# FKGSOFTWARE/TERRA-GAN

Hardware: AMD Instinct MI355X
Metric: DSM tiles/sec train-step (G+D) at 256x256 bs=16 (higher is better)
Workload: dtype f32

## Files before the change

include/terragan_hip.h:

```cpp
#ifndef TERRAGAN_HIP_H
#define TERRAGAN_HIP_H

#include <stddef.h>
#include <stdint.h>

#ifdef __cplusplus
extern "C" {
#endif

typedef void* tg_stream_t;

enum { TG_OK = 0, TG_ERR_ARG = -1, TG_ERR_LAUNCH = -2, TG_ERR_WS = -3 };
enum { TG_ACT_NONE = 0, TG_ACT_RELU = 1, TG_ACT_LEAKY = 2 };
enum { TG_PREC_F32 = 0, TG_PREC_BF16 = 1, TG_PREC_F32_WINO4 = 2 };

typedef struct TgConv {
    int32_t B, H, W, Cin;
    int32_t Ho, Wo, Cout;
    int32_t k, stride, pad;
    int32_t precision;
} TgConv;

int tg_version(void);
const char* tg_last_error(void);


size_t tg_conv_fwd_ws_bytes(const TgConv* g);
int tg_conv_fwd(const TgConv* g, const float* x, const float* in_mask, const float* w,
                const float* bias, const float* ratio, int act, float slope, float* y,
                float* ws, size_t ws_bytes, tg_stream_t stream);

size_t tg_conv_dgrad_ws_bytes(const TgConv* g);
int tg_conv_dgrad(const TgConv* g, const float* dy, const float* w, const float* in_mask,
                  float* dx, int accumulate, float* ws, size_t ws_bytes, tg_stream_t stream);
int tg_conv_dgrad_gated(const TgConv* g, const float* dy, const float* w, const float* in_mask,
                        const float* x_act, int act, float slope, float* dx, float* ws,
                        size_t ws_bytes, tg_stream_t stream);

enum { TG_WPREP_FWD = 0, TG_WPREP_DGRAD = 1 };
size_t tg_conv_wprep_bytes(const TgConv* g, int mode);
int tg_conv_wprep(const TgConv* g, int mode, const float* w, float* wprep, tg_stream_t stream);
size_t tg_conv_wprep_item_bytes(void);
int tg_conv_wprep_item(const TgConv* g, int mode, const float* w, float* wprep, void* item_out);
int tg_conv_wprep_run(const void* items_dev, int n, tg_stream_t stream);
int tg_conv_fwd_p(const TgConv* g, const float* x, const float* in_mask, const float* w, const float* wprep,
                  const float* bias, const float* ratio, int act, float slope, float* y, float* ws,
                  size_t ws_bytes, tg_stream_t stream);
int tg_conv_fwd_pool(const TgConv* g, const float* x, const float* in_mask, const float* w, const float* wprep,
                     const float* bias, const float* ratio, int act, float slope, float* y, float* pool_y, float* ws,
                     size_t ws_bytes, tg_stream_t stream);
int tg_conv_pool_code_supported(const TgConv* g);
int tg_conv_fwd_pool_code(const TgConv* g, const float* x, const float* w, const float* wprep, const float* bias,
                          float* pool_y, unsigned char* code, float* ws, size_t ws_bytes, tg_stream_t stream);
int tg_maxpool2_bwd_code(const float* dout, const unsigned char* code, int B, int Ho, int Wo, int C, float* dx,
                         tg_stream_t stream);
typedef struct TgBnAct {
    const float *mean, *rstd, *gamma, *beta;
    int32_t act;
    float slope;
} TgBnAct;
int tg_conv_bnin_supported(const TgConv* g, int wgrad);
int tg_conv_fwd_bnin(const TgConv* g, const float* x, const TgBnAct* bn, const float* w, const float* bias, int act,
                     float slope, float* y, float* ws, size_t ws_bytes, tg_stream_t stream);
int tg_conv_wgrad_bnin(const TgConv* g, const float* x, const TgBnAct* bn, const float* dy, float* dw, float* db, float* ws,
                       size_t ws_bytes, tg_stream_t stream);
int tg_conv_dgrad_p(const TgConv* g, const float* dy, const float* w, const float* wprep, const float* in_mask,
                    const float* x_act, int act, float slope, float* dx, int accumulate, float* ws,
                    size_t ws_bytes, tg_stream_t stream);
int tg_relu_gate_pack(const float* a, int64_t rows, int C, uint32_t* bits, tg_stream_t stream);
int tg_conv_dgrad_gbits(const TgConv* g, const float* dy, const float* w, const float* wprep, const float* in_mask,
                        const uint32_t* gate_bits, float* dx, int accumulate, float* ws, size_t ws_bytes, tg_stream_t stream);

int tg_set_cu_reserve(int cus);
int tg_set_work_stealing(int mode);

size_t tg_conv_wgrad_ws_bytes(const TgConv* g);
int tg_conv_wgrad(const TgConv* g, const float* x, const float* in_mask, const float* dy,
                  float* dw, float* db, float* ws, size_t ws_bytes, tg_stream_t stream);

int tg_fold_cin(const float* w3, int cout, int taps, int cin, float* w1, tg_stream_t stream);


int tg_mask_update(const float* mask, int B, int H, int W, int k, int stride, int pad, int Ho,
                   int Wo, float* mask_out, float* ratio, tg_stream_t stream);
int tg_mask_up_merge(const float* up_mask, const float* skip_mask, int B, int h, int w, int H,
                     int W, float* out, tg_stream_t stream);

#define TG_MASK_PYRAMID_MAX 24
typedef struct TgMaskOp {
    int kind, H, W, Ho, Wo, k, stride, pad;
    const float* in;
    const float* in2;
    float* out;
    float* out2;
} TgMaskOp;
typedef struct TgMaskPyramid {
    int nops, _pad;
    TgMaskOp op[TG_MASK_PYRAMID_MAX];
} TgMaskPyramid;
int tg_mask_pyramid(const TgMaskPyramid* pm, int B, tg_stream_t stream);


size_t tg_bn_ws_bytes(int64_t rows, int C);
int tg_bn_stats(const float* y, int64_t rows, int C, float eps, float momentum, float* save_mean,
                float* save_rstd, float* running_mean, float* running_var,
                int64_t* num_batches_tracked, float* ws, size_t ws_bytes, tg_stream_t stream);
int tg_bn_fwd(const float* y, int64_t rows, int C, float eps, float momentum, const float* gamma,
              const float* beta, int act, float slope, float* save_mean, float* save_rstd,
              float* running_mean, float* running_var, int64_t* num_batches_tracked, float* out,
              float* ws, size_t ws_bytes, tg_stream_t stream);
int tg_bn_eval_stats(const float* running_mean, const float* running_var, int C, float eps,
                     float* mean, float* rstd, tg_stream_t stream);
int tg_bn_act_fwd(const float* y, int64_t rows, int C, const float* mean, const float* rstd,
                  const float* gamma, const float* beta, int act, float slope, float* out,
                  tg_stream_t stream);
int tg_bn_act_bwd(const float* dout, const float* y, int64_t rows, int C, const float* mean,
                  const float* rstd, const float* gamma, const float* beta, int act, float slope,
                  const float* ratio, float* dy, float* dgamma, float* dbeta, float* dbias, float* ws,
                  size_t ws_bytes, tg_stream_t stream);
int tg_bn_bwd_conv1_supported(int64_t rows, int C);
size_t tg_bn_conv1_ws_bytes(int64_t rows, int C);
int tg_bn_act_bwd_conv1(const float* dz, const float* w, int B, int H, int W, const float* y, int C, const float* mean,
                        const float* rstd, const float* gamma, const float* beta, int act, float slope, const float* ratio,
                        float* dy, float* dgamma, float* dbeta, float* dbias, float* ws, size_t ws_bytes, tg_stream_t stream);
int tg_act_bwd(const float* dout, const float* out, int64_t rows, int C, int act, float slope,
               const float* ratio, float* din, tg_stream_t stream);


int tg_upcat_fwd(const float* up, const float* skip, const float* out_mask, int B, int h, int w,
                 int Cu, int H, int W, int Cs, float* out, tg_stream_t stream);
int tg_upcat_bn_supported(int B, int h, int w, int Cu, int H, int W, int Cs);
int tg_upcat_fwd_bn(const float* up, const TgBnAct* bn, const float* skip, const float* out_mask, int B, int h, int w,
                    int Cu, int H, int W, int Cs, float* out, tg_stream_t stream);
int tg_upcat_bwd(const float* dout, int B, int h, int w, int Cu, int H, int W, int Cs, float* dup,
                 float* dskip, tg_stream_t stream);


int tg_sigmoid_composite_fwd(const float* logits, const float* x, const float* mask, int64_t n,
                             float* out, tg_stream_t stream);
int tg_sigmoid_composite_bwd(const float* dout, const float* logits, const float* mask, int64_t n,
                             float* dlogits, float* dx, tg_stream_t stream);

int tg_maxpool2_fwd(const float* x, int B, int H, int W, int C, float* out, tg_stream_t stream);
int tg_maxpool2_bwd(const float* dout, const float* x, int B, int H, int W, int C, int relu_gate,
                    float* dx, tg_stream_t stream);


size_t tg_pixel_loss_ws_bytes(int B, int H, int W);
int tg_pixel_losses(const float* pred, const float* target, const float* mask,
                    const float* l1_weight, int B, int H, int W,
                    float w_l1, float w_tv, float w_bnd, float bnd_eps, const float* gscale,
                    float* out5, float* dpred, int accumulate, float* ws, size_t ws_bytes,
                    tg_stream_t stream);

size_t tg_reduce_ws_bytes(int64_t n);
int tg_l1_mean(const float* a, const float* b, int64_t n, float coef, const float* gscale,
               float* out1, float* da, float* ws, size_t ws_bytes, tg_stream_t stream);
int tg_l1_mean_relu(const float* a, const float* b, int64_t n, float coef, const float* gscale, float* out1, float* da,
                    float* ws, size_t ws_bytes, tg_stream_t stream);

int tg_bce_logits(const float* z, int64_t n, float target, float coef, const float* gscale,
                  float* out1, float* dz, float* ws, size_t ws_bytes, tg_stream_t stream);


int tg_adam(float* p, const float* g, float* m, float* v, int64_t n, double lr, double beta1,
            double beta2, double eps, int step, float grad_scale, tg_stream_t stream);

typedef struct TgAdamSeg {
    float* p;
    const float* g;
    float* m;
    float* v;
    int64_t n;
} TgAdamSeg;
int tg_adam_multi(const TgAdamSeg* segs_dev, const int32_t* work_dev, int nwork, int chunk_elems,
                  double lr, double beta1, double beta2, double eps, int step, float grad_scale,
                  tg_stream_t stream);

int tg_adam_scalars(double lr, double beta1, double beta2, int step, float* out2_host);
int tg_write_floats(float* dst_dev, int n, const float* vals_host, tg_stream_t stream);
int tg_adam_multi_s(const TgAdamSeg* segs_dev, const int32_t* work_dev, int nwork, int chunk_elems,
                    double beta1, double beta2, double eps, const float* scal_dev, float grad_scale,
                    tg_stream_t stream);

int tg_axpby(const float* x, float a, float b, float* y, int64_t n, tg_stream_t stream);
int tg_lincomb(const float* x, float a, const float* y, float b, float* out, int64_t n,
               tg_stream_t stream);
int tg_mul(const float* a, const float* b, float* out, int64_t n, tg_stream_t stream);
int tg_mul_keep(const float* a, const float* b, float* out, float* a_copy, int64_t n, tg_stream_t stream);
size_t tg_bn_grouped_ws_bytes(int64_t rows_per_group, int groups, int C);
int tg_bn_fwd_grouped(const float* y, int64_t rows_per_group, int groups, int C, float eps, const float* gamma,
                      const float* beta, int act, float slope, float* save_mean, float* save_rstd, float* out,
                      float* ws, size_t ws_bytes, tg_stream_t stream);
int tg_bn_act_bwd_grouped(const float* dout, const float* y, int64_t rows_per_group, int groups, int C,
                          const float* mean, const float* rstd, const float* gamma, const float* beta, int act,
                          float slope, float* dy, float* dgamma, float* dbeta, float* dbias, float* ws,
                          size_t ws_bytes, tg_stream_t stream);
int tg_bn_running_update_multi(const float* save_mean, const float* save_rstd, int64_t rows_per_group, int C,
                               float eps, float momentum, const int* order, int norder, float* running_mean,
                               float* running_var, int64_t* num_batches_tracked, tg_stream_t stream);
int tg_bn_running_update(const float* save_mean, const float* save_rstd, int64_t rows, int C,
                         float eps, float momentum, float* running_mean, float* running_var,
                         int64_t* num_batches_tracked, tg_stream_t stream);
int tg_nchw_to_nhwc(const float* x, int B, int C, int H, int W, float* y, tg_stream_t stream);
int tg_nhwc_to_nchw(const float* x, int B, int C, int H, int W, float* y, tg_stream_t stream);


size_t tg_quality_metrics_ws_bytes(int64_t imgs, int H, int W);
// ... 36 lines not shown
```

terra-gan_amd/csrc/igemm.hip:

```cpp
#include <atomic>
#include <stdlib.h>
#include <string.h>

#include <mutex>
#include <vector>

#include "common.h"

struct ProfRec {
    hipEvent_t a, b;
    int kind;
    double flops, bytes;
    int M, N, K, C, splits, cfg;
    char tag[32];
};
static std::mutex g_prof_mu;
static bool g_prof_on = false;
static std::vector<ProfRec> g_prof;
static thread_local char g_prof_tag[32] = "";

struct ProfScope {
    bool on = false;
    ProfRec r{};
    hipStream_t s;
// ... 1098 lines not shown
        p.splits = cdiv(p.T, p.steps_per_split);
        p.ws = ws + off_f;
        off_f += (size_t)p.splits * p.M * p.N;
        pm.zbeg[i] = i == 0 ? 0 : pm.zbeg[i - 1] + cls[i - 1].splits;
        pm.c[i] = p;
    }
    pm.zbeg[ncls] = pm.zbeg[ncls - 1] + cls[ncls - 1].splits;
    for (int i = ncls; i < 4; ++i) {
        pm.c[i] = pm.c[0];
        pm.zbeg[i + 1] = pm.zbeg[ncls];
    }
    if (cls[0].bf16) *rc = bn == 128 ? launch_igemm_multi_cfg<2, 2, 2, 2, true>(pm, ncls, s) : launch_igemm_multi_cfg<2, 2, 2, 1, true>(pm, ncls, s);
    else *rc = bn == 128 ? launch_igemm_multi_cfg<2, 2, 2, 2, false>(pm, ncls, s) : launch_igemm_multi_cfg<2, 2, 2, 1, false>(pm, ncls, s);
    return true;
}

static int check_conv(const TgConv* g, const char* who) {
    TG_REQUIRE(g != nullptr, "%s: null geometry", who);
    TG_REQUIRE(g->B > 0 && g->H > 0 && g->W > 0 && g->Cin > 0 && g->Cout > 0, "%s: non-positive dims", who);
    TG_REQUIRE(g->k > 0 && g->stride > 0 && g->pad >= 0, "%s: bad k/stride/pad", who);
    TG_REQUIRE(g->Ho == (g->H + 2 * g->pad - g->k) / g->stride + 1 && g->Wo == (g->W + 2 * g->pad - g->k) / g->stride + 1,
               "%s: Ho/Wo (%d,%d) inconsistent with H,W,k,s,p (%d,%d,%d,%d,%d)", who, g->Ho, g->Wo, g->H, g->W, g->k,
               g->stride, g->pad);
    TG_REQUIRE(g->Ho > 0 && g->Wo > 0, "%s: empty output", who);
    TG_REQUIRE((int64_t)g->B * g->H * g->W * (int64_t)g->Cin < (1ll << 31) &&
                   (int64_t)g->B * g->Ho * g->Wo * (int64_t)g->Cout < (1ll << 31),
               "%s: tensor too large for 32-bit pixel indexing", who);
    return TG_OK;
}
static bool aligned16(const void* ptr) { return (reinterpret_cast<uintptr_t>(ptr) & 15) == 0; }

static size_t align_up(size_t v, size_t a) { return (v + a - 1) / a * a; }
#include "wino22.inc"
static size_t conv_wino_floats(const TgConv* g) {
    if (wino22_fwd_geom_ok(g) || wino22_dgrad_geom_ok(g)) return wino22_u_floats(g);
    if (g->k != 3 || g->stride != 1 || (g->Cin % 8) != 0 || (g->Cout % 8) != 0) return 0;
    if (g->precision == TG_PREC_F32_WINO4) return align_up(wino44_u_floats(g->Cout, g->Cin), 64);
    return align_up(wino_u_floats(g->Cout, g->Cin), 64);
}

__global__ __launch_bounds__(256) void s2d_kernel(const float* __restrict__ x, const float* __restrict__ mask, float* __restrict__ x2,
                                                  int B, int H, int W, int C) {
    const int C4 = C >> 2;
    const int64_t total = (int64_t)B * H * W * C4;
    for (int64_t idx = (int64_t)blockIdx.x * 256 + threadIdx.x; idx < total; idx += (int64_t)gridDim.x * 256) {
        const int c4 = (int)(idx % C4);
        int64_t pix = idx / C4;
        const int xw = (int)(pix % W);
        int64_t t = pix / W;
        const int yh = (int)(t % H);
        const int b = (int)(t / H);
        f32x4 v = *reinterpret_cast<const f32x4*>(x + pix * C + 4 * c4);
        if (mask) v *= mask[pix];
        const int64_t p2 = ((int64_t)b * (H >> 1) + (yh >> 1)) * (W >> 1) + (xw >> 1);
        *reinterpret_cast<f32x4*>(x2 + p2 * (4 * C) + ((yh & 1) * 2 + (xw & 1)) * C + 4 * c4) = v;
    }
}
__global__ __launch_bounds__(256) void d2s_kernel(const float* __restrict__ dx2, const float* __restrict__ mask, float* __restrict__ dx,
                                                  int B, int H, int W, int C, int accumulate) {
    const int C4 = C >> 2;
    const int64_t total = (int64_t)B * H * W * C4;
    for (int64_t idx = (int64_t)blockIdx.x * 256 + threadIdx.x; idx < total; idx += (int64_t)gridDim.x * 256) {
        const int c4 = (int)(idx % C4);
        int64_t pix = idx / C4;
        const int xw = (int)(pix % W);
        int64_t t = pix / W;
        const int yh = (int)(t % H);
        const int b = (int)(t / H);
        const int64_t p2 = ((int64_t)b * (H >> 1) + (yh >> 1)) * (W >> 1) + (xw >> 1);
        f32x4 v = *reinterpret_cast<const f32x4*>(dx2 + p2 * (4 * C) + ((yh & 1) * 2 + (xw & 1)) * C + 4 * c4);
        if (mask) v *= mask[pix];
        float* o = dx + pix * C + 4 * c4;
        if (accumulate) v += *reinterpret_cast<const f32x4*>(o);
        *reinterpret_cast<f32x4*>(o) = v;
    }
}
__global__ __launch_bounds__(256) void w5x5_s2d_kernel(const float* __restrict__ src, float* __restrict__ dst, int Cout, int C, int to3) {
    const int64_t total = to3 ? (int64_t)Cout * 36 * C : (int64_t)Cout * 25 * C;
    for (int64_t idx = (int64_t)blockIdx.x * 256 + threadIdx.x; idx < total; idx += (int64_t)gridDim.x * 256) {
        const int c = (int)(idx % C);
        int64_t t = idx / C;
        if (to3) {
            const int ph = (int)(t % 4), tap = (int)((t / 4) % 9), co = (int)(t / 36);
            const int ky = 2 * (tap / 3) + (ph >> 1), kx = 2 * (tap % 3) + (ph & 1);
            dst[idx] = (ky < 5 && kx < 5) ? src[((int64_t)co * 25 + ky * 5 + kx) * C + c] : 0.f;
        } else {
            const int k = (int)(t % 25), co = (int)(t / 25);
            const int ky = k / 5, kx = k % 5;
            dst[idx] = src[(((int64_t)co * 9 + (ky >> 1) * 3 + (kx >> 1)) * 4 + (ky & 1) * 2 + (kx & 1)) * C + c];
        }
    }
}
static bool s2d_ok(const TgConv* g) {
    static const bool off = getenv("TG_NO_WINO") != nullptr || getenv("TG_NO_S2D") != nullptr;
    if (off || (g->precision == TG_PREC_BF16 && getenv("TG_NO_WINO16"))) return false;
    return g->k == 5 && g->stride == 2 && g->pad == 2 && (g->H % 2) == 0 && (g->W % 2) == 0 && (g->Cin % 16) == 0 &&
           (g->Cout % 64) == 0 && g->Ho >= 32 && g->Wo >= 32 && g->Ho == g->H / 2 && g->Wo == g->W / 2;
}
static TgConv s2d_geom(const TgConv* g) {
    TgConv g2 = *g;
    g2.H = g->H / 2; g2.W = g->W / 2; g2.Cin = 4 * g->Cin; g2.k = 3; g2.stride = 1; g2.pad = 1;
    return g2;
}
static size_t s2d_x_floats(const TgConv* g) { return align_up((size_t)g->B * g->H * g->W * g->Cin, 64); }
static size_t s2d_w_floats(const TgConv* g) { return align_up((size_t)g->Cout * 36 * g->Cin, 64); }

static size_t splitk_room_floats(size_t out) {
    const size_t cap = (size_t)64 << 20;
    return out * 64 < cap ? out * 64 : cap;
}
static size_t min_floats(size_t a, size_t b) { return a < b ? a : b; }

extern "C" size_t tg_conv_fwd_ws_bytes(const TgConv* g) {
    if (!g) return 0;
    const size_t out = (size_t)g->B * g->Ho * g->Wo * g->Cout;
    size_t base = (splitk_room_floats(out) + conv_wino_floats(g)) * sizeof(float);
    if (s2d_ok(g)) {
        const TgConv g2 = s2d_geom(g);
        base = (s2d_x_floats(g) + s2d_w_floats(g)) * sizeof(float) + tg_conv_fwd_ws_bytes(&g2);
    }
    return base;
}

static int wino_kc(const TgConv* g) {
    static const bool off16 = getenv("TG_NO_WINO16") != nullptr;
    return g->precision == TG_PREC_BF16 ? (off16 ? 0 : 16) : 8;
}
static bool wino_fwd_geom_ok(const TgConv* g) {
    static const bool off = getenv("TG_NO_WINO") != nullptr;
    const int kc = wino_kc(g);
    return !off && kc && g->k == 3 && g->stride == 1 && (g->Cin % kc) == 0 && (g->Cout % WINO_BN) == 0 && g->Ho >= 16 && g->Wo >= 16;
}
static bool wino_dgrad_geom_ok(const TgConv* g) {
    static const bool off = getenv("TG_NO_WINO") != nullptr;
    const int kc = wino_kc(g);
    return !off && kc && g->k == 3 && g->stride == 1 && (g->Cout % kc) == 0 && (g->Cin % WINO_BN) == 0 && g->H >= 16 && g->W >= 16;
}
static size_t dgrad_wt_floats(const TgConv* g);
extern "C" size_t tg_conv_wprep_bytes(const TgConv* g, int mode) {
    if (!g) return 0;
    if (s2d_ok(g)) {
        const TgConv g2 = s2d_geom(g);
        return s2d_w_floats(g) * sizeof(float) + tg_conv_wprep_bytes(&g2, mode);
    }
    if (mode == TG_WPREP_FWD) return wino_fwd_geom_ok(g) || wino22_fwd_geom_ok(g) ? conv_wino_floats(g) * sizeof(float) : 0;
    if (mode == TG_WPREP_DGRAD) return dgrad_wt_floats(g) * sizeof(float);
    return 0;
}

struct FwdExtras {
    float* pool_dst = nullptr;
    unsigned char* pool_code = nullptr;
    const BnIn* in_bn = nullptr;
    int pool_fused = 0;
};
static int conv_fwd_impl(const TgConv* g, const float* x, const float* in_mask, const float* w, float* wprep, int prep,
                         const float* bias, const float* ratio, int act, float slope, float* y, float* ws, size_t ws_bytes,
                         tg_stream_t stream, float* pool_y = nullptr, FwdExtras* ex = nullptr) {
    if (pool_y) {
        TG_REQUIRE(g && x && y && prep >= 0 && (g->Ho % 2) == 0 && (g->Wo % 2) == 0 && aligned16(pool_y),
                   "tg_conv_fwd_pool: even output sizes and a 16-byte aligned pool_y expected");
        int fused = 0;
        if (!s2d_ok(g) && !wino22_fwd_geom_ok(g)) {
            FwdExtras e;
            e.pool_dst = pool_y;
            const int rc1 = conv_fwd_impl(g, x, in_mask, w, wprep, prep, bias, ratio, act, slope, y, ws, ws_bytes, stream, nullptr, &e);
            if (rc1) return rc1;
            fused = e.pool_fused;
        } else if (int rc1 = conv_fwd_impl(g, x, in_mask, w, wprep, prep, bias, ratio, act, slope, y, ws, ws_bytes, stream)) {
            return rc1;
        }
        return fused ? TG_OK : tg_maxpool2_fwd(y, g->B, g->Ho, g->Wo, g->Cout, pool_y, stream);
    }
    int rc = check_conv(g, "tg_conv_fwd");
    if (rc) return rc;
    TG_REQUIRE(w && (prep < 0 || (x && y)), "tg_conv_fwd: null pointer");
    TG_REQUIRE(aligned16(x) && aligned16(w) && aligned16(y) && aligned16(wprep), "tg_conv_fwd: pointers must be 16-byte aligned");
    TG_REQUIRE(prep == 0 || wprep != nullptr, "tg_conv_fwd: prepared weights expected");
    const bool ws_ok = ws && aligned16(ws) && ws_bytes >= tg_conv_fwd_ws_bytes(g);
    if (s2d_ok(g) && (prep < 0 || ws_ok)) {
        hipStream_t s = (hipStream_t)stream;
        const TgConv g2 = s2d_geom(g);
        float* x2 = ws;
        float* w2 = prep ? wprep : ws + s2d_x_floats(g);
        float* ws2 = ws ? ws + s2d_x_floats(g) + s2d_w_floats(g) : nullptr;
        if (prep < 0 && g_wprep_capture) {
            const int rc2 = conv_fwd_impl(&g2, nullptr, nullptr, w2, wprep + s2d_w_floats(g), -1, nullptr, nullptr, 0, 0.f, nullptr, nullptr,
                                          0, stream);
            if (rc2 == TG_OK && g_wprep_captured == 1 && g_wprep_capture->kind == 1) {
                g_wprep_capture->kind = 4; g_wprep_capture->w = w; g_wprep_capture->taps = g->Cin;
            } else {
                g_wprep_captured = -1;
            }
            return rc2;
        }
        if (prep <= 0) {
            hipLaunchKernelGGL(w5x5_s2d_kernel, dim3(ew_grid((int64_t)g->Cout * 36 * g->Cin, 256)), dim3(256), 0, s, w, w2, g->Cout, g->Cin, 1);
            TG_CHECK_LAUNCH("w5x5_s2d_kernel");
        }
        if (prep >= 0) {
            hipLaunchKernelGGL(s2d_kernel, dim3(ew_grid((int64_t)g->B * g->H * g->W * (g->Cin / 4), 256)), dim3(256), 0, s, x, in_mask, x2,
                               g->B, g->H, g->W, g->Cin);
            TG_CHECK_LAUNCH("s2d_kernel");
        }
        AlgScale sc(25.0 / 36.0);
        return conv_fwd_impl(&g2, x2, nullptr, w2, prep ? wprep + s2d_w_floats(g) : nullptr, prep, bias, ratio, act, slope, y, ws2,
                             ws ? ws_bytes - (s2d_x_floats(g) + s2d_w_floats(g)) * sizeof(float) : 0, stream);
    }
    TG_REQUIRE(!(s2d_ok(g) && prep > 0), "tg_conv_fwd: workspace too small for the prepared 5x5 stride-2 path");
    IGemmParams p = {};
    p.src = x; p.amask = in_mask; p.wmat = w; p.bias = bias; p.rowscale = ratio; p.dst = y; p.ws = ws;
    p.B = g->B; p.IH = g->H; p.IW = g->W; p.C = g->Cin;
    p.OH = g->Ho; p.OW = g->Wo; p.N = g->Cout; p.M = g->B * g->Ho * g->Wo;
    p.DH = g->Ho; p.DW = g->Wo; p.ds = 1; p.dy0 = 0; p.dx0 = 0;
    p.TH = g->k; p.TW = g->k; p.ss = g->stride; p.tstep = 1; p.sy0 = -g->pad; p.sx0 = -g->pad;
    p.KW = g->k; p.kstep = 1; p.ky0 = 0; p.kx0 = 0;
    p.Kfull = g->k * g->k * g->Cin;
    p.act = act; p.slope = slope; p.accumulate = 0;
    p.bf16 = g->precision == TG_PREC_BF16;
    p.wino4 = g->precision == TG_PREC_F32_WINO4;
    p.Ktot = p.TH * p.TW * p.C; p.nchunks = cdiv(p.C, 32);
    p.T = (p.C % 4) ? cdiv(p.Ktot, 32) : p.TH * p.TW * p.nchunks;
    size_t ws_floats = ws ? ws_bytes / sizeof(float) : 0;
    const size_t uf = conv_wino_floats(g);
    const size_t room = splitk_room_floats((size_t)p.M * p.N);
    if (wino22_fwd_geom_ok(g) && (prep || (ws_floats >= uf && aligned16(ws)))) {
        p.w_raw = w;
        p.wino_u = prep ? wprep : ws;
        p.wino_ready = prep;
        if (!prep) {
            p.ws = ws + uf;
            ws_floats -= uf;
        }
        return launch_wino22(g, p, 0, min_floats(ws_floats, room), (hipStream_t)stream);
    }
    if (wino_fwd_geom_ok(g) && (prep || (ws_floats >= uf && aligned16(ws)))) {
        p.w_raw = w; p.w_sn = (long)p.Kfull; p.w_sk = 1; p.w_stap = g->Cin;
        p.wino_u = prep ? wprep : ws;
        p.wino_ready = prep;
        bool in_ws = !prep;
        if (wino44_prepared_unusable(p)) {
            TG_REQUIRE(ws_floats >= uf && aligned16(ws), "tg_conv_fwd: workspace too small to re-prepare the weights (%zu < %zu floats)",
                       ws_floats, uf);
            p.wino_u = ws;
            p.wino_ready = 0;
            in_ws = true;
        }
        TG_REQUIRE(p.bf16 ? wino16_ok(p) : wino_ok(p), "tg_conv_fwd: internal: Winograd geometry predicate mismatch");
        if (in_ws) {
            p.ws = ws + uf;
            ws_floats -= uf;
        }
    }
    if (prep < 0 && !p.wino_u) return TG_OK;
    if (ex) {
        p.pool_dst = ex->pool_dst;
        p.pool_code = ex->pool_code;
        p.pool_only = ex->pool_code != nullptr;
        if (ex->in_bn) {
            p.in_bn = *ex->in_bn;
            TG_REQUIRE(smallconv_bnin_fwd_ok(p), "tg_conv_fwd_bnin: geometry not supported (ask tg_conv_bnin_supported first)");
        }
    }
    ws_floats = min_floats(ws_floats, room);
    plan_splits(p, ws_floats);
    rc = launch_igemm(p, (hipStream_t)stream, ws_floats);
    if (ex) ex->pool_fused = p.pool_done;
    return rc;
}
extern "C" int tg_conv_fwd_pool(const TgConv* g, const float* x, const float* in_mask, const float* w, const float* wprep,
                                const float* bias, const float* ratio, int act, float slope, float* y, float* pool_y, float* ws,
                                size_t ws_bytes, tg_stream_t stream) {
    TG_REQUIRE(pool_y, "tg_conv_fwd_pool: null pointer");
    return conv_fwd_impl(g, x, in_mask, w, const_cast<float*>(wprep), wprep ? 1 : 0, bias, ratio, act, slope, y, ws, ws_bytes, stream,
                         pool_y);
}
extern "C" int tg_conv_pool_code_supported(const TgConv* g) {
    if (!g || (g->precision != TG_PREC_F32 && g->precision != TG_PREC_BF16) || !wino_fwd_geom_ok(g) || s2d_ok(g) || (g->Ho & 1) || (g->Wo & 1)) return 0;
    if (getenv("TG_NO_FUSED_POOL") || getenv("TG_NO_POOL_CODE") || getenv("TG_WINO_NO_PIPE") || getenv("TG_WINO_NO_FAST")) return 0;
    if ((size_t)g->B * g->Ho * g->Wo * g->Cout * 4 >= ((size_t)1 << 31) || (size_t)g->B * g->H * g->W * g->Cin * 4 >= ((size_t)1 << 31)) return 0;
    const int nchunks = g->Cin / wino_kc(g);
    if (nchunks < 2) return 0;
    const long work = (long)cdiv(g->Wo, 16) * cdiv(g->Ho, 16) * g->B * (g->Cout / WINO_BN);
    return nchunks < 16 || work >= 4L * WINO_PLAN_CUS ? 1 : 0;
}
extern "C" int tg_conv_fwd_pool_code(const TgConv* g, const float* x, const float* w, const float* wprep, const float* bias,
                                     float* pool_y, unsigned char* code, float* ws, size_t ws_bytes, tg_stream_t stream) {
    TG_REQUIRE(pool_y && code && aligned16(pool_y) && (reinterpret_cast<uintptr_t>(code) & 3) == 0, "tg_conv_fwd_pool_code: bad pointers");
    TG_REQUIRE(tg_conv_pool_code_supported(g), "tg_conv_fwd_pool_code: geometry not supported (ask tg_conv_pool_code_supported first)");
    FwdExtras e;
    e.pool_dst = pool_y;
    e.pool_code = code;
    const int rc = conv_fwd_impl(g, x, nullptr, w, const_cast<float*>(wprep), wprep ? 1 : 0, bias, nullptr, TG_ACT_RELU, 0.f, pool_y, ws,
                                 ws_bytes, stream, nullptr, &e);
    if (rc) return rc;
    TG_REQUIRE(e.pool_fused, "tg_conv_fwd_pool_code: internal: the launch did not take the fused path");
    return TG_OK;
}
static bool bnin_geom_ok(const TgConv* g) {
    return g && g->Cout == 1 && g->Cin == 64 && g->k == 3 && g->stride == 1 && g->pad == 1 && (g->Wo % 4) == 0;
}
static BnIn bnin_of(const TgBnAct* bn) { return BnIn{bn->mean, bn->rstd, bn->gamma, bn->beta, bn->act, bn->slope}; }
extern "C" int tg_conv_bnin_supported(const TgConv* g, int wgrad) {
    if (!bnin_geom_ok(g)) return 0;
    if (wgrad) {
        WgradParams p = {};
        p.B = g->B; p.H = g->H; p.W = g->W; p.C = g->Cin; p.Ho = g->Ho; p.Wo = g->Wo; p.Cout = g->Cout;
        p.k = g->k; p.stride = g->stride; p.pad = g->pad;
        p.Mpix = g->B * g->Ho * g->Wo; p.Ktot = g->k * g->k * g->Cin;
        return smallconv_wgrad_applies(p) && smallconv_bnin_wgrad_ok(p) ? 1 : 0;
    }
    IGemmParams p = {};
    p.B = g->B; p.IH = g->H; p.IW = g->W; p.C = g->Cin; p.OH = g->Ho; p.OW = g->Wo; p.N = g->Cout; p.M = g->B * g->Ho * g->Wo;
    p.TH = g->k; p.TW = g->k; p.ss = g->stride; p.tstep = 1; p.sy0 = -g->pad; p.sx0 = -g->pad;
    return smallconv_bnin_fwd_ok(p) ? 1 : 0;
}
extern "C" int tg_conv_fwd_bnin(const TgConv* g, const float* x, const TgBnAct* bn, const float* w, const float* bias, int act,
                                float slope, float* y, float* ws, size_t ws_bytes, tg_stream_t stream) {
    TG_REQUIRE(bn && bn->mean && bn->rstd && bn->gamma && bn->beta, "tg_conv_fwd_bnin: null pointer");
    TG_REQUIRE(tg_conv_bnin_supported(g, 0), "tg_conv_fwd_bnin: geometry not supported (ask tg_conv_bnin_supported first)");
    const BnIn b = bnin_of(bn);
    FwdExtras e;
    e.in_bn = &b;
    return conv_fwd_impl(g, x, nullptr, w, nullptr, 0, bias, nullptr, act, slope, y, ws, ws_bytes, stream, nullptr, &e);
}
extern "C" int tg_conv_fwd(const TgConv* g, const float* x, const float* in_mask, const float* w, const float* bias,
                           const float* ratio, int act, float slope, float* y, float* ws, size_t ws_bytes,
                           tg_stream_t stream) {
    return conv_fwd_impl(g, x, in_mask, w, nullptr, 0, bias, ratio, act, slope, y, ws, ws_bytes, stream);
}
extern "C" int tg_conv_fwd_p(const TgConv* g, const float* x, const float* in_mask, const float* w, const float* wprep,
                             const float* bias, const float* ratio, int act, float slope, float* y, float* ws, size_t ws_bytes,
                             tg_stream_t stream) {
    return conv_fwd_impl(g, x, in_mask, w, const_cast<float*>(wprep), wprep ? 1 : 0, bias, ratio, act, slope, y, ws, ws_bytes,
                         stream);
}

__global__ __launch_bounds__(256) void transpose_w_kernel(const float* __restrict__ w, float* __restrict__ wt,
                                                          int cout, int taps, int cin) {
    const size_t total = (size_t)cout * taps * cin;
    for (size_t idx = (size_t)blockIdx.x * 256 + threadIdx.x; idx < total; idx += (size_t)gridDim.x * 256) {
        int co = (int)(idx % cout);
        size_t r = idx / cout;
        int t = (int)(r % taps);
        int ci = (int)(r / taps);
        wt[idx] = w[((size_t)co * taps + t) * cin + ci];
    }
}

static size_t dgrad_wt_floats(const TgConv* g) {
    size_t wt = align_up((size_t)g->Cout * g->k * g->k * g->Cin, 64);
    size_t uf = conv_wino_floats(g);
    return wt > uf ? wt : uf;
}
extern "C" size_t tg_conv_dgrad_ws_bytes(const TgConv* g) {
    if (!g) return 0;
    if (s2d_ok(g)) {
        const TgConv g2 = s2d_geom(g);
        return (s2d_x_floats(g) + s2d_w_floats(g)) * sizeof(float) + tg_conv_dgrad_ws_bytes(&g2);
    }
    return (dgrad_wt_floats(g) + splitk_room_floats((size_t)g->B * g->H * g->W * g->Cin)) * sizeof(float);
}

static int conv_dgrad_impl(const TgConv* g, const float* dy, const float* w, float* wprep, int prep, const float* in_mask, float* dx,
                           int accumulate, const float* gate, int gate_act, float gate_slope, float* ws, size_t ws_bytes,
                           tg_stream_t stream, const uint32_t* gate_bits = nullptr, int* gate_bits_done = nullptr);
extern "C" int tg_conv_dgrad(const TgConv* g, const float* dy, const float* w, const float* in_mask, float* dx,
                             int accumulate, float* ws, size_t ws_bytes, tg_stream_t stream) {
    return conv_dgrad_impl(g, dy, w, nullptr, 0, in_mask, dx, accumulate, nullptr, 0, 0.f, ws, ws_bytes, stream);
}
extern "C" int tg_conv_dgrad_gated(const TgConv* g, const float* dy, const float* w, const float* in_mask, const float* x_act,
                                   int act, float slope, float* dx, float* ws, size_t ws_bytes, tg_stream_t stream) {
    TG_REQUIRE(x_act != nullptr && (act == TG_ACT_RELU || act == TG_ACT_LEAKY), "tg_conv_dgrad_gated: needs x_act and a ReLU/LeakyReLU");
    return conv_dgrad_impl(g, dy, w, nullptr, 0, in_mask, dx, 0, x_act, act, slope, ws, ws_bytes, stream);
}
extern "C" int tg_conv_dgrad_p(const TgConv* g, const float* dy, const float* w, const float* wprep, const float* in_mask,
                               const float* x_act, int act, float slope, float* dx, int accumulate, float* ws, size_t ws_bytes,
                               tg_stream_t stream) {
    TG_REQUIRE(x_act == nullptr || ((act == TG_ACT_RELU || act == TG_ACT_LEAKY) && !accumulate),
               "tg_conv_dgrad_p: a gated dgrad needs a ReLU/LeakyReLU and accumulate == 0");
    const bool usable = wprep != nullptr && !(x_act != nullptr && g && s2d_ok(g));
    return conv_dgrad_impl(g, dy, w, usable ? const_cast<float*>(wprep) : nullptr, usable ? 1 : 0, in_mask, dx, accumulate, x_act,
                           act, slope, ws, ws_bytes, stream);
}
extern "C" int tg_conv_dgrad_gbits(const TgConv* g, const float* dy, const float* w, const float* wprep, const float* in_mask,
                                   const uint32_t* gate_bits, float* dx, int accumulate, float* ws, size_t ws_bytes, tg_stream_t stream) {
    int rc = check_conv(g, "tg_conv_dgrad_gbits");
    if (rc) return rc;
    TG_REQUIRE(dy && w && gate_bits && dx && ws, "tg_conv_dgrad_gbits: null pointer");
    TG_REQUIRE(!accumulate, "tg_conv_dgrad_gbits: a gated dgrad does not accumulate");
    TG_REQUIRE(g->Cin % 32 == 0, "tg_conv_dgrad_gbits: needs Cin %% 32 == 0 (one gate word per 32 channels), got %d", g->Cin);
    TG_REQUIRE((reinterpret_cast<uintptr_t>(gate_bits) & 15) == 0, "tg_conv_dgrad_gbits: pointers must be 16-byte aligned");
    const bool usable = wprep != nullptr && !s2d_ok(g);
    int done = 0;
    rc = conv_dgrad_impl(g, dy, w, usable ? const_cast<float*>(wprep) : nullptr, usable ? 1 : 0, in_mask, dx, 0, nullptr, TG_ACT_NONE, 0.f,
                         ws, ws_bytes, stream, gate_bits, &done);
    if (rc || done) return rc;
    return gate_bits_apply_launch(dx, gate_bits, (int64_t)g->B * g->H * g->W, g->Cin, (hipStream_t)stream);
}
extern "C" int tg_conv_wprep(const TgConv* g, int mode, const float* w, float* wprep, tg_stream_t stream) {
    TG_REQUIRE(g && w && wprep, "tg_conv_wprep: null pointer");
    TG_REQUIRE(mode == TG_WPREP_FWD || mode == TG_WPREP_DGRAD, "tg_conv_wprep: bad mode %d", mode);
    TG_REQUIRE(tg_conv_wprep_bytes(g, mode) > 0, "tg_conv_wprep: this (geometry, mode) runs on the raw weights");
    if (mode == TG_WPREP_FWD)
        return conv_fwd_impl(g, nullptr, nullptr, w, wprep, -1, nullptr, nullptr, 0, 0.f, nullptr, nullptr, 0, stream);
    return conv_dgrad_impl(g, nullptr, w, wprep, -1, nullptr, nullptr, 0, nullptr, 0, 0.f, nullptr, 0, stream);
}
extern "C" size_t tg_conv_wprep_item_bytes(void) { return sizeof(TgWprepItem); }
extern "C" int tg_conv_wprep_item(const TgConv* g, int mode, const float* w, float* wprep, void* item_out) {
    if (!g || !w || !wprep || !item_out || (mode != TG_WPREP_FWD && mode != TG_WPREP_DGRAD)) return 0;
    if (tg_conv_wprep_bytes(g, mode) == 0) return 0;
    TgWprepItem it = {};
    g_wprep_capture = &it;
    g_wprep_captured = 0;
    int rc = mode == TG_WPREP_FWD ? conv_fwd_impl(g, nullptr, nullptr, w, wprep, -1, nullptr, nullptr, 0, 0.f, nullptr, nullptr, 0, nullptr)
                                  : conv_dgrad_impl(g, nullptr, w, wprep, -1, nullptr, nullptr, 0, nullptr, 0, 0.f, nullptr, 0, nullptr);
    g_wprep_capture = nullptr;
    if (rc != TG_OK || g_wprep_captured != 1) return 0;
    memcpy(item_out, &it, sizeof(it));
    return 1;
}
extern "C" int tg_conv_wprep_run(const void* items_dev, int n, tg_stream_t stream) {
    TG_REQUIRE(items_dev && n > 0, "tg_conv_wprep_run: bad arguments");
    hipLaunchKernelGGL(wprep_multi_kernel, dim3(2048, n), dim3(256), 0, (hipStream_t)stream, static_cast<const TgWprepItem*>(items_dev));
    TG_CHECK_LAUNCH("wprep_multi_kernel");
    return TG_OK;
}
static int conv_dgrad_impl(const TgConv* g, const float* dy, const float* w, float* wprep, int prep, const float* in_mask, float* dx,
                           int accumulate, const float* gate, int gate_act, float gate_slope, float* ws, size_t ws_bytes,
                           tg_stream_t stream, const uint32_t* gate_bits, int* gate_bits_done) {
    int rc = check_conv(g, "tg_conv_dgrad");
    if (rc) return rc;
    TG_REQUIRE(w && (prep < 0 || (dy && dx && ws)), "tg_conv_dgrad: null pointer");
    TG_REQUIRE(aligned16(dy) && aligned16(w) && aligned16(dx) && aligned16(ws) && aligned16(wprep),
               "tg_conv_dgrad: pointers must be 16-byte aligned");
    TG_REQUIRE(prep == 0 || wprep != nullptr, "tg_conv_dgrad: prepared weights expected");
    if (s2d_ok(g) && gate == nullptr && gate_bits == nullptr && (prep < 0 || ws_bytes >= tg_conv_dgrad_ws_bytes(g))) {
        hipStream_t s2 = (hipStream_t)stream;
        const TgConv g2 = s2d_geom(g);
        float* dx2 = ws;
        float* w2 = prep ? wprep : ws + s2d_x_floats(g);
        float* wsr = ws ? ws + s2d_x_floats(g) + s2d_w_floats(g) : nullptr;
        if (prep < 0 && g_wprep_capture) {
            const int rc2 = conv_dgrad_impl(&g2, nullptr, w2, wprep + s2d_w_floats(g), -1, nullptr, nullptr, 0, nullptr, 0, 0.f, nullptr, 0, stream);
            if (rc2 == TG_OK && g_wprep_captured == 1 && g_wprep_capture->kind == 1) {
                g_wprep_capture->kind = 4; g_wprep_capture->w = w; g_wprep_capture->taps = g->Cin;
            } else {
                g_wprep_captured = -1;
            }
            return rc2;
// ... 816 lines not shown
```

terra-gan_amd/csrc/igemm_params.h:

```cpp
#pragma once
#include "common.h"

struct BnIn {
    const float *mean, *rstd, *gamma, *beta;
    int act;
    float slope;
};
struct IGemmParams {
    const float* src;
    const float* amask;
    const float* wmat;
    const float* bias;
    const float* rowscale;
    float* dst;
    float* ws;
    int B, IH, IW, C;
    int OH, OW, N, M;
    int DH, DW, ds, dy0, dx0;
    int TH, TW, ss, tstep, sy0, sx0;
    int KW, kstep, ky0, kx0;
    int Kfull, Ktot;
    int nchunks, T;
    int splits, steps_per_split;
    int act;
    float slope;
    int accumulate;
    int bf16;
    const float* gate;
    int gate_act;
    float gate_slope;
    const float* w_raw;
    long w_sn, w_sk, w_stap;
    float* wino_u;
    int wino4;
    int wino_ready;
    float* pool_dst;
    int pool_done;
    unsigned char* pool_code;
    int pool_only;
    BnIn in_bn;
    const uint32_t* gate_bits;
    int gate_bits_done;
};
__device__ __forceinline__ float gate_factor(const IGemmParams& p, size_t idx) {
    const float gv = p.gate[idx];
    return gv > 0.f ? 1.f : (p.gate_act == TG_ACT_LEAKY ? p.gate_slope : 0.f);
}

int gate_bits_apply_launch(float* dx, const uint32_t* bits, int64_t rows, int C, hipStream_t s);

struct IGemmMulti {
    IGemmParams c[4];
    int zbeg[5];
};

struct WgradParams {
    const float* x;
    const float* amask;
    const float* dy;
    float* out;
    int B, H, W, C, Ho, Wo, Cout, k, stride, pad;
    int Mpix, Ktot, T, splits, steps_per_split;
    int nx, ny;
    int rowseg;
    BnIn in_bn;
};

bool smallconv_fwd_applies(const IGemmParams& p);
int smallconv_fwd_launch(const IGemmParams& p, hipStream_t s);
bool smallconv_to1_multi_applies(const IGemmParams* cls, int ncls);
int smallconv_to1_multi_launch(const IGemmParams* cls, int ncls, hipStream_t s);
bool smallconv_wgrad_applies(const WgradParams& p);
bool smallconv_bnin_fwd_ok(const IGemmParams& p);
bool smallconv_bnin_wgrad_ok(const WgradParams& p);
size_t smallconv_wgrad_ws_floats(const WgradParams& p);
int smallconv_wgrad_launch(const WgradParams& p, float* dw, float* ws, size_t ws_floats, hipStream_t s, float* db = nullptr,
                           int* db_done = nullptr);
```

terra-gan_amd/csrc/pointwise.hip:

```cpp
#include <math.h>
#include <string.h>

#include "common.h"

static thread_local char g_err[512] = "";
void tg_set_error(const char* fmt, ...) {
    va_list ap;
    va_start(ap, fmt);
    vsnprintf(g_err, sizeof(g_err), fmt, ap);
    va_end(ap);
}
extern "C" const char* tg_last_error(void) { return g_err; }
extern "C" int tg_version(void) { return 100; }

static size_t align_up(size_t v, size_t a) { return (v + a - 1) / a * a; }
static inline hipStream_t S(tg_stream_t s) { return (hipStream_t)s; }

constexpr int CR_MAXPASS = 4;

struct ColGeom {
    int cpp;
    int rlanes;
    int npass;
    int grid;
// ... 158 lines not shown
    const float* x;
    int C;
    __device__ void operator()(int64_t r, int c, float (&q)[1]) const { q[0] += x[r * C + c]; }
};
__global__ __launch_bounds__(256) void colsum_final_kernel(const float* __restrict__ partial, int nblocks, int C,
                                                           float* __restrict__ out) {
    double s[1];
    int c;
    if (final_reduce<1>(partial, nblocks, C, s, &c)) out[c] = (float)s[0];
}
size_t tg_colsum_ws_floats(int64_t rows, int C) {
    ColGeom g = col_geom(rows, C);
    return align_up((size_t)g.grid * C, 64);
}
int tg_colsum_launch(const float* x, int64_t rows, int C, float* out, float* ws, hipStream_t s) {
    TG_REQUIRE(C >= 1 && C <= 1024, "colsum: C=%d out of range [1,1024]", C);
    ColGeom g = col_geom(rows, C);
    ColSumF f{x, C};
    hipLaunchKernelGGL((colreduce_kernel<1, ColSumF>), dim3(g.grid), dim3(256), 0, s, f, rows, C, g.cpp, g.rlanes,
                       g.rows_per_block, ws);
    TG_CHECK_LAUNCH("colsum");
    hipLaunchKernelGGL(colsum_final_kernel, dim3(fr_grid(C)), dim3(256), 0, s, ws, g.grid, C, out);
    TG_CHECK_LAUNCH("colsum_final");
    return TG_OK;
}

__global__ __launch_bounds__(256) void mask_update_kernel(const float* __restrict__ mask, int B, int H, int W, int k,
                                                          int stride, int pad, int Ho, int Wo,
                                                          float* __restrict__ mask_out, float* __restrict__ ratio) {
    const int64_t total = (int64_t)B * Ho * Wo;
    for (int64_t idx = (int64_t)blockIdx.x * 256 + threadIdx.x; idx < total; idx += (int64_t)gridDim.x * 256) {
        int ox = (int)(idx % Wo);
        int64_t t = idx / Wo;
        int oy = (int)(t % Ho);
        int b = (int)(t / Ho);
        float s = 0.f;
        for (int ky = 0; ky < k; ++ky) {
            int iy = oy * stride - pad + ky;
            if (iy < 0 || iy >= H) continue;
            for (int kx = 0; kx < k; ++kx) {
                int ix = ox * stride - pad + kx;
                if (ix < 0 || ix >= W) continue;
                s += mask[((int64_t)b * H + iy) * W + ix];
            }
        }
        const float on = s > 0.f ? 1.f : 0.f;
        mask_out[idx] = on;
        ratio[idx] = (1.0f / (s + 1e-8f)) * (float)(k * k) * on;
    }
}
extern "C" int tg_mask_update(const float* mask, int B, int H, int W, int k, int stride, int pad, int Ho, int Wo,
                              float* mask_out, float* ratio, tg_stream_t stream) {
    TG_REQUIRE(mask && mask_out && ratio, "tg_mask_update: null pointer");
    TG_REQUIRE(B > 0 && H > 0 && W > 0 && k > 0 && stride > 0 && pad >= 0, "tg_mask_update: bad dims");
    TG_REQUIRE(Ho == (H + 2 * pad - k) / stride + 1 && Wo == (W + 2 * pad - k) / stride + 1 && Ho > 0 && Wo > 0,
               "tg_mask_update: Ho/Wo inconsistent");
    hipLaunchKernelGGL(mask_update_kernel, dim3(ew_grid((int64_t)B * Ho * Wo, 256)), dim3(256), 0, S(stream), mask, B, H, W,
                       k, stride, pad, Ho, Wo, mask_out, ratio);
    TG_CHECK_LAUNCH("mask_update_kernel");
    return TG_OK;
}

__host__ __device__ inline int floordiv2(int a) { return a >= 0 ? a / 2 : -((-a + 1) / 2); }

__global__ __launch_bounds__(256) void mask_up_merge_kernel(const float* __restrict__ up, const float* __restrict__ skip,
                                                            int B, int h, int w, int H, int W, int offy, int offx,
                                                            float* __restrict__ out) {
    const int64_t total = (int64_t)B * H * W;
    for (int64_t idx = (int64_t)blockIdx.x * 256 + threadIdx.x; idx < total; idx += (int64_t)gridDim.x * 256) {
        int X = (int)(idx % W);
        int64_t t = idx / W;
        int Y = (int)(t % H);
        int b = (int)(t / H);
        int yu = Y - offy, xu = X - offx;
        float v = 0.f;
        if (yu >= 0 && yu < 2 * h && xu >= 0 && xu < 2 * w) v = up[((int64_t)b * h + (yu >> 1)) * w + (xu >> 1)];
        out[idx] = fmaxf(v, skip[idx]);
    }
}
extern "C" int tg_mask_up_merge(const float* up_mask, const float* skip_mask, int B, int h, int w, int H, int W,
                                float* out, tg_stream_t stream) {
    TG_REQUIRE(up_mask && skip_mask && out && B > 0 && h > 0 && w > 0 && H > 0 && W > 0, "tg_mask_up_merge: bad arguments");
    hipLaunchKernelGGL(mask_up_merge_kernel, dim3(ew_grid((int64_t)B * H * W, 256)), dim3(256), 0, S(stream), up_mask,
                       skip_mask, B, h, w, H, W, floordiv2(H - 2 * h), floordiv2(W - 2 * w), out);
    TG_CHECK_LAUNCH("mask_up_merge_kernel");
    return TG_OK;
}


__device__ __forceinline__ void mask_update_one(const float* __restrict__ mask, int H, int W, int k, int stride, int pad, int Ho,
                                                int Wo, int b, int idx, float* __restrict__ mask_out, float* __restrict__ ratio) {
    const int ox = idx % Wo, oy = idx / Wo;
    float s = 0.f;
    if (k == 3) {
        float v[9];
#pragma unroll
        for (int t = 0; t < 9; ++t) {
            const int iy = oy * stride - pad + t / 3, ix = ox * stride - pad + t % 3;
            const bool ok = iy >= 0 && iy < H && ix >= 0 && ix < W;
            const float m = mask[((int64_t)b * H + (ok ? iy : 0)) * W + (ok ? ix : 0)];
            v[t] = ok ? m : 0.f;
        }
#pragma unroll
        for (int t = 0; t < 9; ++t) s += v[t];
    } else {
        for (int ky = 0; ky < k; ++ky) {
            const int iy = oy * stride - pad + ky;
            if (iy < 0 || iy >= H) continue;
            for (int kx = 0; kx < k; ++kx) {
                const int ix = ox * stride - pad + kx;
                if (ix < 0 || ix >= W) continue;
                s += mask[((int64_t)b * H + iy) * W + ix];
            }
        }
    }
    const float on = s > 0.f ? 1.f : 0.f;
    const int64_t o = ((int64_t)b * Ho + oy) * Wo + ox;
    mask_out[o] = on;
    ratio[o] = (1.0f / (s + 1e-8f)) * (float)(k * k) * on;
}
__global__ __launch_bounds__(1024) void mask_pyramid_kernel(const TgMaskPyramid pm) {
    const int b = blockIdx.x;
    for (int i = 0; i < pm.nops; ++i) {
        const TgMaskOp op = pm.op[i];
        if (op.kind == 0) {
            for (int idx = threadIdx.x; idx < op.Ho * op.Wo; idx += 1024)
                mask_update_one(op.in, op.H, op.W, op.k, op.stride, op.pad, op.Ho, op.Wo, b, idx, op.out, op.out2);
        } else {
            const int offy = floordiv2(op.Ho - 2 * op.H), offx = floordiv2(op.Wo - 2 * op.W);
            for (int idx = threadIdx.x; idx < op.Ho * op.Wo; idx += 1024) {
                const int X = idx % op.Wo, Y = idx / op.Wo;
                const int yu = Y - offy, xu = X - offx;
                float v = 0.f;
                if (yu >= 0 && yu < 2 * op.H && xu >= 0 && xu < 2 * op.W) v = op.in[((int64_t)b * op.H + (yu >> 1)) * op.W + (xu >> 1)];
                const int64_t o = ((int64_t)b * op.Ho + Y) * op.Wo + X;
                op.out[o] = fmaxf(v, op.in2[o]);
            }
        }
        __syncthreads();
    }
}
extern "C" int tg_mask_pyramid(const TgMaskPyramid* pm, int B, tg_stream_t stream) {
    TG_REQUIRE(pm && B > 0 && pm->nops >= 1 && pm->nops <= TG_MASK_PYRAMID_MAX, "tg_mask_pyramid: bad arguments");
    for (int i = 0; i < pm->nops; ++i) {
        const TgMaskOp& op = pm->op[i];
        TG_REQUIRE(op.in && op.out && (op.kind == 0 ? op.out2 != nullptr : op.in2 != nullptr), "tg_mask_pyramid: op %d: null pointer", i);
        TG_REQUIRE(op.H > 0 && op.W > 0 && op.Ho > 0 && op.Wo > 0, "tg_mask_pyramid: op %d: bad dims", i);
        if (op.kind == 0)
            TG_REQUIRE(op.k > 0 && op.stride > 0 && op.pad >= 0 && op.Ho == (op.H + 2 * op.pad - op.k) / op.stride + 1 &&
                       op.Wo == (op.W + 2 * op.pad - op.k) / op.stride + 1, "tg_mask_pyramid: op %d: Ho/Wo inconsistent", i);
    }
    hipLaunchKernelGGL(mask_pyramid_kernel, dim3(B), dim3(1024), 0, S(stream), *pm);
    TG_CHECK_LAUNCH("mask_pyramid_kernel");
    return TG_OK;
}

struct BnStatF {
    const float* y;
    int C;
    __device__ BnStatF group(int g, int64_t rows_g) const { return BnStatF{y + (size_t)g * rows_g * C, C}; }
    __device__ void operator()(int64_t r, int c, float (&q)[2]) const {
        float d = y[r * C + c] - y[c];
        q[0] += d;
        q[1] += d * d;
    }
    __device__ void quad(int64_t r, int c0, float (&q)[2][4]) const {
        const f32x4 v = *reinterpret_cast<const f32x4*>(y + r * C + c0);
        const f32x4 sh = *reinterpret_cast<const f32x4*>(y + c0);
#pragma unroll
        for (int e = 0; e < 4; ++e) {
            float d = v[e] - sh[e];
            q[0][e] += d;
            q[1][e] += d * d;
        }
    }
};
__global__ __launch_bounds__(256) void bn_finalize_kernel(const float* __restrict__ partial, int nblocks, int C,
                                                          const float* __restrict__ y, int64_t rows, float eps,
                                                          float momentum, float* __restrict__ mean_out,
                                                          float* __restrict__ rstd_out, float* __restrict__ rm,
                                                          float* __restrict__ rv, int64_t* __restrict__ nbt) {
    if (blockIdx.x == 0 && threadIdx.x == 0 && nbt) *nbt += 1;
    double q[2];
    int c;
    if (!final_reduce<2>(partial, nblocks, C, q, &c)) return;
    const double n = (double)rows;
    const double md = q[0] / n;
    double var = q[1] / n - md * md;
    if (var < 0.0) var = 0.0;
    const double mean = (double)y[c] + md;
    mean_out[c] = (float)mean;
    rstd_out[c] = (float)(1.0 / sqrt(var + (double)eps));
    if (rm) rm[c] = (float)((1.0 - (double)momentum) * (double)rm[c] + (double)momentum * mean);
    if (rv) rv[c] = (float)((1.0 - (double)momentum) * (double)rv[c] + (double)momentum * var * (n / (n - 1.0)));
}
extern "C" size_t tg_bn_ws_bytes(int64_t rows, int C) {
    if (rows <= 0 || C <= 0) return 0;
    ColGeom g = col_geom(rows, C);
    int grid = g.grid;
    if (C % 4 == 0) {
        ColGeom4 g4 = col_geom4(rows, C);
        if (g4.grid > grid) grid = g4.grid;
    }
    return align_up((size_t)grid * 5 * C, 64) * sizeof(float);
}
extern "C" int tg_bn_stats(const float* y, int64_t rows, int C, float eps, float momentum, float* save_mean,
                           float* save_rstd, float* running_mean, float* running_var, int64_t* num_batches_tracked,
                           float* ws, size_t ws_bytes, tg_stream_t stream) {
    TG_REQUIRE(y && save_mean && save_rstd && ws, "tg_bn_stats: null pointer");
    TG_REQUIRE(C >= 1 && C <= 1024, "tg_bn_stats: C=%d out of range [1,1024]", C);
    TG_REQUIRE(rows > 1, "tg_bn_stats: Expected more than 1 value per channel when training (rows=%lld)", (long long)rows);
    TG_REQUIRE(ws_bytes >= tg_bn_ws_bytes(rows, C), "tg_bn_stats: workspace too small");
    BnStatF f{y, C};
    int nblocks;
    if (C % 4 == 0) {
        ColGeom4 g = col_geom4(rows, C);
        nblocks = g.grid;
        hipLaunchKernelGGL((colreduce4_kernel<2, BnStatF>), dim3(g.grid), dim3(256), 0, S(stream), f, rows, C, g.qpp, g.rlanes,
                           g.rows_per_block, ws, 0);
    } else {
        ColGeom g = col_geom(rows, C);
        nblocks = g.grid;
        hipLaunchKernelGGL((colreduce_kernel<2, BnStatF>), dim3(g.grid), dim3(256), 0, S(stream), f, rows, C, g.cpp, g.rlanes,
                           g.rows_per_block, ws);
    }
    TG_CHECK_LAUNCH("bn_stats");
    hipLaunchKernelGGL(bn_finalize_kernel, dim3(fr_grid(C)), dim3(256), 0, S(stream), ws, nblocks, C, y, rows, eps,
                       momentum, save_mean, save_rstd, running_mean, running_var, num_batches_tracked);
    TG_CHECK_LAUNCH("bn_finalize");
    return TG_OK;
}

__global__ __launch_bounds__(256) void bn_eval_stats_kernel(const float* rm, const float* rv, int C, float eps, float* mean,
                                                            float* rstd) {
    int c = blockIdx.x * 256 + threadIdx.x;
    if (c >= C) return;
    mean[c] = rm[c];
    rstd[c] = 1.0f / sqrtf(rv[c] + eps);
}
extern "C" int tg_bn_eval_stats(const float* running_mean, const float* running_var, int C, float eps, float* mean,
                                float* rstd, tg_stream_t stream) {
    TG_REQUIRE(running_mean && running_var && mean && rstd && C > 0, "tg_bn_eval_stats: bad arguments");
    hipLaunchKernelGGL(bn_eval_stats_kernel, dim3(cdiv(C, 256)), dim3(256), 0, S(stream), running_mean, running_var, C, eps,
                       mean, rstd);
    TG_CHECK_LAUNCH("bn_eval_stats_kernel");
    return TG_OK;
}

__global__ __launch_bounds__(256) void bn_act_fwd4_kernel(const float* __restrict__ y, int64_t rows, int C, int qpp, int rlanes,
                                                          const float* __restrict__ mean, const float* __restrict__ rstd,
                                                          const float* __restrict__ gamma, const float* __restrict__ beta,
                                                          int act, float slope, float* __restrict__ out) {
    const int cq = threadIdx.x % qpp, rl = threadIdx.x / qpp;
    if (rl >= rlanes) return;
    const int nquads = C >> 2;
    for (int q0 = blockIdx.y * qpp; q0 < nquads; q0 += gridDim.y * qpp) {
        const int c0 = (q0 + cq) * 4;
        if (c0 >= C) continue;
        const f32x4 mv = *reinterpret_cast<const f32x4*>(mean + c0), rv = *reinterpret_cast<const f32x4*>(rstd + c0);
        const f32x4 gv = *reinterpret_cast<const f32x4*>(gamma + c0), bv = *reinterpret_cast<const f32x4*>(beta + c0);
        for (int64_t r = (int64_t)blockIdx.x * rlanes + rl; r < rows; r += (int64_t)gridDim.x * rlanes) {
            const f32x4 v = *reinterpret_cast<const f32x4*>(y + r * C + c0);
            f32x4 o;
#pragma unroll
            for (int e = 0; e < 4; ++e) o[e] = apply_act(bn_affine(v[e], mv[e], rv[e], gv[e], bv[e]), act, slope);
            *reinterpret_cast<f32x4*>(out + r * C + c0) = o;
        }
    }
}
__global__ __launch_bounds__(256) void bn_act_fwd1_kernel(const float* __restrict__ y, int64_t total, int C,
                                                          const float* __restrict__ mean, const float* __restrict__ rstd,
                                                          const float* __restrict__ gamma, const float* __restrict__ beta,
                                                          int act, float slope, float* __restrict__ out) {
    for (int64_t i = (int64_t)blockIdx.x * 256 + threadIdx.x; i < total; i += (int64_t)gridDim.x * 256) {
        const int c = (int)(i % C);
        float xh = (y[i] - mean[c]) * rstd[c];
        out[i] = apply_act(xh * gamma[c] + beta[c], act, slope);
    }
}
struct RowGeom {
    int qpp, rlanes;
    dim3 grid;
};
static RowGeom row_geom(int64_t rows, int C) {
    RowGeom g;
    const int nquads = C / 4;
    g.qpp = nquads < 256 ? nquads : 256;
    g.rlanes = 256 / g.qpp;
    int64_t gx = cdiv64(rows, (int64_t)g.rlanes * 4);
    if (gx > 2048) gx = 2048;
    if (gx < 1) gx = 1;
    g.grid = dim3((unsigned)gx, (unsigned)cdiv(nquads, g.qpp));
    return g;
}
extern "C" int tg_bn_act_fwd(const float* y, int64_t rows, int C, const float* mean, const float* rstd, const float* gamma,
                             const float* beta, int act, float slope, float* out, tg_stream_t stream) {
    TG_REQUIRE(y && mean && rstd && gamma && beta && out && rows > 0 && C > 0, "tg_bn_act_fwd: bad arguments");
    if (C % 4 == 0) {
        RowGeom g = row_geom(rows, C);
        hipLaunchKernelGGL(bn_act_fwd4_kernel, g.grid, dim3(256), 0, S(stream), y, rows, C, g.qpp, g.rlanes, mean, rstd, gamma,
                           beta, act, slope, out);
    } else {
        hipLaunchKernelGGL(bn_act_fwd1_kernel, dim3(ew_grid(rows * C, 256)), dim3(256), 0, S(stream), y, rows * C, C, mean, rstd,
                           gamma, beta, act, slope, out);
    }
    TG_CHECK_LAUNCH("bn_act_fwd_kernel");
// ... 1697 lines not shown
```

terra-gan_amd/csrc/wino.inc:

```
#pragma once
#include <utility>

struct WinoGeom {
    int tiles_x, tiles_y, total_work, chunks_per_split, nt;
    int sy_min, sx_min;
    int interleave;
    int* qctr;
};
struct WinoWeights {
    long sn, sk, stap;
    int kyu[3], kxv[3];
    int k_fast;
};
typedef unsigned int u32x4 __attribute__((ext_vector_type(4)));
constexpr int WINO_BN = 64;
constexpr int WINO_V = 16 * 64 * 8;
constexpr int WINO_U = 16 * WINO_BN * 8;
constexpr int WINO_PPIX = 18 * 18;
constexpr int WINO_P = WINO_PPIX * 8;
constexpr int WINO_LDS_FLOATS = 2 * WINO_V + 2 * WINO_U + WINO_P;
constexpr int WINO_THREADS = 512;

__device__ __forceinline__ void wino_barrier() { asm volatile("s_waitcnt lgkmcnt(0)\n\ts_barrier" ::: "memory"); }

template <class F, int... T>
__device__ __forceinline__ void wino_static_for(std::integer_sequence<int, T...>, F&& f) {
    (f(std::integral_constant<int, T>{}), ...);
}

__device__ __forceinline__ void wino_distribute(int total, int interleave, int& item, int& item_end, int& step) {
    const int G = gridDim.x;
    if (interleave) {
        const int xcd = blockIdx.x & 7, slot = blockIdx.x >> 3, nslots = (G - xcd + 7) >> 3;
        const int ch_q = total >> 3, ch_r = total & 7;
        const int chunk0 = xcd < ch_r ? xcd * (ch_q + 1) : ch_r * (ch_q + 1) + (xcd - ch_r) * ch_q;
        item = chunk0 + slot;
        item_end = chunk0 + ch_q + (xcd < ch_r ? 1 : 0);
        step = nslots;
    } else {
        const int rblk = xcd_remap(blockIdx.x, G);
        const int per = total / G, rem = total % G;
        item = rblk * per + min(rblk, rem);
        item_end = item + per + (rblk < rem ? 1 : 0);
        step = 1;
    }
}

constexpr int WQ_Z = 16;
constexpr int WQ_INTS = 8 * WQ_Z + 8;
__device__ __forceinline__ int wq_chunk0(int total, int c) { const int q = total >> 3, r = total & 7; return c < r ? c * (q + 1) : r * (q + 1) + (c - r) * q; }
__device__ __forceinline__ int wq_len(int total, int c) { return (total >> 3) + (c < (total & 7) ? 1 : 0); }
template <bool STEAL>
struct WinoWork {
    int item;
    int item_end, step;
    int* home_ctr;
    int home_c0, home_len;

    __device__ __forceinline__ void init(int total, int interleave, int* ctr, int* slot) {
        if constexpr (!STEAL) {
            wino_distribute(total, interleave, item, item_end, step);
            if (item >= item_end) item = -1;
        } else {
            const int home = blockIdx.x & 7, rank = blockIdx.x >> 3;
            const int nwg = (gridDim.x - home + 7) >> 3;
            const int len = wq_len(total, home), c0 = wq_chunk0(total, home);
            home_ctr = ctr + 8 * blockIdx.z + home;
            home_c0 = c0 + nwg;
            home_len = len - nwg;
            item = rank < len ? c0 + rank : -1;
            step = 0; item_end = 0;
            if (threadIdx.x == 0) {
                int nx = -1;
                if (item >= 0 && home_len > 0) {
                    const int i = atomicAdd(home_ctr, 1);
                    if (i < home_len) nx = home_c0 + i;
                }
                slot[0] = nx;
            }
            __syncthreads();
        }
    }
    __device__ __forceinline__ int next(const int* slot) const {
        if constexpr (!STEAL) return item + step < item_end ? item + step : -1;
        else return __builtin_amdgcn_readfirstlane(slot[step]);
    }
    __device__ __forceinline__ int request(int nxt) const {
        int r = -1;
        if constexpr (STEAL) {
            if (threadIdx.x == 0 && nxt >= 0) {
                const int i = atomicAdd(home_ctr, 1);
                r = i < home_len ? home_c0 + i : -1;
            }
        }
        return r;
    }
    __device__ __forceinline__ void publish(int pulled, int* slot) const {
        if constexpr (STEAL) { if (threadIdx.x == 0) slot[step ^ 1] = pulled; }
    }
    __device__ __forceinline__ void advance(int nxt) {
        item = nxt;
        if constexpr (STEAL) step ^= 1;
    }
    __device__ __forceinline__ void done(int* ctr) const {
        if constexpr (STEAL) {
            if (threadIdx.x == 0) {
                const int n = gridDim.x * gridDim.z;
                if (atomicAdd(ctr + 8 * WQ_Z, 1) == n - 1) {
                    for (int i = 0; i <= 8 * WQ_Z; ++i) __hip_atomic_store(ctr + i, 0, __ATOMIC_RELAXED, __HIP_MEMORY_SCOPE_AGENT);
                }
            }
        }
    }
};

static bool wino_interleave_ok(size_t u_bytes) {
    static const char* e = getenv("TG_WINO_INTERLEAVE");
    if (e) return atoi(e) != 0;
    return u_bytes <= ((size_t)6 << 20);
}

__host__ __device__ __forceinline__ int wino_swz(int row, int kk) { return ((((kk >> 2) ^ (row >> 4)) & 1) << 2) + (kk & 3); }

template <bool S2D>
__device__ __forceinline__ void wino_weights_body(const float* __restrict__ w, float* __restrict__ U, int N, int K,
                                                  const WinoWeights& ww, int cin5 = 0) {
    const int NT = N / WINO_BN;
    const size_t total = (size_t)N * K;
    const int KC = K >> 3;
    for (size_t idx = (size_t)blockIdx.x * 256 + threadIdx.x; idx < total; idx += (size_t)gridDim.x * 256) {
        const int blk = (int)(idx >> 9);
        const int k = (blk % KC) * 8 + (int)(idx & 7), n = (blk / KC) * WINO_BN + (int)((idx >> 3) & 63);
        float g[3][3];
        if constexpr (S2D) {
            const int c2 = ww.k_fast ? k : n, co = ww.k_fast ? n : k;
            const int ph = c2 / cin5, c = c2 - ph * cin5, dy = ph >> 1, dx = ph & 1;
            const float* wp = w + (size_t)co * 25 * cin5 + c;
#pragma unroll
            for (int u = 0; u < 3; ++u)
#pragma unroll
                for (int v = 0; v < 3; ++v) {
                    const int ky = 2 * ww.kyu[u] + dy, kx = 2 * ww.kxv[v] + dx;
                    g[u][v] = (ky < 5 && kx < 5) ? wp[(size_t)(ky * 5 + kx) * cin5] : 0.f;
                }
        } else {
            const float* wp = w + (size_t)n * ww.sn + (size_t)k * ww.sk;
#pragma unroll
            for (int u = 0; u < 3; ++u)
#pragma unroll
                for (int v = 0; v < 3; ++v) g[u][v] = wp[(size_t)(ww.kyu[u] * 3 + ww.kxv[v]) * ww.stap];
        }
        float tg[4][3];
#pragma unroll
        for (int v = 0; v < 3; ++v) {
            tg[0][v] = g[0][v];
            tg[1][v] = 0.5f * (g[0][v] + g[1][v] + g[2][v]);
            tg[2][v] = 0.5f * (g[0][v] - g[1][v] + g[2][v]);
            tg[3][v] = g[2][v];
        }
        const int row = n % WINO_BN;
// ... 164 lines not shown

    if (wk.item < 0 || c_begin >= c_end) { wk.done(q.qctr); return; }
    locate();
    decode();
#pragma unroll
    for (int i = 0; i < 2; ++i) pload1(c_begin, i);
#pragma unroll
    for (int j = 0; j < 4; ++j) uload1(c_begin, j);

    for (;;) {
    f32x16 acc[8];
#pragma unroll
    for (int i = 0; i < 8; ++i)
#pragma unroll
        for (int r = 0; r < 16; ++r) acc[i][r] = 0.f;

    {
#pragma unroll
        for (int i = 0; i < 2; ++i) pstore1(i);
#pragma unroll
        for (int j = 0; j < 4; ++j) ustore1(0, j);
#pragma unroll
        for (int i = 0; i < 2; ++i) pload1(min(c_begin + 1, c_last), i);
#pragma unroll
        for (int j = 0; j < 4; ++j) uload1(min(c_begin + 1, c_last), j);
        wino_barrier();
#pragma unroll
        for (int k = 0; k < 8; ++k) t_read1(k);
#pragma unroll
        for (int j = 0; j < 4; ++j) t_row1(j);
#pragma unroll
        for (int k = 0; k < 4; ++k) t_col1(0, k);
        wino_barrier();
        f32x4 fa[2], fb[2];
        fa[0] = *reinterpret_cast<const f32x4*>(Vs + a_off);
        fb[0] = *reinterpret_cast<const f32x4*>(Us + b_off);
        int cur = 0;
        for (int c = c_begin; c < c_end; ++c) {
            const int nxt = cur ^ 1;
            const int c2 = min(c + 2, c_last);
            const float* Vc = Vs + cur * WINO_V + a_off;
            const float* Uc = Us + cur * WINO_U + b_off;
            const float* Vn = Vs + nxt * WINO_V + a_off;
            const float* Un = Us + nxt * WINO_U + b_off;
            wino_static_for(std::make_integer_sequence<int, 32>{}, [&](auto tc) {
                constexpr int t = decltype(tc)::value;
                constexpr int xi = t >> 2, e = t & 3;
                if constexpr (t < 2) pstore1(t);
                if constexpr (t >= 2 && t < 4) pload1(c2, t - 2);
                if constexpr (t == 4) wino_barrier();
                if constexpr (t >= 5 && t < 9) { t_read1(t - 5); t_read1(4 + t - 5); }
                if constexpr (t >= 8 && t < 12) { t_row1(t - 8); }
                if constexpr (t >= 14 && t < 18) t_col1(nxt, t - 14);
                if constexpr (t >= 18 && t < 22) ustore1(nxt, t - 18);
                if constexpr (t >= 22 && t < 26) uload1(c2, t - 22);
                if constexpr (t == 26) wino_barrier();
                if constexpr (e == 0 && xi < 7) {
                    fa[(xi + 1) & 1] = *reinterpret_cast<const f32x4*>(Vc + (xi + 1) * 512);
                    fb[(xi + 1) & 1] = *reinterpret_cast<const f32x4*>(Uc + (xi + 1) * 512);
                }
                if constexpr (e == 0 && xi == 7) {
                    fa[0] = *reinterpret_cast<const f32x4*>(Vn);
                    fb[0] = *reinterpret_cast<const f32x4*>(Un);
                }
                __builtin_amdgcn_sched_barrier(0);
                acc[xi] = __builtin_amdgcn_mfma_f32_32x32x2f32(fa[xi & 1][e], fb[xi & 1][e], acc[xi], 0, 0, 0);
                __builtin_amdgcn_sched_barrier(0);
            });
            cur = nxt;
        }
    }
    const int e_n0 = n0, e_oy0 = oy0, e_ox0 = ox0, e_b = b;
    const int wq_next = wk.next(wq_slot);
    const bool more_items = wq_next >= 0;
    const int wq_pulled = wk.request(wq_next);
    wino_barrier();

    float* X = smem;
    float* scratch = smem + 16 * 1024 + wave * (32 * 36);
    f32x16 own[2];
#pragma unroll
    for (int j = 0; j < 2; ++j) {
        float* xs = X + (((xh * 2 + nw) * 2 + mw) * 2 + j) * 1024 + lane;
#pragma unroll
        for (int r = 0; r < 16; ++r) {
            const float s0 = j == 0 ? acc[0][r] + acc[1][r] + acc[2][r] : acc[1][r] - acc[2][r] - acc[3][r];
            const float s1 = j == 0 ? acc[4][r] + acc[5][r] + acc[6][r] : acc[5][r] - acc[6][r] - acc[7][r];
            own[j][r] = xh == 0 ? s0 + s1 : -s0 - s1;
            xs[r * 64] = xh == 0 ? s1 : s0;
        }
    }
    if (more_items) {
        wk.item = wq_next;
        locate();
        decode();
#pragma unroll
        for (int i = 0; i < 2; ++i) pload1(c_begin, i);
#pragma unroll
        for (int j = 0; j < 4; ++j) uload1(c_begin, j);
    }
    wino_barrier();
    constexpr bool gated = GATED;
    f32x4 bq = {0.f, 0.f, 0.f, 0.f};
    if (p.bias && p.splits == 1) bq = *reinterpret_cast<const f32x4*>(p.bias + e_n0 + 32 * nw + 4 * (lane & 7));
    float rsq[2][4] = {{1.f, 1.f, 1.f, 1.f}, {1.f, 1.f, 1.f, 1.f}};
    if (p.rowscale && p.splits == 1) {
#pragma unroll
        for (int j = 0; j < 2; ++j)
#pragma unroll
            for (int t4 = 0; t4 < 4; ++t4) {
                const int t = 32 * mw + (lane >> 3) + 8 * t4;
                const int oy = min(e_oy0 + 2 * (t >> 3) + xh, p.OH - 1), ox = min(e_ox0 + 2 * (t & 7) + j, p.OW - 1);
                rsq[j][t4] = p.rowscale[((size_t)e_b * p.DH + (oy * p.ds + p.dy0)) * p.DW + (ox * p.ds + p.dx0)];
            }
    }
#pragma unroll
    for (int j = 0; j < 2; ++j) {
        f32x4 gq[GATED ? 4 : 1];
        if constexpr (gated) {
#pragma unroll
            for (int t4 = 0; t4 < 4; ++t4) {
                const int t = 32 * mw + (lane >> 3) + 8 * t4;
                const int oy = min(e_oy0 + 2 * (t >> 3) + xh, p.OH - 1), ox = min(e_ox0 + 2 * (t & 7) + j, p.OW - 1);
                const size_t pix = ((size_t)e_b * p.DH + (oy * p.ds + p.dy0)) * p.DW + (ox * p.ds + p.dx0);
                gq[t4] = *reinterpret_cast<const f32x4*>(p.gate + pix * p.N + e_n0 + 32 * nw + 4 * (lane & 7));
            }
        }
        const float* xr = X + ((((xh ^ 1) * 2 + nw) * 2 + mw) * 2 + j) * 1024 + lane;
        f32x16 y;
#pragma unroll
        for (int r = 0; r < 16; ++r) y[r] = own[j][r] + xr[r * 64];
        tile_rows4i(scratch, y, lane, [&](int t4, int rr, int cc, f32x4 v4) {
            const int t = 32 * mw + rr;
            const int oy = e_oy0 + 2 * (t >> 3) + xh, ox = e_ox0 + 2 * (t & 7) + j;
            const int nb = e_n0 + 32 * nw + cc;
            if (oy >= p.OH || ox >= p.OW) return;
            if (p.splits > 1) {
                const size_t m = ((size_t)e_b * p.OH + oy) * p.OW + ox;
                *reinterpret_cast<f32x4*>(p.ws + ((size_t)blockIdx.z * p.M + m) * p.N + nb) = v4;
            } else {
                const size_t pix = ((size_t)e_b * p.DH + (oy * p.ds + p.dy0)) * p.DW + (ox * p.ds + p.dx0);
                *reinterpret_cast<f32x4*>(p.dst + pix * p.N + nb) = epilogue4(p, v4, pix, nb, gated ? &gq[gated ? t4 : 0] : nullptr, &rsq[j][t4], &bq);
            }
        });
    }
    wk.publish(wq_pulled, wq_slot);
    if (!more_items) break;
    wino_barrier();
    wk.advance(wq_next);
    }
    wk.done(q.qctr);
}

template <bool GATED, bool STEAL, bool POOL = false, bool GBITS = false>
__global__ __launch_bounds__(WINO_THREADS) void wino_pipe_kernel(const IGemmParams p, const WinoGeom q, const float* __restrict__ U) {
    extern __shared__ __attribute__((aligned(16))) float smem[];
    float* Vs = smem;
    float* Us = smem + 2 * WINO_V;
    float* Ps = smem + 2 * WINO_V + 2 * WINO_U;

    const int tid = threadIdx.x, lane = tid & 63, wave = tid >> 6;
    const int mw = wave & 1, nw = (wave >> 1) & 1, xh = wave >> 2;
    __shared__ int wq_slot[2];
    WinoWork<STEAL> wk;
    wk.init(q.total_work, q.interleave, q.qctr, wq_slot);

    struct Item { int nt, n0, oy0, ox0, b; uint32_t poff[2]; };
    auto decode_item = [&](int it) {
        Item r;
        r.nt = it % q.nt;
        int tile = it / q.nt;
        const int tx = tile % q.tiles_x;
        tile /= q.tiles_x;
        const int ty = tile % q.tiles_y;
        r.b = tile / q.tiles_y;
        r.n0 = r.nt * WINO_BN; r.oy0 = ty * 16; r.ox0 = tx * 16;
        const int py0 = r.oy0 + q.sy_min, px0 = r.ox0 + q.sx_min;
#pragma unroll
        for (int i = 0; i < 2; ++i) {
            const int pp = (tid + WINO_THREADS * i) >> 1, spy = pp / 18, spx = pp - spy * 18;
            const int iy = py0 + spy, ix = px0 + spx;
            r.poff[i] = 0x80000000u;
            if (pp < WINO_PPIX && iy >= 0 && iy < p.IH && ix >= 0 && ix < p.IW)
                r.poff[i] = ((((uint32_t)r.b * p.IH + iy) * p.IW + ix) * (uint32_t)p.C + 4 * (tid & 1)) * 4u;
        }
        return r;
    };
    const auto srsrc = __builtin_amdgcn_make_buffer_rsrc(const_cast<float*>(p.src), 0, (int)((size_t)p.B * p.IH * p.IW * p.C * 4), 0x00020000);
    const auto ursrc = __builtin_amdgcn_make_buffer_rsrc(const_cast<float*>(U), 0, (int)((size_t)16 * p.N * p.C * 4), 0x00020000);
    const uint32_t u_voff = tid * 16;
    const bool p1_ok = ((tid + WINO_THREADS) >> 1) < WINO_PPIX;
    const int c_begin = blockIdx.z * q.chunks_per_split;
    const int c_end = min(p.C >> 3, c_begin + q.chunks_per_split);
    const size_t ustep = (size_t)q.nt * WINO_U;

    f32x4 ru[4], rp[2];
    auto pload1 = [&](uint32_t voff, int c, int i) { rp[i] = __builtin_bit_cast(f32x4, __builtin_amdgcn_raw_buffer_load_b128(srsrc, voff, c * 32, 0)); };
    auto uload1 = [&](int nt, int c, int j) {
        ru[j] = __builtin_bit_cast(f32x4, __builtin_amdgcn_raw_buffer_load_b128(
            ursrc, u_voff, (int)(((size_t)nt * WINO_U + (size_t)c * ustep) * 4) + 16 * WINO_THREADS * j, 0));
    };
    auto pstore1 = [&](int i) { if (i == 0 || p1_ok) *reinterpret_cast<f32x4*>(Ps + 4 * (tid + WINO_THREADS * i)) = rp[i]; };
    auto ustore1 = [&](int buf, int j) { *reinterpret_cast<f32x4*>(Us + buf * WINO_U + 4 * (tid + WINO_THREADS * j)) = ru[j]; };

    const int t_quad = lane & 1, t_tile = (lane >> 1) + 32 * (wave & 1), t_a = wave >> 1;
    const int t_r0 = t_a == 0 ? 0 : (t_a == 2 ? 2 : 1), t_r1 = t_a == 3 ? 3 : (t_a == 2 ? 1 : 2);
    const float t_s1 = t_a == 1 ? 1.f : -1.f;
    const int t_src0 = ((2 * (t_tile >> 3) + t_r0) * 18 + 2 * (t_tile & 7)) * 8 + 4 * t_quad;
    const int t_src1 = ((2 * (t_tile >> 3) + t_r1) * 18 + 2 * (t_tile & 7)) * 8 + 4 * t_quad;
    const int t_dst = (t_a * 4) * 512 + t_tile * 8 + (((t_quad ^ (t_tile >> 4)) & 1) << 2);
    f32x4 td[2][4], tt[4];
    auto t_read1 = [&](int k) { td[k >> 2][k & 3] = *reinterpret_cast<const f32x4*>(Ps + ((k >> 2) ? t_src1 : t_src0) + (k & 3) * 8); };
    auto t_row1 = [&](int j) { tt[j] = td[0][j] + td[1][j] * t_s1; };
    auto t_col1 = [&](int buf, int k) {
        const f32x4 v = k == 0 ? tt[0] - tt[2] : k == 1 ? tt[1] + tt[2] : k == 2 ? tt[2] - tt[1] : tt[1] - tt[3];
        *reinterpret_cast<f32x4*>(Vs + buf * WINO_V + t_dst + k * 512) = v;
    };

    const int arow = 32 * mw + (lane & 31), brow = 32 * nw + (lane & 31);
    const int a_off = (8 * xh) * 512 + arow * 8 + ((((lane >> 5) ^ (arow >> 4)) & 1) << 2);
    const int b_off = (8 * xh) * 512 + brow * 8 + ((((lane >> 5) ^ (brow >> 4)) & 1) << 2);

    if (wk.item < 0 || c_begin >= c_end) { wk.done(q.qctr); return; }
    Item ci = decode_item(wk.item);
#pragma unroll
    for (int i = 0; i < 2; ++i) pload1(ci.poff[i], c_begin, i);
#pragma unroll
    for (int j = 0; j < 4; ++j) uload1(ci.nt, c_begin, j);
#pragma unroll
    for (int i = 0; i < 2; ++i) pstore1(i);
#pragma unroll
    for (int j = 0; j < 4; ++j) ustore1(0, j);
#pragma unroll
    for (int i = 0; i < 2; ++i) pload1(ci.poff[i], c_begin + 1, i);
#pragma unroll
    for (int j = 0; j < 4; ++j) uload1(ci.nt, c_begin + 1, j);
    wino_barrier();
#pragma unroll
    for (int k = 0; k < 8; ++k) t_read1(k);
#pragma unroll
    for (int j = 0; j < 4; ++j) t_row1(j);
#pragma unroll
    for (int k = 0; k < 4; ++k) t_col1(0, k);
    wino_barrier();
    int cur = 0;

    for (;;) {
        f32x16 acc[8];
#pragma unroll
        for (int i = 0; i < 8; ++i)
#pragma unroll
            for (int r = 0; r < 16; ++r) acc[i][r] = 0.f;
        const int wq_next = wk.next(wq_slot);
        const bool more_items = wq_next >= 0;
        const Item ni = decode_item(more_items ? wq_next : wk.item);
        f32x4 fa[2], fb[2];
        fa[0] = *reinterpret_cast<const f32x4*>(Vs + cur * WINO_V + a_off);
        fb[0] = *reinterpret_cast<const f32x4*>(Us + cur * WINO_U + b_off);
        auto kstep = [&](uint32_t pv0, uint32_t pv1, int unt, int c2) {
            const int nxt = cur ^ 1;
            const float* Vc = Vs + cur * WINO_V + a_off;
            const float* Uc = Us + cur * WINO_U + b_off;
            const float* Vn = Vs + nxt * WINO_V + a_off;
            const float* Un = Us + nxt * WINO_U + b_off;
            wino_static_for(std::make_integer_sequence<int, 32>{}, [&](auto tc) {
                constexpr int t = decltype(tc)::value;
                constexpr int xi = t >> 2, e = t & 3;
                if constexpr (t < 2) pstore1(t);
                if constexpr (t == 2) pload1(pv0, c2, 0);
                if constexpr (t == 3) pload1(pv1, c2, 1);
                if constexpr (t == 4) wino_barrier();
                if constexpr (t >= 5 && t < 9) { t_read1(t - 5); t_read1(4 + t - 5); }
                if constexpr (t >= 8 && t < 12) { t_row1(t - 8); }
                if constexpr (t >= 14 && t < 18) t_col1(nxt, t - 14);
                if constexpr (t >= 18 && t < 22) ustore1(nxt, t - 18);
                if constexpr (t >= 22 && t < 26) uload1(unt, c2, t - 22);
                if constexpr (t == 26) wino_barrier();
                if constexpr (e == 0 && xi < 7) {
                    fa[(xi + 1) & 1] = *reinterpret_cast<const f32x4*>(Vc + (xi + 1) * 512);
                    fb[(xi + 1) & 1] = *reinterpret_cast<const f32x4*>(Uc + (xi + 1) * 512);
                }
                if constexpr (e == 0 && xi == 7) {
                    fa[0] = *reinterpret_cast<const f32x4*>(Vn);
                    fb[0] = *reinterpret_cast<const f32x4*>(Un);
                }
                __builtin_amdgcn_sched_barrier(0);
                acc[xi] = __builtin_amdgcn_mfma_f32_32x32x2f32(fa[xi & 1][e], fb[xi & 1][e], acc[xi], 0, 0, 0);
                __builtin_amdgcn_sched_barrier(0);
            });
            cur = nxt;
        };
        for (int c = c_begin; c < c_end - 2; ++c) kstep(ci.poff[0], ci.poff[1], ci.nt, c + 2);
        kstep(ni.poff[0], ni.poff[1], ni.nt, c_begin);
        kstep(ni.poff[0], ni.poff[1], ni.nt, c_begin + 1);
        const int wq_pulled = wk.request(wk.next(wq_slot));
        const int fr = cur ^ 1;
        float* X = Vs + fr * WINO_V;
        float* scratch = wave < 7 ? Us + fr * WINO_U + wave * (32 * 36) : Ps;
        const int e_wave = __builtin_amdgcn_readfirstlane(wave);
        const int e_mw = e_wave & 1, e_nw = (e_wave >> 1) & 1, e_xh = e_wave >> 2;
        const int e_row0 = ci.oy0 + 8 * e_mw + e_xh;
        const int e_pitch = p.DW * p.ds;
        const int e_pix0 = (ci.b * p.DH + p.dy0) * p.DW + p.dx0 + ci.ox0 * p.ds;
        const int e_nb0 = ci.n0 + 32 * e_nw;
        const uint32_t e_lane_px = 2 * (lane >> 3) * p.ds;
        const bool e_single = p.splits == 1;
        const float act_neg = p.act == TG_ACT_RELU ? 0.f : (p.act == TG_ACT_LEAKY ? p.slope : 1.f);
        const float gate_neg = p.gate_act == TG_ACT_LEAKY ? p.gate_slope : 0.f;
        const auto drsrc = __builtin_amdgcn_make_buffer_rsrc(p.dst, 0, (int)((size_t)p.B * p.DH * p.DW * p.N * 4), 0x00020000);
        f32x4 bq = {0.f, 0.f, 0.f, 0.f};
        if (p.bias && e_single) bq = *reinterpret_cast<const f32x4*>(p.bias + e_nb0 + 4 * (lane & 7));
        f32x4 pmx[POOL ? 4 : 1];
        uint32_t jbits = 0;
        if constexpr (POOL) {
#pragma unroll
            for (int t4 = 0; t4 < 4; ++t4) pmx[t4] = f32x4{0.f, 0.f, 0.f, 0.f};
        }
        float rsq[2][4] = {{1.f, 1.f, 1.f, 1.f}, {1.f, 1.f, 1.f, 1.f}};
        if (p.rowscale && e_single) {
            const auto rrsrc = __builtin_amdgcn_make_buffer_rsrc(const_cast<float*>(p.rowscale), 0, (int)((size_t)p.B * p.DH * p.DW * 4), 0x00020000);
#pragma unroll
            for (int j = 0; j < 2; ++j) {
                const uint32_t voff = ci.ox0 + 2 * (lane >> 3) + j < p.OW ? e_lane_px * 4u : 0x80000000u;
#pragma unroll
                for (int t4 = 0; t4 < 4; ++t4) {
                    const int row = min(e_row0 + 2 * t4, p.OH - 1);
                    rsq[j][t4] = __builtin_bit_cast(float, __builtin_amdgcn_raw_buffer_load_b32(
                        rrsrc, voff, (e_pix0 + row * e_pitch + j * p.ds) * 4, 0));
                }
            }
        }
#pragma unroll
        for (int j = 0; j < 2; ++j) {
            f32x16 own;
            {
                float* xs = X + ((xh * 2 + nw) * 2 + mw) * 1024 + lane;
#pragma unroll
                for (int r = 0; r < 16; ++r) {
                    const float s0 = j == 0 ? acc[0][r] + acc[1][r] + acc[2][r] : acc[1][r] - acc[2][r] - acc[3][r];
                    const float s1 = j == 0 ? acc[4][r] + acc[5][r] + acc[6][r] : acc[5][r] - acc[6][r] - acc[7][r];
                    own[r] = xh == 0 ? s0 + s1 : -s0 - s1;
                    xs[r * 64] = xh == 0 ? s1 : s0;
                }
            }
            const uint32_t e_voff = ci.ox0 + 2 * (lane >> 3) + j < p.OW
                                        ? ((e_lane_px + j * p.ds) * (uint32_t)p.N + 4 * (lane & 7)) * 4u : 0x80000000u;
            f32x4 gq[GATED && !GBITS ? 4 : 1];
            uint32_t gw[GBITS ? 4 : 1];
            if constexpr (GBITS) {
                const int nw32 = p.N >> 5;
                const auto brsrc = __builtin_amdgcn_make_buffer_rsrc(const_cast<uint32_t*>(p.gate_bits), 0, (int)((size_t)p.B * p.DH * p.DW * nw32 * 4), 0x00020000);
                const uint32_t b_voff = ci.ox0 + 2 * (lane >> 3) + j < p.OW ? (e_lane_px + j * p.ds) * (uint32_t)nw32 * 4u : 0x80000000u;
#pragma unroll
                for (int t4 = 0; t4 < 4; ++t4) {
                    const int row = min(e_row0 + 2 * t4, p.OH - 1);
                    gw[t4] = __builtin_amdgcn_raw_buffer_load_b32(brsrc, b_voff, ((e_pix0 + row * e_pitch) * nw32 + (e_nb0 >> 5)) * 4, 0)
                             >> (4 * (lane & 7));
                }
            } else if constexpr (GATED) {
                const auto grsrc = __builtin_amdgcn_make_buffer_rsrc(const_cast<float*>(p.gate), 0, (int)((size_t)p.B * p.DH * p.DW * p.N * 4), 0x00020000);
#pragma unroll
                for (int t4 = 0; t4 < 4; ++t4) {
                    const int row = min(e_row0 + 2 * t4, p.OH - 1);
                    gq[t4] = __builtin_bit_cast(f32x4, __builtin_amdgcn_raw_buffer_load_b128(
                        grsrc, e_voff, ((e_pix0 + row * e_pitch) * p.N + e_nb0) * 4, 0));
                }
            }
            wino_barrier();
            const float* xr = X + (((xh ^ 1) * 2 + nw) * 2 + mw) * 1024 + lane;
            f32x16 y;
#pragma unroll
            for (int r = 0; r < 16; ++r) y[r] = own[r] + xr[r * 64];
            tile_rows4i(scratch, y, lane, [&](int t4, int rr, int cc, f32x4 v4) {
                if (e_single) {
                    const int row = e_row0 + 2 * t4;
                    if (row >= p.OH) return;
                    const int soff = ((e_pix0 + row * e_pitch) * p.N + e_nb0) * 4;
                    f32x4 o = (v4 + bq) * rsq[j][t4];
#pragma unroll
                    for (int e = 0; e < 4; ++e) o[e] = o[e] > 0.f ? o[e] : o[e] * act_neg + 0.f;
                    if constexpr (GBITS) {
#pragma unroll
                        for (int e = 0; e < 4; ++e) o[e] *= (gw[t4] >> e) & 1u ? 1.f : 0.f;
                    } else if constexpr (GATED) {
#pragma unroll
                        for (int e = 0; e < 4; ++e) o[e] *= gq[t4][e] > 0.f ? 1.f : gate_neg;
                    }
                    if (p.accumulate) o += __builtin_bit_cast(f32x4, __builtin_amdgcn_raw_buffer_load_b128(drsrc, e_voff, soff, 0));
                    if constexpr (POOL) {
#pragma unroll
                        for (int e = 0; e < 4; ++e) {
                            const bool gt = j == 1 && o[e] > pmx[t4][e];
                            pmx[t4][e] = (j == 0 || gt) ? o[e] : pmx[t4][e];
                            jbits |= (gt ? 1u : 0u) << (4 * t4 + e);
                        }
                        if (p.pool_only) return;
                    }
                    __builtin_amdgcn_raw_buffer_store_b128(__builtin_bit_cast(u32x4, o), drsrc, e_voff + (uint32_t)soff, 0, 0);
                } else {
                    const int t = 32 * mw + rr;
                    const int oy = ci.oy0 + 2 * (t >> 3) + xh, ox = ci.ox0 + 2 * (t & 7) + j;
                    if (oy >= p.OH || ox >= p.OW) return;
                    const size_t m = ((size_t)ci.b * p.OH + oy) * p.OW + ox;
                    *reinterpret_cast<f32x4*>(p.ws + ((size_t)blockIdx.z * p.M + m) * p.N + ci.n0 + 32 * nw + cc) = v4;
                }
            });
            if constexpr (POOL) {
                if (j == 1 && e_xh == 1) {
                    float* ps = X + ((0 * 2 + nw) * 2 + mw) * 1024 + lane;
#pragma unroll
                    for (int t4 = 0; t4 < 4; ++t4)
#pragma unroll
                        for (int e = 0; e < 4; ++e) {
                            const float v = pmx[t4][e];
                            ps[(t4 * 4 + e) * 64] = (p.pool_code && ((jbits >> (4 * t4 + e)) & 1u)) ? -v : v;
                        }
                }
            }
            wino_barrier();
        }
        if constexpr (POOL) {
            if (e_xh == 0 && e_single) {
                const float* pr = X + ((0 * 2 + nw) * 2 + mw) * 1024 + lane;
                const int PH = p.OH >> 1, PW = p.OW >> 1;
                const auto prsrc = __builtin_amdgcn_make_buffer_rsrc(p.pool_dst, 0, (int)((size_t)p.B * PH * PW * p.N * 4), 0x00020000);
                const uint32_t p_voff = (ci.ox0 >> 1) + (lane >> 3) < PW ? ((uint32_t)(lane >> 3) * p.N + 4 * (lane & 7)) * 4u : 0x80000000u;
                const auto crsrc = __builtin_amdgcn_make_buffer_rsrc(p.pool_code ? p.pool_code : reinterpret_cast<unsigned char*>(p.pool_dst), 0,
                                                                     (int)((size_t)p.B * PH * PW * p.N), 0x00020000);
                const uint32_t c_voff = (ci.ox0 >> 1) + (lane >> 3) < PW ? (uint32_t)(lane >> 3) * p.N + 4 * (lane & 7) : 0x80000000u;
#pragma unroll
                for (int t4 = 0; t4 < 4; ++t4) {
                    const int prow = (ci.oy0 >> 1) + 4 * e_mw + t4;
                    if (prow >= PH) continue;
                    f32x4 m;
                    uint32_t code = 0;
#pragma unroll
                    for (int e = 0; e < 4; ++e) {
                        const float raw = pr[(t4 * 4 + e) * 64];
                        const float r0 = pmx[t4][e], r1 = p.pool_code ? fabsf(raw) : raw;
                        const bool row1 = r1 > r0;
                        m[e] = row1 ? r1 : r0;
                        const uint32_t j0 = (jbits >> (4 * t4 + e)) & 1u, j1 = __float_as_uint(raw) >> 31;
                        code |= ((row1 ? 2u + j1 : j0) | (m[e] > 0.f ? 4u : 0u)) << (8 * e);
                    }
                    const int pix = (ci.b * PH + prow) * PW + (ci.ox0 >> 1);
                    __builtin_amdgcn_raw_buffer_store_b128(__builtin_bit_cast(u32x4, m), prsrc, p_voff + (uint32_t)((pix * p.N + e_nb0) * 4), 0, 0);
                    if (p.pool_code) __builtin_amdgcn_raw_buffer_store_b32(code, crsrc, c_voff + (uint32_t)(pix * p.N + e_nb0), 0, 0);
                }
            }
        }
        wk.publish(wq_pulled, wq_slot);
        const int wq_nxt2 = wk.next(wq_slot);
        if (wq_nxt2 < 0) break;
        ci = ni;
        if constexpr (STEAL) wino_barrier();
        wk.advance(wq_nxt2);
    }
    wk.done(q.qctr);
}

static bool wino_ok(const IGemmParams& p) {
    static const bool off = getenv("TG_NO_WINO") != nullptr;
    if (off || p.wino_u == nullptr || p.bf16) return false;
    if (p.TH != 3 || p.TW != 3 || p.ss != 1 || (p.tstep != 1 && p.tstep != -1) || (p.kstep != 1 && p.kstep != -1)) return false;
    if ((p.C % 8) != 0 || (p.N % WINO_BN) != 0 || p.OH < 16 || p.OW < 16) return false;
    return true;
}
static size_t wino_u_floats(int N, int C) { return (size_t)16 * N * C; }

static int launch_wino(IGemmParams& p, size_t ws_floats_avail, hipStream_t s) {
    WinoGeom q = {};
    q.tiles_x = cdiv(p.OW, 16);
    q.tiles_y = cdiv(p.OH, 16);
    q.nt = p.N / WINO_BN;
    q.total_work = q.tiles_x * q.tiles_y * p.B * q.nt;
    q.interleave = wino_interleave_ok(wino_u_floats(p.N, p.C) * sizeof(float));
    const int sy_b = p.sy0 + 2 * p.tstep, sx_b = p.sx0 + 2 * p.tstep;
    q.sy_min = p.sy0 < sy_b ? p.sy0 : sy_b;
    q.sx_min = p.sx0 < sx_b ? p.sx0 : sx_b;
    WinoWeights ww = {};
    ww.sn = p.w_sn; ww.sk = p.w_sk; ww.stap = p.w_stap;
    ww.k_fast = p.w_sk == 1;
    for (int t = 0; t < 3; ++t) {
        ww.kyu[p.sy0 + t * p.tstep - q.sy_min] = p.ky0 + t * p.kstep;
        ww.kxv[p.sx0 + t * p.tstep - q.sx_min] = p.kx0 + t * p.kstep;
    }
    const int nchunks = p.C / 8;
    int splits = 1;
    if (nchunks >= 16) {
        int smax = nchunks / 8 < 16 ? nchunks / 8 : 16;
        while (smax > 1 && (size_t)smax * p.M * p.N > ws_floats_avail) --smax;
        splits = choose_splits(q.total_work, smax, WINO_PLAN_CUS);
    }
    q.chunks_per_split = cdiv(nchunks, splits);
    p.splits = cdiv(nchunks, q.chunks_per_split);
    p.Ktot = 9 * p.C;

    if (p.wino_ready < 0 && g_wprep_capture) {
        TgWprepItem it = {};
        it.kind = 1; it.N = p.N; it.K = p.C; it.w = p.w_raw; it.out = p.wino_u; it.ww = ww;
        *g_wprep_capture = it;
        g_wprep_captured = 1;
        return TG_OK;
    }
    if (p.wino_ready <= 0) {
        hipLaunchKernelGGL(wino_weights_kernel, dim3(ew_grid((int64_t)p.N * p.C, 256)), dim3(256), 0, s, p.w_raw, p.wino_u, p.N,
                           p.C, ww);
        TG_CHECK_LAUNCH("wino_weights_kernel");
    }
    if (p.wino_ready < 0) return TG_OK;
    const size_t lds = (size_t)WINO_LDS_FLOATS * sizeof(float);
    static const bool no_fast = getenv("TG_WINO_NO_FAST") != nullptr;
    const bool fast = !no_fast && p.amask == nullptr && (size_t)p.B * p.IH * p.IW * p.C * 4 < ((size_t)1 << 31) &&
                      wino_u_floats(p.N, p.C) * 4 < ((size_t)1 << 31);
    const bool gated = p.gate != nullptr && p.splits == 1;
    static const bool no_pipe = getenv("TG_WINO_NO_PIPE") != nullptr;
    const bool pipe = fast && !no_pipe && nchunks - (p.splits - 1) * q.chunks_per_split >= 2 && q.chunks_per_split >= 2 &&
                      (size_t)p.B * p.DH * p.DW * p.N * 4 < ((size_t)1 << 31);
    typedef void (*WinoKern)(const IGemmParams, const WinoGeom, const float*);
    static const WinoKern kerns[16] = {wino_kernel<false, false, false>, wino_kernel<false, true, false>, wino_kernel<true, false, false>,
                                       wino_kernel<true, true, false>, wino_pipe_kernel<false, false>, wino_pipe_kernel<true, false>,
                                       wino_kernel<false, false, true>, wino_kernel<false, true, true>, wino_kernel<true, false, true>,
                                       wino_kernel<true, true, true>, wino_pipe_kernel<false, true>, wino_pipe_kernel<true, true>,
                                       wino_pipe_kernel<false, false, true>, wino_pipe_kernel<false, true, true>,
                                       wino_pipe_kernel<true, false, false, true>, wino_pipe_kernel<true, true, false, true>};
    static LdsOptIn opts[16];
    q.qctr = wino_queue_block(s, p.splits, q.total_work);
    static const bool no_pool = getenv("TG_NO_FUSED_POOL") != nullptr;
    const bool pool = p.pool_dst && !no_pool && pipe && !gated && p.splits == 1 && !(p.OH & 1) && !(p.OW & 1) && p.ds == 1 && p.dy0 == 0 &&
                      p.dx0 == 0 && p.DH == p.OH && p.DW == p.OW && !p.accumulate;
    if (pool) p.pool_done = 1;
    TG_REQUIRE(pool || !(p.pool_code || p.pool_only), "tg_conv_fwd_pool_code: this launch cannot write the pool from its output transform");
    TG_REQUIRE(!p.pool_code || p.act == TG_ACT_RELU, "tg_conv_fwd_pool_code: needs a ReLU output");
    const bool gbits = p.gate_bits != nullptr && pipe && p.splits == 1;
    if (gbits) p.gate_bits_done = 1;
    const int ki = gbits ? (q.qctr ? 15 : 14)
                 : pool ? (q.qctr ? 13 : 12) : (q.qctr ? 6 : 0) + (pipe ? 4 + (gated ? 1 : 0) : (fast ? 2 : 0) + (gated ? 1 : 0));
    if (int rc = lds_opt_in(opts[ki], reinterpret_cast<const void*>(kerns[ki]), lds, "wino")) return rc;
    {
        const double flops = 2.0 * p.M * (double)p.N * p.Ktot * g_alg_scale;
        const double bytes = 4.0 * ((double)p.B * p.IH * p.IW * p.C + (double)p.M + (double)p.N * p.Ktot + (double)p.M * p.N +
                                    (p.amask ? (double)p.B * p.IH * p.IW : 0.0) + (pool ? 0.25 * (double)p.M * p.N : 0.0)) -
                             (p.pool_only ? (4.0 - 0.25) * (double)p.M * p.N : 0.0);
        ProfScope ps(s, 0, flops, bytes, p.M, p.N, p.Ktot, p.C, p.splits, 4064);
        const int grid = q.total_work < wino_cus() ? q.total_work : wino_cus();
        hipLaunchKernelGGL(kerns[ki], dim3(grid, 1, p.splits), dim3(WINO_THREADS), lds, s, p, q, (const float*)p.wino_u);
    }
    TG_CHECK_LAUNCH("wino_kernel");
    if (p.splits > 1) {
        hipLaunchKernelGGL(igemm_splitk_epilogue, dim3(ew_grid((int64_t)p.M * p.N, 256)), dim3(256), 0, s, p);
        TG_CHECK_LAUNCH("igemm_splitk_epilogue");
    }
    return TG_OK;
}

struct WinoWgradGeom {
    int strips_x, tiles_y, nstrips, steps_per_split, splits, ntco, ntci;
};

constexpr int WG_PITCH = 72;
constexpr int WG_XR = 4 * 18 * WG_PITCH;
constexpr int WG_DR = 2 * 16 * WG_PITCH;
constexpr int WINO_WG_LDS_FLOATS = 4 * WINO_V + WG_XR + WG_DR;

__global__ __launch_bounds__(WINO_THREADS) void wino_wgrad_kernel(const WgradParams p, const WinoWgradGeom q, float* __restrict__ slabs) {
    extern __shared__ __attribute__((aligned(16))) float smem[];
    float* As = smem;
    float* Bs = smem + 2 * WINO_V;
    float* Xr = smem + 4 * WINO_V;
    float* Dr = Xr + WG_XR;

    const int tid = threadIdx.x, lane = tid & 63, wave = tid >> 6;
    const int mw = wave & 1, nw = (wave >> 1) & 1, xh = wave >> 2;
    const int work = xcd_remap(blockIdx.x, q.ntco * q.ntci * q.splits);
    const int tco = work % q.ntco, tci = (work / q.ntco) % q.ntci, split = work / (q.ntco * q.ntci);
    const int s_begin = split * q.steps_per_split;
    const int s_end = min(q.nstrips, s_begin + q.steps_per_split);

    const int k = lane & 7, qd = (lane >> 3) + 8 * (wave & 1), a = wave >> 1;
    const int r0 = a == 0 ? 0 : (a == 2 ? 2 : 1), r1 = a == 3 ? 3 : (a == 2 ? 1 : 2);
    const float xs1 = a == 1 ? 1.f : -1.f;
    const float dc0 = a == 3 ? 0.f : 1.f, dc1 = a == 0 ? 0.f : (a == 1 ? 1.f : -1.f);
    int icol[4];
#pragma unroll
    for (int e = 0; e < 4; ++e) icol[e] = (4 * a) * 512 + (qd + 16 * e) * 8 + ((((k >> 2) ^ e) & 1) << 2) + (k & 3);
    const int xrd0 = (r0 * 18 + 2 * k) * WG_PITCH + 4 * qd, xrd1 = (r1 * 18 + 2 * k) * WG_PITCH + 4 * qd;
    const int drd = (2 * k) * WG_PITCH + 4 * qd;

    const auto xrsrc = __builtin_amdgcn_make_buffer_rsrc(const_cast<float*>(p.x), 0, (int)((size_t)p.B * p.H * p.W * p.C * 4), 0x00020000);
    const auto drsrc = __builtin_amdgcn_make_buffer_rsrc(const_cast<float*>(p.dy), 0, (int)((size_t)p.B * p.Ho * p.Wo * p.Cout * 4), 0x00020000);
    const uint32_t OOB = 0xFFFFFFF0u;

    int xs_r[3], xs_px[3], xs_lds[3];
    bool xs_on[3];
    uint32_t xs_ch;
#pragma unroll
    for (int i = 0; i < 3; ++i) {
        const int idx = tid + WINO_THREADS * i;
        const int ps = idx >> 4;
        xs_on[i] = ps < 4 * 18;
        xs_r[i] = ps / 18;
        xs_px[i] = ps - xs_r[i] * 18;
        xs_lds[i] = ps * WG_PITCH + 4 * (idx & 15);
    }
    xs_ch = (uint32_t)(tci * 64 + 4 * (tid & 15)) * 4u;
    const int ds_i = tid >> 8, ds_px = (tid >> 4) & 15, ds_lds = (tid >> 4) * WG_PITCH + 4 * (tid & 15);
    const uint32_t ds_ch = (uint32_t)(tco * 64 + 4 * (tid & 15)) * 4u;

    f32x4 rx[3], rd;
    int ls = s_begin, lsx = s_begin % q.strips_x, lty = (s_begin / q.strips_x) % q.tiles_y, lb = s_begin / (q.strips_x * q.tiles_y);
    auto raw_load = [&]() {
        const bool live = ls < s_end;
#pragma unroll
        for (int i = 0; i < 3; ++i) {
            const int py = 2 * lty - p.pad + xs_r[i], px = 16 * lsx - p.pad + xs_px[i];
            const bool ok = live && xs_on[i] && py >= 0 && py < p.H && px >= 0 && px < p.W;
            const uint32_t off = ok ? (((uint32_t)(lb * p.H + py) * p.W + px) * (uint32_t)p.C) * 4u + xs_ch : OOB;
            rx[i] = __builtin_bit_cast(f32x4, __builtin_amdgcn_raw_buffer_load_b128(xrsrc, off, 0, 0));
        }
        {
            const int oy = 2 * lty + ds_i, ox = 16 * lsx + ds_px;
            const bool ok = live && oy < p.Ho && ox < p.Wo;
            const uint32_t off = ok ? (((uint32_t)(lb * p.Ho + oy) * p.Wo + ox) * (uint32_t)p.Cout) * 4u + ds_ch : OOB;
            rd = __builtin_bit_cast(f32x4, __builtin_amdgcn_raw_buffer_load_b128(drsrc, off, 0, 0));
        }
        ++ls;
        if (++lsx == q.strips_x) { lsx = 0; if (++lty == q.tiles_y) { lty = 0; ++lb; } }
    };
    auto raw_store = [&]() {
#pragma unroll
        for (int i = 0; i < 3; ++i)
            if (xs_on[i]) *reinterpret_cast<f32x4*>(Xr + xs_lds[i]) = rx[i];
        *reinterpret_cast<f32x4*>(Dr + ds_lds) = rd;
    };
    f32x4 xr[2][4], dr[2][2], tt[4], rr[2];
    auto x_read = [&](int j) {
        xr[0][j] = *reinterpret_cast<const f32x4*>(Xr + xrd0 + j * WG_PITCH);
        xr[1][j] = *reinterpret_cast<const f32x4*>(Xr + xrd1 + j * WG_PITCH);
    };
    auto d_read = [&](int i) {
        dr[i][0] = *reinterpret_cast<const f32x4*>(Dr + drd + (i * 16) * WG_PITCH);
        dr[i][1] = *reinterpret_cast<const f32x4*>(Dr + drd + (i * 16 + 1) * WG_PITCH);
    };
    auto x_rows = [&]() {
#pragma unroll
        for (int j = 0; j < 4; ++j) tt[j] = xr[0][j] + xr[1][j] * xs1;
    };
    auto d_rows = [&]() {
#pragma unroll
        for (int j = 0; j < 2; ++j) rr[j] = dr[0][j] * dc0 + dr[1][j] * dc1;
    };
    auto x_out = [&](int buf, int b, int h) {
        const f32x4 v = b == 0 ? tt[0] - tt[2] : b == 1 ? tt[1] + tt[2] : b == 2 ? tt[2] - tt[1] : tt[1] - tt[3];
        float* dst = Bs + buf * WINO_V + b * 512;
        dst[icol[2 * h]] = v[2 * h];
        dst[icol[2 * h + 1]] = v[2 * h + 1];
    };
    auto d_out = [&](int buf, int b, int h) {
        const f32x4 v = b == 0 ? rr[0] : b == 1 ? rr[0] + rr[1] : b == 2 ? rr[0] - rr[1] : -rr[1];
        float* dst = As + buf * WINO_V + b * 512;
        dst[icol[2 * h]] = v[2 * h];
        dst[icol[2 * h + 1]] = v[2 * h + 1];
    };

    const int arow = 32 * mw + (lane & 31), brow = 32 * nw + (lane & 31);
    const int a_off = (8 * xh) * 512 + arow * 8 + ((((lane >> 5) ^ (arow >> 4)) & 1) << 2);
    const int b_off = (8 * xh) * 512 + brow * 8 + ((((lane >> 5) ^ (brow >> 4)) & 1) << 2);

    f32x16 acc[8];
#pragma unroll
    for (int i = 0; i < 8; ++i)
#pragma unroll
        for (int r = 0; r < 16; ++r) acc[i][r] = 0.f;

    if (s_begin < s_end) {
        raw_load();
        raw_store();
        raw_load();
        wino_barrier();
#pragma unroll
        for (int j = 0; j < 4; ++j) x_read(j);
        d_read(0);
        d_read(1);
        x_rows();
        d_rows();
#pragma unroll
        for (int b = 0; b < 4; ++b) { x_out(0, b, 0); x_out(0, b, 1); d_out(0, b, 0); d_out(0, b, 1); }
        wino_barrier();
        f32x4 fa[2], fb[2];
// ... 137 lines not shown
```

terra-gan_amd/tg_hip/engine.py:

```python
import os
from types import SimpleNamespace as NS

import torch

from . import ops as O

G_ENC = [("enc1", 1, 64, 7, 2, 3), ("enc2", 64, 128, 5, 2, 2), ("enc3", 128, 256, 5, 2, 2),
         ("enc4", 256, 512, 3, 2, 1), ("enc5", 512, 512, 3, 2, 1), ("enc6", 512, 512, 3, 2, 1),
         ("enc7", 512, 512, 3, 2, 1)]
G_DEC = [("dec7", 1024, 512, 3, 1, 1), ("dec6", 1024, 512, 3, 1, 1), ("dec5", 1024, 512, 3, 1, 1),
         ("dec4", 768, 256, 3, 1, 1), ("dec3", 384, 128, 3, 1, 1), ("dec2", 192, 64, 3, 1, 1),
         ("dec1", 64, 64, 3, 1, 1)]
D_LAYERS = [(0, None, None, 64, 4, 2, 1, True), (2, 3, 64, 128, 4, 2, 1, True), (5, 6, 128, 256, 4, 2, 1, True),
            (8, 9, 256, 512, 4, 2, 1, True), (11, None, 512, 1, 4, 1, 1, False)]
VGG_TRUNK = [0, 2, "M", 5, 7, "M", 10, 12, 14]


VGG_WINO4 = os.environ.get("TG_VGG_WINO4", "1") != "0"
VGG_WINO4_FWD = os.environ.get("TG_VGG_WINO4_FWD", "0") == "1"
VGG_WINO4_MINCH = int(os.environ.get("TG_VGG_WINO4_MINCH", "128"))
POOL_CODE = os.environ.get("TG_NO_POOL_CODE") is None


def _vgg_wino4(w, B, H, W, cout, mode=None, default=True):
    if mode is False or (mode is None and not default):
        return False
    wide = max(w.shape[0], w.shape[1]) >= VGG_WINO4_MINCH
    if mode is True:
        return wide
    items = B * ((H + 15) // 16) * ((W + 31) // 32) * (cout // 64)
    return wide and items >= 256
_side = {}
SIDE_WGRAD = os.environ.get("TG_SIDE_STREAM") == "1"
PROBE = None


def _side_stream():
    dev = torch.cuda.current_device()
    st = _side.get(dev)
    if st is None:
        st = _side[dev] = torch.cuda.Stream(device=dev)
    return st


def _wgrad(gbuf, inputs, fn):
    if gbuf is None or not SIDE_WGRAD:
        return fn()
    main, side = torch.cuda.current_stream(), _side_stream()
    side.wait_stream(main)
    with torch.cuda.stream(side):
        out = fn()
    for t in inputs:
        if t is not None:
            t.record_stream(side)
    return out


def join_side():
    if SIDE_WGRAD and torch.cuda.current_device() in _side:
        torch.cuda.current_stream().wait_stream(_side_stream())


def _pconv_fwd(P, name, k, s, p, x, in_mask, ratio, training, premasked=False, defer_act=False):
    O.tag(f"{name}.fwd")
    y = O.conv_fwd(x, P[f"{name}.input_conv.weight"], P[f"{name}.input_conv.bias"].detach(), k, s, p,
                   in_mask=None if premasked else in_mask, ratio=ratio)
    if training:
        mean, rstd, a = O.bn_fwd(y, P[f"{name}.bn.weight"], P[f"{name}.bn.bias"], O.ACT_RELU, 0.0, P[f"{name}.bn.running_mean"],
                                 P[f"{name}.bn.running_var"], P[f"{name}.bn.num_batches_tracked"], apply=not defer_act)
    else:
        mean, rstd = O.bn_eval_stats(P[f"{name}.bn.running_mean"], P[f"{name}.bn.running_var"])
        a = None if defer_act else O.bn_act_fwd(y, mean, rstd, P[f"{name}.bn.weight"], P[f"{name}.bn.bias"], O.ACT_RELU)
    if PROBE is not None:
        PROBE("fwd", name, a if a is not None else O.bn_act_fwd(y, mean, rstd, P[f"{name}.bn.weight"], P[f"{name}.bn.bias"], O.ACT_RELU))
    return a, NS(name=name, k=k, s=s, p=p, x=x, in_mask=in_mask, ratio=ratio, y=y, mean=mean, rstd=rstd,
                 premasked=premasked)


def _notify(on_ready, grads, keys):
    if on_ready is not None and not SIDE_WGRAD:
        for k in keys:
            on_ready(k, grads[k])


def _pconv_bwd(P, c, da, grads, dx_out=None, want_dx=True, gbuf=None, on_ready=None, conv1=None):
    name = c.name
    if PROBE is not None:
        PROBE("bwd", name, da)
    outs = (gbuf[f"{name}.bn.weight"], gbuf[f"{name}.bn.bias"], gbuf[f"{name}.input_conv.bias"]) if gbuf is not None else None
    if conv1 is not None:
        dyr, dgamma, dbeta, db = O.bn_act_bwd_conv1(conv1[0], conv1[1], c.y, c.mean, c.rstd, P[f"{name}.bn.weight"], P[f"{name}.bn.bias"],
                                                    O.ACT_RELU, ratio=c.ratio, outs=outs)
    else:
        dyr, dgamma, dbeta, db = O.bn_act_bwd(da, c.y, c.mean, c.rstd, P[f"{name}.bn.weight"], P[f"{name}.bn.bias"], O.ACT_RELU,
                                              ratio=c.ratio, outs=outs)
    O.tag(f"{name}.dgrad")
    dx = O.conv_dgrad(dyr, P[f"{name}.input_conv.weight"], tuple(c.x.shape), c.k, c.s, c.p, in_mask=c.in_mask, out=dx_out) \
        if want_dx else None
    wmask = None if getattr(c, "premasked", False) else c.in_mask
    O.tag(f"{name}.wgrad")
    dw, _ = _wgrad(gbuf, (c.x, dyr, wmask), lambda: O.conv_wgrad(
        c.x, dyr, P[f"{name}.input_conv.weight"], c.k, c.s, c.p, in_mask=wmask, want_bias=False,
        dw_out=gbuf[f"{name}.input_conv.weight"] if gbuf is not None else None))
    grads[f"{name}.input_conv.weight"], grads[f"{name}.input_conv.bias"] = dw, db
    grads[f"{name}.bn.weight"], grads[f"{name}.bn.bias"] = dgamma, dbeta
    _notify(on_ready, grads, (f"{name}.bn.bias", f"{name}.bn.weight", f"{name}.input_conv.bias", f"{name}.input_conv.weight"))
    return dx


def generator_forward(P, x, mask, training=True, checkpoint=False, out=None):
    B, H, W = x.shape
    m, er, dmasks, dr = O.mask_pyramid(mask, [(k, s, p) for (_n, _ci, _co, k, s, p) in G_ENC],
                                       [(k, s, p) for (_n, _ci, _co, k, s, p) in G_DEC])

    enc_ctx, e = [], [x.reshape(B, H, W, 1)]
    for i, (name, _ci, _co, k, s, p) in enumerate(G_ENC):
        a, c = _pconv_fwd(P, name, k, s, p, e[-1], m[i], er[i + 1], training)
        e.append(a)
        enc_ctx.append(c)
    d, dec_ctx = e[7], []
    fshape = (B, H, W, G_DEC[6][2])
    bnin_final = BNIN_FINAL and O.conv_bnin_supported(fshape, 1, 3, 1, 1) and O.conv_bnin_supported(fshape, 1, 3, 1, 1, wgrad=True)
    up_c = None
    for i, (name, _ci, _co, k, s, p) in enumerate(G_DEC):
        skip = e[6 - i] if i < 6 else None
        Hs, Ws = (skip.shape[1], skip.shape[2]) if skip is not None else (H, W)
        if up_c is not None:
            up_shape = tuple(up_c.y.shape)
            cat = O.upcat_fwd(up_c.y, skip, Hs, Ws, out_mask=dmasks[i], up_bn=_bn_in(P, up_c))
        else:
            up_shape = tuple(d.shape)
            cat = O.upcat_fwd(d, skip, Hs, Ws, out_mask=dmasks[i])
        if i == 6:
            defer = bnin_final
        else:
            nskip = e[5 - i] if i < 5 else None
            nH, nW = (nskip.shape[1], nskip.shape[2]) if nskip is not None else (H, W)
            defer = BNIN_UPCAT and Hs * Ws * B > O.BN_SMALL_ROWS and \
                O.upcat_bn_supported((B, Hs, Ws, _co), None if nskip is None else tuple(nskip.shape), nH, nW)
        d, c = _pconv_fwd(P, name, k, s, p, cat, dmasks[i], dr[i], training, premasked=True, defer_act=defer)
        up_c = c if (defer and i < 6) else None
        c.up_shape, c.x_shape, c.skip_hw = up_shape, tuple(cat.shape), (Hs, Ws)
        if checkpoint:
            c.x = None
        dec_ctx.append(c)
    O.tag("final.fwd")
    if bnin_final:
        logits = O.conv_fwd_bnin(dec_ctx[6].y, _bn_in(P, dec_ctx[6]), P["final.weight"], P["final.bias"].detach(), 3, 1, 1)
    else:
        logits = O.conv_fwd(d, P["final.weight"], P["final.bias"].detach(), 3, 1, 1)
    out = O.sigmoid_composite_fwd(logits.reshape(B, H, W), x, mask, out=out)
    if PROBE is not None:
        PROBE("fwd", "final", logits)
        PROBE("fwd", "gen", out)
    if checkpoint:
        for i in range(1, 7):
            enc_ctx[i].x_shape = tuple(enc_ctx[i].x.shape)
            enc_ctx[i].x = None
        d = None
    return out, NS(enc=enc_ctx, dec=dec_ctx, d0=d, logits=logits, mask=mask, shape=(B, H, W), checkpoint=checkpoint,
                   bnin_final=bnin_final)


def _act_of(P, c):
    return O.bn_act_fwd(c.y, c.mean, c.rstd, P[f"{c.name}.bn.weight"], P[f"{c.name}.bn.bias"], O.ACT_RELU)


def _bn_in(P, c):
    return (c.mean, c.rstd, P[f"{c.name}.bn.weight"], P[f"{c.name}.bn.bias"], O.ACT_RELU, 0.0)


BNIN_FINAL = os.environ.get("TG_NO_BNIN") is None
BN_CONV1 = os.environ.get("TG_NO_BN_CONV1") is None
# ... 45 lines not shown
            dskips[6 - i] = dskip
    dx = None
    for i in range(6, -1, -1):
        c = ctx.enc[i]
        if ckpt and i > 0:
            c.x = _act_of(P, ctx.enc[i - 1])
        if i > 0:
            da = _pconv_bwd(P, c, da, grads, dx_out=dskips[i], gbuf=gbuf, on_ready=on_ready)
            if ckpt:
                c.x = None
        else:
            dx = _pconv_bwd(P, c, da, grads, want_dx=want_dx, gbuf=gbuf, on_ready=on_ready)
    if want_dx:
        dx = O.axpby_(dx_comp, 1.0, 1.0, dx.reshape(B, H, W))
    join_side()
    return grads, dx


def discriminator_forward(P, img, training=True, groups=1, update_running=True):
    h = img if img.dim() == 4 else img.reshape(*img.shape, 1)
    Bg = h.shape[0] // groups
    assert Bg * groups == h.shape[0]
    layers = []
    for (ci, bi, _cin, _cout, k, s, p, leaky) in D_LAYERS:
        w, b = P[f"model.{ci}.weight"], P[f"model.{ci}.bias"].detach()
        O.tag(f"d{ci}.fwd")
        if bi is None:
            act = O.ACT_LEAKY if leaky else O.ACT_NONE
            a = O.conv_fwd(h, w, b, k, s, p, act=act, slope=0.2)
            layers.append(NS(ci=ci, bi=None, k=k, s=s, p=p, x=h, a=a, act=act))
        else:
            y = O.conv_fwd(h, w, b, k, s, p)
            if groups > 1 and training and y.shape[-1] % 4 == 0:
                mean2, rstd2, a = O.bn_fwd_grouped(y, groups, P[f"model.{bi}.weight"], P[f"model.{bi}.bias"], O.ACT_LEAKY, 0.2)
                if update_running:
                    O.bn_running_update_multi(mean2, rstd2, y.numel() // y.shape[-1] // groups, list(range(groups)),
                                              P[f"model.{bi}.running_mean"], P[f"model.{bi}.running_var"],
                                              P[f"model.{bi}.num_batches_tracked"])
                means, rstds = [mean2[gi] for gi in range(groups)], [rstd2[gi] for gi in range(groups)]
                layers.append(NS(ci=ci, bi=bi, k=k, s=s, p=p, x=h, y=y, mean=means[0], rstd=rstds[0], means=means, rstds=rstds,
                                 mean2=mean2, rstd2=rstd2, a=a))
                h = a
                continue
            a = torch.empty_like(y)
            means, rstds = [], []
            for gi in range(groups):
                yg, ag = y[gi * Bg:(gi + 1) * Bg], a[gi * Bg:(gi + 1) * Bg]
                if training:
                    run = (P[f"model.{bi}.running_mean"], P[f"model.{bi}.running_var"], P[f"model.{bi}.num_batches_tracked"]) \
                        if update_running else (None, None, None)
                    mean, rstd = O.bn_stats(yg, *run)
                else:
                    mean, rstd = O.bn_eval_stats(P[f"model.{bi}.running_mean"], P[f"model.{bi}.running_var"])
                O.bn_act_fwd(yg, mean, rstd, P[f"model.{bi}.weight"], P[f"model.{bi}.bias"], O.ACT_LEAKY, 0.2, out=ag)
                means.append(mean), rstds.append(rstd)
            layers.append(NS(ci=ci, bi=bi, k=k, s=s, p=p, x=h, y=y, mean=means[0], rstd=rstds[0], means=means, rstds=rstds, a=a))
        h = a
    return h, NS(layers=layers, groups=groups)


def discriminator_group(ctx, gi):
    G = ctx.groups
    out = []
    for c in ctx.layers:
        Bg = c.x.shape[0] // G
        sl = slice(gi * Bg, (gi + 1) * Bg)
        d = dict(vars(c))
        d["x"], d["a"] = c.x[sl], c.a[sl]
        if c.bi is not None:
            d["y"], d["mean"], d["rstd"] = c.y[sl], c.means[gi], c.rstds[gi]
            d["means"], d["rstds"] = [c.means[gi]], [c.rstds[gi]]
        out.append(NS(**d))
    return NS(layers=out, groups=1)


def discriminator_backward(P, ctx, dlogits, want_wgrad=True, want_dimg=False, gbuf=None, on_ready=None):
    grads, da, gated = {}, dlogits, False
    for li in range(len(ctx.layers) - 1, -1, -1):
        c = ctx.layers[li]
        w = P[f"model.{c.ci}.weight"]
        db = None
        if c.bi is None:
            dy = da if (gated or c.act == O.ACT_NONE) else O.act_bwd(da, c.a, c.act, 0.2)
        else:
            outs = (gbuf[f"model.{c.bi}.weight"], gbuf[f"model.{c.bi}.bias"], gbuf[f"model.{c.ci}.bias"]) \
                if (gbuf is not None and want_wgrad) else None
            G_ = getattr(ctx, "groups", 1)
            if G_ > 1 and hasattr(c, "mean2"):
                dy, dgamma, dbeta, db = O.bn_act_bwd_grouped(da, c.y, G_, c.mean2, c.rstd2, P[f"model.{c.bi}.weight"],
                                                             P[f"model.{c.bi}.bias"], O.ACT_LEAKY, 0.2, want_dbias=want_wgrad, outs=outs)
            elif G_ == 1:
                dy, dgamma, dbeta, db = O.bn_act_bwd(da, c.y, c.mean, c.rstd, P[f"model.{c.bi}.weight"], P[f"model.{c.bi}.bias"],
                                                     O.ACT_LEAKY, 0.2, want_dbias=want_wgrad, outs=outs)
            else:
                Bg = da.shape[0] // G_
                dy = da
                for gi in range(G_):
                    sl = slice(gi * Bg, (gi + 1) * Bg)
                    _d, g1, b1, db1 = O.bn_act_bwd(da[sl], c.y[sl], c.means[gi], c.rstds[gi], P[f"model.{c.bi}.weight"],
                                                   P[f"model.{c.bi}.bias"], O.ACT_LEAKY, 0.2, want_dbias=want_wgrad,
                                                   outs=outs if gi == 0 else None)
                    if gi == 0:
                        dgamma, dbeta, db = g1, b1, db1
                    elif want_wgrad:
                        O.axpby_(g1, 1.0, 1.0, dgamma), O.axpby_(b1, 1.0, 1.0, dbeta), O.axpby_(db1, 1.0, 1.0, db)
            if want_wgrad:
                grads[f"model.{c.bi}.weight"], grads[f"model.{c.bi}.bias"] = dgamma, dbeta
        gated = False
        O.tag(f"d{c.ci}.dgrad")
        if li > 0 or want_dimg:
            below = ctx.layers[li - 1] if li > 0 else None
            if below is not None and below.bi is None and below.act != O.ACT_NONE:
                da = O.conv_dgrad(dy, w, tuple(c.x.shape), c.k, c.s, c.p, gate=below.a, gate_act=below.act, gate_slope=0.2)
                gated = True
            else:
                da = O.conv_dgrad(dy, w, tuple(c.x.shape), c.k, c.s, c.p)
        else:
            da = None
        O.tag(f"d{c.ci}.wgrad")
        if want_wgrad:
            dw, db2 = _wgrad(gbuf, (c.x, dy), lambda c=c, dy=dy, w=w, db=db: O.conv_wgrad(
                c.x, dy, w, c.k, c.s, c.p, want_bias=db is None,
                dw_out=gbuf[f"model.{c.ci}.weight"] if gbuf is not None else None,
                db_out=gbuf[f"model.{c.ci}.bias"] if (gbuf is not None and db is None) else None))
            grads[f"model.{c.ci}.weight"], grads[f"model.{c.ci}.bias"] = dw, (db if db is not None else db2)
            if c.bi is not None:
                _notify(on_ready, grads, (f"model.{c.bi}.bias", f"model.{c.bi}.weight"))
            _notify(on_ready, grads, (f"model.{c.ci}.bias", f"model.{c.ci}.weight"))
    join_side()
    return grads, da


def discriminator_replay_running_stats(P, ctx, order=(0,)):
    G_ = getattr(ctx, "groups", 1)
    for c in ctx.layers:
        if c.bi is not None:
            rows = c.y.numel() // c.y.shape[-1] // G_
            if hasattr(c, "mean2"):
                O.bn_running_update_multi(c.mean2, c.rstd2, rows, list(order), P[f"model.{c.bi}.running_mean"],
                                          P[f"model.{c.bi}.running_var"], P[f"model.{c.bi}.num_batches_tracked"])
                continue
            for gi in order:
                mean, rstd = (c.means[gi], c.rstds[gi]) if hasattr(c, "means") else (c.mean, c.rstd)
                O.bn_running_update(mean, rstd, rows, P[f"model.{c.bi}.running_mean"], P[f"model.{c.bi}.running_var"],
                                    P[f"model.{c.bi}.num_batches_tracked"])


def vgg_forward(V, img, keep=True, wino4=None, nb=None):
    gates = keep == "gates"
    assert keep in (True, False) or gates, keep
    h = img.reshape(*img.shape, 1)
    steps = []
    pooled = code = None
    for i, item in enumerate(VGG_TRUNK):
        if item == "M":
            o = pooled if pooled is not None else O.maxpool2_fwd(h)
            if keep:
                steps.append(NS(kind="M", x=h if (code is None or not gates) else None, code=code))
            pooled = code = None
        else:
            w = V["0.folded"] if item == 0 else V[f"{item}.weight"]
            O.tag(f"vgg{item}.fwd")
            pool = i + 1 < len(VGG_TRUNK) and VGG_TRUNK[i + 1] == "M" and h.shape[1] % 2 == 0 and h.shape[2] % 2 == 0
            w4 = _vgg_wino4(w, h.shape[0], h.shape[1], h.shape[2], w.shape[0], wino4, VGG_WINO4_FWD)
            if pool and POOL_CODE and not w4 and O.conv_pool_code_supported(tuple(h.shape), w.shape[0]):
                pooled, code = O.conv_fwd_pool_code(h, w, V[f"{item}.bias"])
                o = None
            else:
                o = O.conv_fwd(h, w, V[f"{item}.bias"], 3, 1, 1, act=O.ACT_RELU, pool=pool, wino4=w4)
                if pool:
                    o, pooled = o
            if gates:
                feeds = i + 1 < len(VGG_TRUNK) and VGG_TRUNK[i + 1] != "M"
                steps.append(NS(kind="C", w=w, x_shape=tuple(h.shape), a=None, bits=O.relu_gate_pack(o, nb) if feeds else None))
            elif keep:
                steps.append(NS(kind="C", w=w, x_shape=tuple(h.shape), a=o))
        h = o
    return h, NS(steps=steps)


def vgg_backward(ctx, dfeat, nb=None, wino4=None, gated=False):
    da = dfeat
    steps = ctx.steps
    w4 = wino4
    for i in range(len(steps) - 1, -1, -1):
        st = steps[i]
        if st.kind == "M":
            if getattr(st, "code", None) is not None:
                da = O.maxpool2_bwd_code(da, st.code)
            else:
                x = st.x if nb is None else st.x[:nb]
                da = O.maxpool2_bwd(da, x, relu_gate=True)
            gated = True
        else:
            a = None if st.a is None else (st.a if nb is None else st.a[:nb])
            if not gated and a is None:
                raise ValueError("vgg_backward: this context keeps no activation of the trunk's output: pass gated=True")
            dy = da if gated else O.act_bwd(da, a, O.ACT_RELU)
            shp = st.x_shape if nb is None else (nb,) + tuple(st.x_shape[1:])
            below = steps[i - 1] if i > 0 else None
            O.tag(f"vgg{VGG_TRUNK[i]}.dgrad")
            if below is not None and below.kind == "C" and getattr(below, "bits", None) is not None:
                assert below.bits.shape[0] == shp[0], "vgg_backward: the gate bits were packed for another number of images"
                da = O.conv_dgrad(dy, st.w, shp, 3, 1, 1, gate_bits=below.bits,
                                  wino4=_vgg_wino4(st.w, shp[0], shp[1], shp[2], shp[3], w4, VGG_WINO4))
                gated = True
            elif below is not None and below.kind == "C":
                ga = below.a if nb is None else below.a[:nb]
                da = O.conv_dgrad(dy, st.w, shp, 3, 1, 1, gate=ga, gate_act=O.ACT_RELU,
                                  wino4=_vgg_wino4(st.w, shp[0], shp[1], shp[2], shp[3], w4, VGG_WINO4))
                gated = True
            else:
                da = O.conv_dgrad(dy, st.w, shp, 3, 1, 1, wino4=_vgg_wino4(st.w, shp[0], shp[1], shp[2], shp[3], w4, VGG_WINO4))
                gated = False
    return da.reshape(da.shape[0], da.shape[1], da.shape[2])
```

terra-gan_amd/tg_hip/lib.py:

```python
import ctypes as C
import os

import torch

_HERE = os.path.dirname(os.path.abspath(__file__))
LIB_PATH = os.environ.get("TG_HIP_LIB") or os.path.join(os.path.dirname(_HERE), "lib", "libterragan_hip.so")


class TgConv(C.Structure):
    _fields_ = [(n, C.c_int32) for n in ("B", "H", "W", "Cin", "Ho", "Wo", "Cout", "k", "stride", "pad", "precision")]


TG_MASK_PYRAMID_MAX = 24


class TgMaskOp(C.Structure):
    _fields_ = [(n, C.c_int32) for n in ("kind", "H", "W", "Ho", "Wo", "k", "stride", "pad")] + \
               [(n, C.c_void_p) for n in ("in_", "in2", "out", "out2")]


class TgMaskPyramid(C.Structure):
    _fields_ = [("nops", C.c_int32), ("_pad", C.c_int32), ("op", TgMaskOp * TG_MASK_PYRAMID_MAX)]


class TgBnAct(C.Structure):
    _fields_ = [(n, C.c_void_p) for n in ("mean", "rstd", "gamma", "beta")] + [("act", C.c_int32), ("slope", C.c_float)]


class TgRasterPlan(C.Structure):
    _fields_ = [(n, C.c_int32) for n in ("H", "W", "wh", "ww", "overlap", "ny", "nx")]


class TgError(RuntimeError):
    pass


P, I, I64, F, SZ, D = C.c_void_p, C.c_int, C.c_int64, C.c_float, C.c_size_t, C.c_double
CP = C.POINTER(TgConv)
RP = C.POINTER(TgRasterPlan)

SIGNATURES = {
    "tg_version": (I, []),
    "tg_last_error": (C.c_char_p, []),
    "tg_conv_fwd_ws_bytes": (SZ, [CP]),
    "tg_conv_fwd": (I, [CP, P, P, P, P, P, I, F, P, P, SZ, P]),
    "tg_conv_dgrad_ws_bytes": (SZ, [CP]),
    "tg_conv_dgrad": (I, [CP, P, P, P, P, I, P, SZ, P]),
    "tg_conv_dgrad_gated": (I, [CP, P, P, P, P, I, F, P, P, SZ, P]),
    "tg_set_cu_reserve": (I, [I]),
    "tg_set_work_stealing": (I, [I]),
    "tg_conv_wprep_bytes": (SZ, [CP, I]),
    "tg_conv_wprep": (I, [CP, I, P, P, P]),
    "tg_conv_wprep_item_bytes": (SZ, []),
    "tg_conv_wprep_item": (I, [CP, I, P, P, P]),
    "tg_conv_wprep_run": (I, [P, I, P]),
    "tg_conv_fwd_p": (I, [CP, P, P, P, P, P, P, I, F, P, P, SZ, P]),
    "tg_conv_fwd_pool": (I, [CP, P, P, P, P, P, P, I, F, P, P, P, SZ, P]),
    "tg_conv_pool_code_supported": (I, [CP]),
    "tg_conv_fwd_pool_code": (I, [CP, P, P, P, P, P, P, P, SZ, P]),
    "tg_maxpool2_bwd_code": (I, [P, P, I, I, I, I, P, P]),
    "tg_conv_bnin_supported": (I, [CP, I]),
    "tg_conv_fwd_bnin": (I, [CP, P, C.POINTER(TgBnAct), P, P, I, F, P, P, SZ, P]),
    "tg_conv_wgrad_bnin": (I, [CP, P, C.POINTER(TgBnAct), P, P, P, P, SZ, P]),
    "tg_conv_dgrad_p": (I, [CP, P, P, P, P, P, I, F, P, I, P, SZ, P]),
    "tg_relu_gate_pack": (I, [P, I64, I, P, P]),
    "tg_conv_dgrad_gbits": (I, [CP, P, P, P, P, P, P, I, P, SZ, P]),
    "tg_conv_wgrad_ws_bytes": (SZ, [CP]),
    "tg_conv_wgrad": (I, [CP, P, P, P, P, P, P, SZ, P]),
    "tg_fold_cin": (I, [P, I, I, I, P, P]),
    "tg_mask_update": (I, [P, I, I, I, I, I, I, I, I, P, P, P]),
    "tg_mask_up_merge": (I, [P, P, I, I, I, I, I, P, P]),
    "tg_mask_pyramid": (I, [C.POINTER(TgMaskPyramid), I, P]),
    "tg_bn_ws_bytes": (SZ, [I64, I]),
    "tg_bn_stats": (I, [P, I64, I, F, F, P, P, P, P, P, P, SZ, P]),
    "tg_bn_eval_stats": (I, [P, P, I, F, P, P, P]),
    "tg_bn_act_fwd": (I, [P, I64, I, P, P, P, P, I, F, P, P]),
    "tg_bn_fwd": (I, [P, I64, I, F, F, P, P, I, F, P, P, P, P, P, P, P, SZ, P]),
    "tg_bn_act_bwd": (I, [P, P, I64, I, P, P, P, P, I, F, P, P, P, P, P, P, SZ, P]),
    "tg_bn_bwd_conv1_supported": (I, [I64, I]),
    "tg_bn_conv1_ws_bytes": (SZ, [I64, I]),
    "tg_bn_act_bwd_conv1": (I, [P, P, I, I, I, P, I, P, P, P, P, I, F, P, P, P, P, P, P, SZ, P]),
    "tg_act_bwd": (I, [P, P, I64, I, I, F, P, P, P]),
    "tg_upcat_fwd": (I, [P, P, P, I, I, I, I, I, I, I, P, P]),
    "tg_upcat_bn_supported": (I, [I, I, I, I, I, I, I]),
    "tg_upcat_fwd_bn": (I, [P, C.POINTER(TgBnAct), P, P, I, I, I, I, I, I, I, P, P]),
    "tg_upcat_bwd": (I, [P, I, I, I, I, I, I, I, P, P, P]),
    "tg_sigmoid_composite_fwd": (I, [P, P, P, I64, P, P]),
    "tg_sigmoid_composite_bwd": (I, [P, P, P, I64, P, P, P]),
    "tg_maxpool2_fwd": (I, [P, I, I, I, I, P, P]),
    "tg_maxpool2_bwd": (I, [P, P, I, I, I, I, I, P, P]),
    "tg_pixel_loss_ws_bytes": (SZ, [I, I, I]),
    "tg_pixel_losses": (I, [P, P, P, P, I, I, I, F, F, F, F, P, P, P, I, P, SZ, P]),
    "tg_reduce_ws_bytes": (SZ, [I64]),
    "tg_l1_mean": (I, [P, P, I64, F, P, P, P, P, SZ, P]),
    "tg_l1_mean_relu": (I, [P, P, I64, F, P, P, P, P, SZ, P]),
    "tg_bce_logits": (I, [P, I64, F, F, P, P, P, P, SZ, P]),
    "tg_adam": (I, [P, P, P, P, I64, D, D, D, D, I, F, P]),
    "tg_adam_multi": (I, [P, P, I, I, D, D, D, D, I, F, P]),
    "tg_adam_scalars": (I, [D, D, D, I, P]),
    "tg_write_floats": (I, [P, I, P, P]),
    "tg_adam_multi_s": (I, [P, P, I, I, D, D, D, P, F, P]),
    "tg_axpby": (I, [P, F, F, P, I64, P]),
    "tg_lincomb": (I, [P, F, P, F, P, I64, P]),
    "tg_mul": (I, [P, P, P, I64, P]),
    "tg_mul_keep": (I, [P, P, P, P, I64, P]),
    "tg_bn_running_update": (I, [P, P, I64, I, F, F, P, P, P, P]),
    "tg_bn_grouped_ws_bytes": (SZ, [I64, I, I]),
    "tg_bn_fwd_grouped": (I, [P, I64, I, I, F, P, P, I, F, P, P, P, P, SZ, P]),
    "tg_bn_act_bwd_grouped": (I, [P, P, I64, I, I, P, P, P, P, I, F, P, P, P, P, P, SZ, P]),
    "tg_bn_running_update_multi": (I, [P, P, I64, I, F, F, C.POINTER(C.c_int), I, P, P, P, P]),
    "tg_quality_metrics_ws_bytes": (SZ, [I64, I, I]),
    "tg_quality_metrics": (I, [P, P, P, I64, I, I, P, P, SZ, P]),
    "tg_u8_to_tiles": (I, [P, P, I64, P, P, P]),
    "tg_raster_window_stats": (I, [P, P, RP, I, F, P, P, P, P]),
    "tg_raster_gather": (I, [P, P, RP, I, F, P, P, P, I, P, P, P]),
    "tg_raster_blend": (I, [P, P, RP, I, F, P, P, P, P, I, P, P, P]),
    "tg_hole_masks": (I, [P, P, I, I, P, P]),
    "tg_raster_sample": (I, [P, I64, I64, P, I, I, P, I, P, P, P, P]),
    "tg_prof_enable": (I, [I]),
    "tg_prof_summary": (I, [I, C.POINTER(C.c_double), C.POINTER(C.c_int64), C.POINTER(C.c_double), C.POINTER(C.c_double)]),
    "tg_prof_dump": (I, [C.c_char_p]),
    "tg_prof_tag": (I, [C.c_char_p]),
    "tg_nchw_to_nhwc": (I, [P, I, I, I, I, P, P]),
    "tg_nhwc_to_nchw": (I, [P, I, I, I, I, P, P]),
}

_lib = None


def load():
    global _lib
    if _lib is None:
        if not os.path.exists(LIB_PATH):
            raise TgError(f"{LIB_PATH} is missing: build it with `python terra-gan_amd/build.py` "
                          "(or __graft_entry__.build()); this framework has no CPU / eager fallback")
        lib = C.CDLL(LIB_PATH)
        for name, (res, args) in SIGNATURES.items():
            fn = getattr(lib, name)
            fn.restype, fn.argtypes = res, args
        _lib = lib
    return _lib


def check(rc, what=""):
    if rc != 0:
        raise TgError(f"{what} failed (rc={rc}): {load().tg_last_error().decode()}")
```

terra-gan_amd/tg_hip/ops.py:

```python
import ctypes as C

import torch

from . import lib as L

ACT_NONE, ACT_RELU, ACT_LEAKY = 0, 1, 2
PREC_F32, PREC_BF16, PREC_F32_WINO4 = 0, 1, 2
_precision = PREC_F32


def set_precision(name):
    global _precision
    _precision = {"f32": PREC_F32, "fp32": PREC_F32, "bf16": PREC_BF16}[name]


def get_precision():
    return "bf16" if _precision == PREC_BF16 else "f32"
BN_EPS, BN_MOMENTUM = 1e-5, 0.1
PROF_TAGS = False


def tag(name):
    if PROF_TAGS:
        _lib().tg_prof_tag(name.encode())
# ... 4 lines not shown
def _lib():
    return L.load()


def _stream():
    return C.c_void_p(torch.cuda.current_stream().cuda_stream)


def _p(t):
    return None if t is None else C.c_void_p(t.data_ptr())


def _chk(t, name="tensor"):
    if t is None:
        return
    if not t.is_cuda:
        raise L.TgError(f"{name}: expected a HIP (cuda) tensor -- there is no CPU path")
    if t.dtype != torch.float32:
        raise L.TgError(f"{name}: expected float32, got {t.dtype}")
    if not t.is_contiguous():
        raise L.TgError(f"{name}: expected a contiguous tensor, strides {t.stride()}")


def workspace(nbytes):
    dev = torch.cuda.current_device()
    key = (dev, torch.cuda.current_stream().cuda_stream)
    buf = _ws.get(key)
    if buf is None or buf.numel() * 4 < nbytes:
        n = max(int(nbytes) // 4 + 64, 1 << 20)
        buf = torch.empty(n, dtype=torch.float32, device=f"cuda:{dev}")
        _ws[key] = buf
    return buf


def empty(*shape, like=None, device=None):
    return torch.empty(*shape, dtype=torch.float32, device=like.device if like is not None else device)


def weight_view(w):
    v = w.detach().permute(0, 2, 3, 1)
    if not v.is_contiguous():
        w.data = w.data.contiguous(memory_format=torch.channels_last)
        v = w.detach().permute(0, 2, 3, 1)
        if not v.is_contiguous():
            dense = v.contiguous()
            w.data = dense.permute(0, 3, 1, 2)
            v = w.detach().permute(0, 2, 3, 1)
    return v


def _prec(wino4):
    return PREC_F32_WINO4 if (wino4 and _precision == PREC_F32) else _precision


def conv_geom(x, cout, k, stride, pad, wino4=False):
    B, H, W, Cin = x.shape
    Ho, Wo = (H + 2 * pad - k) // stride + 1, (W + 2 * pad - k) // stride + 1
    return L.TgConv(B, H, W, Cin, Ho, Wo, cout, k, stride, pad, _prec(wino4))


WPREP_FWD, WPREP_DGRAD = 0, 1
WPREP_CACHE = True
WPREP_VERIFY = __import__("os").environ.get("TG_WPREP_VERIFY") == "1"
WPREP_BATCH = True
_wprep = {}
_wstamp = {}
_wprep_tables = {}
wprep_capture_log = None


def weights_updated(params):
    ptrs = set()
    for p in params:
        if p.dim() == 4:
            ptr = p.data_ptr()
            _wstamp[ptr] = _wstamp.get(ptr, 0) + 1
            ptrs.add(ptr)
    if WPREP_BATCH and WPREP_CACHE and ptrs:
        _prepare_batch(ptrs)


def _prepare_batch(ptrs):
    ents = []
    for key, e in _wprep.items():
        if key[0] in ptrs and e[3] and e[4] and e[0]() is not None:
            ents.append((key, e))
    if not ents:
        return
    raw = b"".join(e[3] for _, e in ents)
    tkey = (ents[0][1][2].device, raw)
    table = _wprep_tables.get(tkey)
    if table is None:
        import numpy as np
        table = torch.from_numpy(np.frombuffer(raw, dtype=np.uint8).copy()).to(ents[0][1][2].device)
        if len(_wprep_tables) > 16:
            _wprep_tables.clear()
        _wprep_tables[tkey] = table
    L.check(_lib().tg_conv_wprep_run(C.c_void_p(table.data_ptr()), len(ents), _stream()), "tg_conv_wprep_run")
    for key, e in ents:
        e[1] = (e[0]()._version, _wstamp.get(key[0], 0))
        e[4] = False
    if wprep_capture_log is not None:
        wprep_capture_log.extend(key for key, _e in ents)


def graph_replayed(weight_ptrs, refreshed_keys):
    for ptr in weight_ptrs:
        _wstamp[ptr] = _wstamp.get(ptr, 0) + 1
    for key in refreshed_keys:
        e = _wprep.get(key)
        if e is not None:
            w = e[0]()
            if w is not None:
                e[1] = (w._version, _wstamp.get(key[0], 0))


def _prepared(w, wv, g, mode):
    if not WPREP_CACHE:
        return None
    import weakref
    ptr = wv.data_ptr()
    key = (ptr, mode, g.H, g.W, g.Cin, g.Cout, g.k, g.stride, g.pad, g.precision)
    stamp = (w._version, _wstamp.get(ptr, 0))
    ent = _wprep.get(key)
    if ent is not None and ent[0]() is w and ent[1] == stamp:
        ent[4] = True
        if WPREP_VERIFY and ent[2] is not None:
            fresh = torch.empty_like(ent[2])
            L.check(_lib().tg_conv_wprep(C.byref(g), mode, _p(wv), _p(fresh), _stream()), "tg_conv_wprep")
            if not torch.equal(fresh.view(torch.int32), ent[2].view(torch.int32)):
                raise L.TgError("prepared weights are stale: a parameter was rewritten without tg_hip.ops.weights_updated()")
        return ent[2]
    lib = _lib()
    if ent is None or ent[0]() is not w:
        nb = lib.tg_conv_wprep_bytes(C.byref(g), mode)
        buf = torch.empty((nb + 3) // 4, dtype=torch.float32, device=wv.device) if nb else None
        if len(_wprep) > 512:
            for k_ in [k_ for k_, e in _wprep.items() if e[0]() is None]:
                del _wprep[k_]
        item = False
        if buf is not None:
            raw = C.create_string_buffer(lib.tg_conv_wprep_item_bytes())
            if lib.tg_conv_wprep_item(C.byref(g), mode, _p(wv), _p(buf), raw):
                item = raw.raw
        ent = [weakref.ref(w), None, buf, item, True]
        _wprep[key] = ent
    if ent[2] is not None:
        L.check(lib.tg_conv_wprep(C.byref(g), mode, _p(wv), _p(ent[2]), _stream()), "tg_conv_wprep")
    ent[1] = stamp
    ent[4] = True
    return ent[2]


def conv_fwd(x, w, bias, k, stride, pad, in_mask=None, ratio=None, act=ACT_NONE, slope=0.0, wino4=False, pool=False):
    _chk(x, "x"); _chk(bias, "bias"); _chk(in_mask, "in_mask"); _chk(ratio, "ratio")
    wv = weight_view(w)
    _chk(wv, "weight")
    g = conv_geom(x, wv.shape[0], k, stride, pad, wino4)
    assert wv.shape == (g.Cout, k, k, g.Cin), (tuple(wv.shape), g.Cout, k, g.Cin)
    y = empty(g.B, g.Ho, g.Wo, g.Cout, like=x)
    lib = _lib()
    nb = lib.tg_conv_fwd_ws_bytes(C.byref(g))
    ws = workspace(nb)
    if pool:
        yp = empty(g.B, g.Ho // 2, g.Wo // 2, g.Cout, like=x)
        L.check(lib.tg_conv_fwd_pool(C.byref(g), _p(x), _p(in_mask), _p(wv), _p(_prepared(w, wv, g, WPREP_FWD)), _p(bias), _p(ratio),
                                     act, slope, _p(y), _p(yp), _p(ws), ws.numel() * 4, _stream()), "tg_conv_fwd_pool")
        return y, yp
    L.check(lib.tg_conv_fwd_p(C.byref(g), _p(x), _p(in_mask), _p(wv), _p(_prepared(w, wv, g, WPREP_FWD)), _p(bias), _p(ratio),
                              act, slope, _p(y), _p(ws), ws.numel() * 4, _stream()), "tg_conv_fwd")
    return y


def _bn_act(in_bn):
    mean, rstd, gamma, beta = in_bn[:4]
    for t in (mean, rstd, gamma, beta):
        _chk(t, "in_bn")
    act = in_bn[4] if len(in_bn) > 4 else ACT_RELU
    slope = in_bn[5] if len(in_bn) > 5 else 0.0
    return L.TgBnAct(mean.data_ptr(), rstd.data_ptr(), gamma.detach().data_ptr(), beta.detach().data_ptr(), act, slope)


def conv_bnin_supported(x_shape, cout, k, stride, pad, wgrad=False):
    B, H, W, Cin = x_shape
    Ho, Wo = (H + 2 * pad - k) // stride + 1, (W + 2 * pad - k) // stride + 1
    g = L.TgConv(B, H, W, Cin, Ho, Wo, cout, k, stride, pad, _precision)
    return bool(_lib().tg_conv_bnin_supported(C.byref(g), 1 if wgrad else 0))


def conv_fwd_bnin(x, in_bn, w, bias, k, stride, pad, act=ACT_NONE, slope=0.0):
    _chk(x, "x"); _chk(bias, "bias")
    wv = weight_view(w)
    _chk(wv, "weight")
    g = conv_geom(x, wv.shape[0], k, stride, pad)
    y = empty(g.B, g.Ho, g.Wo, g.Cout, like=x)
    lib = _lib()
    ws = workspace(lib.tg_conv_fwd_ws_bytes(C.byref(g)))
    bn = _bn_act(in_bn)
    L.check(lib.tg_conv_fwd_bnin(C.byref(g), _p(x), C.byref(bn), _p(wv), _p(bias), act, slope, _p(y), _p(ws), ws.numel() * 4, _stream()),
            "tg_conv_fwd_bnin")
    return y


def conv_pool_code_supported(x_shape, cout):
    B, H, W, Cin = x_shape
    g = L.TgConv(B, H, W, Cin, H, W, cout, 3, 1, 1, _precision)
    return bool(_lib().tg_conv_pool_code_supported(C.byref(g)))


def conv_fwd_pool_code(x, w, bias):
    _chk(x, "x"); _chk(bias, "bias")
    wv = weight_view(w)
    _chk(wv, "weight")
    g = conv_geom(x, wv.shape[0], 3, 1, 1)
    yp = empty(g.B, g.Ho // 2, g.Wo // 2, g.Cout, like=x)
    code = torch.empty((g.B, g.Ho // 2, g.Wo // 2, g.Cout), dtype=torch.uint8, device=x.device)
    lib = _lib()
    ws = workspace(lib.tg_conv_fwd_ws_bytes(C.byref(g)))
    L.check(lib.tg_conv_fwd_pool_code(C.byref(g), _p(x), _p(wv), _p(_prepared(w, wv, g, WPREP_FWD)), _p(bias), _p(yp),
                                      C.c_void_p(code.data_ptr()), _p(ws), ws.numel() * 4, _stream()), "tg_conv_fwd_pool_code")
    return yp, code


def maxpool2_bwd_code(dout, code):
    _chk(dout, "dout")
    B, Ho, Wo, Cc = dout.shape
    assert code.dtype == torch.uint8 and code.is_contiguous() and tuple(code.shape[1:]) == (Ho, Wo, Cc) and code.shape[0] >= B
    dx = empty(B, 2 * Ho, 2 * Wo, Cc, like=dout)
    L.check(_lib().tg_maxpool2_bwd_code(_p(dout), C.c_void_p(code.data_ptr()), B, Ho, Wo, Cc, _p(dx), _stream()), "tg_maxpool2_bwd_code")
    return dx


def relu_gate_pack(a, nb=None):
    _chk(a, "a")
    B, H, W, Cc = a.shape
    nb = B if nb is None else nb
    assert 0 < nb <= B, (nb, B)
    bits = torch.empty((nb, H, W, Cc // 32), dtype=torch.uint32, device=a.device)
    L.check(_lib().tg_relu_gate_pack(_p(a), nb * H * W, Cc, C.c_void_p(bits.data_ptr()), _stream()), "tg_relu_gate_pack")
    return bits


def conv_dgrad(dy, w, x_shape, k, stride, pad, in_mask=None, out=None, gate=None, gate_act=ACT_RELU, gate_slope=0.0, wino4=False,
               gate_bits=None):
    _chk(dy, "dy"); _chk(in_mask, "in_mask"); _chk(out, "out"); _chk(gate, "gate")
    wv = weight_view(w)
    B, H, W, Cin = x_shape
    g = L.TgConv(B, H, W, Cin, dy.shape[1], dy.shape[2], dy.shape[3], k, stride, pad, _prec(wino4))
    acc = 1 if out is not None else 0
    dx = out if out is not None else empty(B, H, W, Cin, like=dy)
    lib = _lib()
    ws = workspace(lib.tg_conv_dgrad_ws_bytes(C.byref(g)))
    if gate_bits is not None:
        assert gate is None and out is None, "conv_dgrad: gate_bits is exclusive with gate and does not accumulate"
        assert gate_bits.dtype == torch.uint32 and gate_bits.is_contiguous() and tuple(gate_bits.shape) == (B, H, W, Cin // 32), \
            (gate_bits.dtype, tuple(gate_bits.shape), tuple(x_shape))
        L.check(lib.tg_conv_dgrad_gbits(C.byref(g), _p(dy), _p(wv), _p(_prepared(w, wv, g, WPREP_DGRAD)), _p(in_mask),
                                        C.c_void_p(gate_bits.data_ptr()), _p(dx), 0, _p(ws), ws.numel() * 4, _stream()),
                "tg_conv_dgrad_gbits")
        return dx
    if gate is not None:
        assert out is None and tuple(gate.shape) == tuple(x_shape)
    L.check(lib.tg_conv_dgrad_p(C.byref(g), _p(dy), _p(wv), _p(_prepared(w, wv, g, WPREP_DGRAD)), _p(in_mask), _p(gate),
                                gate_act if gate is not None else ACT_NONE, gate_slope, _p(dx), acc, _p(ws), ws.numel() * 4,
                                _stream()), "tg_conv_dgrad")
    return dx


def conv_wgrad(x, dy, w, k, stride, pad, in_mask=None, want_bias=True, dw_out=None, db_out=None, in_bn=None):
    _chk(x, "x"); _chk(dy, "dy"); _chk(in_mask, "in_mask")
    wv = weight_view(w)
    B, H, W, Cin = x.shape
    g = L.TgConv(B, H, W, Cin, dy.shape[1], dy.shape[2], dy.shape[3], k, stride, pad, _precision)
    if dw_out is not None:
        dwv = dw_out.permute(0, 2, 3, 1)
        assert dwv.is_contiguous() and dwv.shape == wv.shape
    else:
        dwv = torch.empty_like(wv)
    db = (db_out if db_out is not None else empty(g.Cout, like=x)) if want_bias else None
    lib = _lib()
    ws = workspace(lib.tg_conv_wgrad_ws_bytes(C.byref(g)))
    if in_bn is not None:
        assert in_mask is None
        bn = _bn_act(in_bn)
        L.check(lib.tg_conv_wgrad_bnin(C.byref(g), _p(x), C.byref(bn), _p(dy), _p(dwv), _p(db), _p(ws), ws.numel() * 4, _stream()),
                "tg_conv_wgrad_bnin")
        return dwv.permute(0, 3, 1, 2), db
    L.check(lib.tg_conv_wgrad(C.byref(g), _p(x), _p(in_mask), _p(dy), _p(dwv), _p(db), _p(ws), ws.numel() * 4, _stream()),
            "tg_conv_wgrad")
    return dwv.permute(0, 3, 1, 2), db


def fold_cin(w):
    wv = weight_view(w)
    co, kh, kw, ci = wv.shape
    out = empty(co, kh, kw, 1, like=wv)
    L.check(_lib().tg_fold_cin(_p(wv), co, kh * kw, ci, _p(out), _stream()), "tg_fold_cin")
    return out.permute(0, 3, 1, 2)


def mask_update(mask, k, stride, pad):
    _chk(mask, "mask")
    B, H, W = mask.shape
    Ho, Wo = (H + 2 * pad - k) // stride + 1, (W + 2 * pad - k) // stride + 1
    mo, ratio = empty(B, Ho, Wo, like=mask), empty(B, Ho, Wo, like=mask)
    L.check(_lib().tg_mask_update(_p(mask), B, H, W, k, stride, pad, Ho, Wo, _p(mo), _p(ratio), _stream()), "tg_mask_update")
    return mo, ratio


def mask_up_merge(up_mask, skip_mask):
    _chk(up_mask, "up_mask"); _chk(skip_mask, "skip_mask")
    B, h, w = up_mask.shape
    _, H, W = skip_mask.shape
    out = torch.empty_like(skip_mask)
    L.check(_lib().tg_mask_up_merge(_p(up_mask), _p(skip_mask), B, h, w, H, W, _p(out), _stream()), "tg_mask_up_merge")
    return out


MASK_FUSE_PIXELS = 64 * 64


def mask_pyramid(mask, enc, dec):
    _chk(mask, "mask")
    B, H, W = mask.shape
    ne, nd = len(enc), len(dec)
    dims = [(H, W)]
    for (k, s, p) in enc:
        h, w = dims[-1]
        dims.append(((h + 2 * p - k) // s + 1, (w + 2 * p - k) // s + 1))
    sizes = [B * h * w for (h, w) in dims[1:]] * 2
    ddims = []
    cur = dims[ne]
    for j, (k, s, p) in enumerate(dec):
        sk = dims[ne - 1 - j]
        ddims.append((cur, sk))
        cur = ((sk[0] + 2 * p - k) // s + 1, (sk[1] + 2 * p - k) // s + 1)
        sizes += [B * sk[0] * sk[1], B * cur[0] * cur[1], B * cur[0] * cur[1]]
    offs, tot = [], 0
    for n in sizes:
        offs.append(tot)
        tot += (n + 63) // 64 * 64
    buf = torch.empty(tot, dtype=torch.float32, device=mask.device)
    it = iter(zip(offs, sizes))

    def view(shape):
        o, n = next(it)
        return buf[o:o + n].view(shape)

    m, er = [mask], [None]
    mo_views = [view((B,) + dims[i + 1]) for i in range(ne)]
    r_views = [view((B,) + dims[i + 1]) for i in range(ne)]
    pm = L.TgMaskPyramid()
    n_ops = 0
    lib = _lib()

    def flush():
        nonlocal n_ops, pm
        if n_ops:
            pm.nops = n_ops
            L.check(lib.tg_mask_pyramid(C.byref(pm), B, _stream()), "tg_mask_pyramid")
            pm, n_ops = L.TgMaskPyramid(), 0

    def put(kind, hin, hout, k, s, p, a, a2, o, o2):
        nonlocal n_ops
        if hout[0] * hout[1] > MASK_FUSE_PIXELS:
            flush()
            if kind == 0:
                L.check(lib.tg_mask_update(_p(a), B, hin[0], hin[1], k, s, p, hout[0], hout[1], _p(o), _p(o2), _stream()), "tg_mask_update")
            else:
                L.check(lib.tg_mask_up_merge(_p(a), _p(a2), B, hin[0], hin[1], hout[0], hout[1], _p(o), _stream()), "tg_mask_up_merge")
            return
# ... 535 lines not shown
```

Measured before the change: 1013.

## Skip VGG forward tiles where predicted and target images are identical

Adds a kernel that compares the predicted and target halves of the VGG perceptual-loss batch bitwise. It propagates the difference mask through the conv (3x3 dilation) and pool plan to build, for each conv layer, a list of 16x16 tiles whose receptive field can differ. The Winograd pipe kernel gets a SPARSE variant that computes only the listed tiles, presumably copying the shared result for the other half. The aim is to avoid recomputing identical activations in regions the generator leaves unchanged (inpainting outside the mask), at the cost of an extra map kernel with cross-block ticket sync, and correctness depends on the kernel handling skipped tiles properly.

```diff
diff --git a/include/terragan_hip.h b/include/terragan_hip.h
--- a/include/terragan_hip.h
+++ b/include/terragan_hip.h
@@ -54,6 +54,18 @@
                           float* pool_y, unsigned char* code, float* ws, size_t ws_bytes, tg_stream_t stream);
 int tg_maxpool2_bwd_code(const float* dout, const unsigned char* code, int B, int Ho, int Wo, int C, float* dx,
                          tg_stream_t stream);
+typedef struct TgSparseMap {
+    const uint32_t* bits;
+    const int32_t* list;
+    const int32_t* count;
+    int32_t nb, tiles_y, tiles_x, _pad;
+} TgSparseMap;
+size_t tg_vgg_sparse_map_bytes(int nb, int H, int W, const char* plan);
+int tg_vgg_sparse_map(const float* x, int nb, int H, int W, const char* plan, void* buf, size_t buf_bytes, int* ticket,
+                      TgSparseMap* maps, tg_stream_t stream);
+int tg_conv_fwd_sparse(const TgConv* g, const float* x, const float* w, const float* wprep, const float* bias, int act,
+                       float slope, float* y, float* pool_y, unsigned char* code, const TgSparseMap* sp, float* ws,
+                       size_t ws_bytes, tg_stream_t stream);
 typedef struct TgBnAct {
     const float *mean, *rstd, *gamma, *beta;
     int32_t act;
diff --git a/terra-gan_amd/csrc/igemm.hip b/terra-gan_amd/csrc/igemm.hip
--- a/terra-gan_amd/csrc/igemm.hip
+++ b/terra-gan_amd/csrc/igemm.hip
@@ -1274,6 +1274,7 @@
     float* pool_dst = nullptr;
     unsigned char* pool_code = nullptr;
     const BnIn* in_bn = nullptr;
+    const TgSparseMap* sparse = nullptr;
     int pool_fused = 0;
 };
 static int conv_fwd_impl(const TgConv* g, const float* x, const float* in_mask, const float* w, float* wprep, int prep,
@@ -1286,6 +1287,7 @@
         if (!s2d_ok(g) && !wino22_fwd_geom_ok(g)) {
             FwdExtras e;
             e.pool_dst = pool_y;
+            e.sparse = ex ? ex->sparse : nullptr;
             const int rc1 = conv_fwd_impl(g, x, in_mask, w, wprep, prep, bias, ratio, act, slope, y, ws, ws_bytes, stream, nullptr, &e);
             if (rc1) return rc1;
             fused = e.pool_fused;
@@ -1379,6 +1381,7 @@
         p.pool_dst = ex->pool_dst;
         p.pool_code = ex->pool_code;
         p.pool_only = ex->pool_code != nullptr;
+        p.sparse = ex->sparse;
         if (ex->in_bn) {
             p.in_bn = *ex->in_bn;
             TG_REQUIRE(smallconv_bnin_fwd_ok(p), "tg_conv_fwd_bnin: geometry not supported (ask tg_conv_bnin_supported first)");
@@ -1406,18 +1409,35 @@
     const long work = (long)cdiv(g->Wo, 16) * cdiv(g->Ho, 16) * g->B * (g->Cout / WINO_BN);
     return nchunks < 16 || work >= 4L * WINO_PLAN_CUS ? 1 : 0;
 }
-extern "C" int tg_conv_fwd_pool_code(const TgConv* g, const float* x, const float* w, const float* wprep, const float* bias,
-                                     float* pool_y, unsigned char* code, float* ws, size_t ws_bytes, tg_stream_t stream) {
+static int conv_fwd_pool_code(const TgConv* g, const float* x, const float* w, const float* wprep, const float* bias, float* pool_y,
+                              unsigned char* code, const TgSparseMap* sp, float* ws, size_t ws_bytes, tg_stream_t stream) {
     TG_REQUIRE(pool_y && code && aligned16(pool_y) && (reinterpret_cast<uintptr_t>(code) & 3) == 0, "tg_conv_fwd_pool_code: bad pointers");
     TG_REQUIRE(tg_conv_pool_code_supported(g), "tg_conv_fwd_pool_code: geometry not supported (ask tg_conv_pool_code_supported first)");
     FwdExtras e;
     e.pool_dst = pool_y;
     e.pool_code = code;
+    e.sparse = sp;
     const int rc = conv_fwd_impl(g, x, nullptr, w, const_cast<float*>(wprep), wprep ? 1 : 0, bias, nullptr, TG_ACT_RELU, 0.f, pool_y, ws,
                                  ws_bytes, stream, nullptr, &e);
     if (rc) return rc;
     TG_REQUIRE(e.pool_fused, "tg_conv_fwd_pool_code: internal: the launch did not take the fused path");
     return TG_OK;
+}
+extern "C" int tg_conv_fwd_pool_code(const TgConv* g, const float* x, const float* w, const float* wprep, const float* bias,
+                                     float* pool_y, unsigned char* code, float* ws, size_t ws_bytes, tg_stream_t stream) {
+    return conv_fwd_pool_code(g, x, w, wprep, bias, pool_y, code, nullptr, ws, ws_bytes, stream);
+}
+extern "C" int tg_conv_fwd_sparse(const TgConv* g, const float* x, const float* w, const float* wprep, const float* bias, int act,
+                                  float slope, float* y, float* pool_y, unsigned char* code, const TgSparseMap* sp, float* ws,
+                                  size_t ws_bytes, tg_stream_t stream) {
+    if (code) {
+        TG_REQUIRE(act == TG_ACT_RELU, "tg_conv_fwd_sparse: the pool code needs a ReLU output");
+        return conv_fwd_pool_code(g, x, w, wprep, bias, pool_y, code, sp, ws, ws_bytes, stream);
+    }
+    FwdExtras e;
+    e.sparse = sp;
+    return conv_fwd_impl(g, x, nullptr, w, const_cast<float*>(wprep), wprep ? 1 : 0, bias, nullptr, act, slope, y, ws, ws_bytes, stream,
+                         pool_y, &e);
 }
 static bool bnin_geom_ok(const TgConv* g) {
     return g && g->Cout == 1 && g->Cin == 64 && g->k == 3 && g->stride == 1 && g->pad == 1 && (g->Wo % 4) == 0;
diff --git a/terra-gan_amd/csrc/igemm_params.h b/terra-gan_amd/csrc/igemm_params.h
--- a/terra-gan_amd/csrc/igemm_params.h
+++ b/terra-gan_amd/csrc/igemm_params.h
@@ -41,6 +41,7 @@
     BnIn in_bn;
     const uint32_t* gate_bits;
     int gate_bits_done;
+    const TgSparseMap* sparse;
 };
 __device__ __forceinline__ float gate_factor(const IGemmParams& p, size_t idx) {
     const float gv = p.gate[idx];
diff --git a/terra-gan_amd/csrc/pointwise.hip b/terra-gan_amd/csrc/pointwise.hip
--- a/terra-gan_amd/csrc/pointwise.hip
+++ b/terra-gan_amd/csrc/pointwise.hip
@@ -334,6 +334,239 @@
     }
     hipLaunchKernelGGL(mask_pyramid_kernel, dim3(B), dim3(1024), 0, S(stream), *pm);
     TG_CHECK_LAUNCH("mask_pyramid_kernel");
+    return TG_OK;
+}
+
+constexpr int VSM_MAX_OPS = 24, VSM_MAX_CONV = 16, VSM_LDS_WORDS = 4096;
+struct VggMapArgs {
+    const uint32_t* x;
+    int nb, H, W, nops, nconv;
+    char ops[VSM_MAX_OPS];
+    int tiles_y[VSM_MAX_CONV], tiles_x[VSM_MAX_CONV];
+    int32_t* count[VSM_MAX_CONV];
+    uint32_t* bits[VSM_MAX_CONV];
+    int32_t* list[VSM_MAX_CONV];
+    unsigned char* flags[VSM_MAX_CONV];
+    uint64_t* d0;
+    int rows_per_slice;
+    int* ticket;
+};
+__device__ __forceinline__ uint32_t vsm_even_bits(uint64_t v) {
+    v &= 0x5555555555555555ull;
+    v = (v | (v >> 1)) & 0x3333333333333333ull;
+    v = (v | (v >> 2)) & 0x0f0f0f0f0f0f0f0full;
+    v = (v | (v >> 4)) & 0x00ff00ff00ff00ffull;
+    v = (v | (v >> 8)) & 0x0000ffff0000ffffull;
+    v = (v | (v >> 16)) & 0x00000000ffffffffull;
+    return (uint32_t)v;
+}
+__device__ __forceinline__ uint64_t vsm_row_mask(int W, int w, int WW) {
+    return (w == WW - 1 && (W & 63)) ? (1ull << (W & 63)) - 1 : ~0ull;
+}
+__device__ __forceinline__ bool vsm_last_arrival(int* ctr, int n, int* s_last) {
+    __builtin_amdgcn_s_waitcnt(0);
+    __syncthreads();
+    if (threadIdx.x == 0) {
+        __threadfence();
+        const bool last = atomicAdd(ctr, 1) == n - 1;
+        if (last) __threadfence();
+        *s_last = last;
+    }
+    __syncthreads();
+    return *s_last;
+}
+__global__ __launch_bounds__(1024) void vgg_sparse_map_kernel(const VggMapArgs a) {
+    extern __shared__ uint64_t vsm[];
+    __shared__ int scan[1024];
+    __shared__ int s_last;
+    const int tid = threadIdx.x, lane = tid & 63, wave = tid >> 6, b = blockIdx.y;
+    int H = a.H, W = a.W, WW = (W + 63) >> 6;
+    uint64_t* cur = vsm;
+    uint64_t* nxt = vsm + H * WW;
+    uint64_t* d0 = a.d0 + (size_t)b * H * WW;
+    {
+        const uint32_t* xp = a.x + (size_t)b * H * W;
+        const uint32_t* tp = a.x + ((size_t)a.nb + b) * H * W;
+        const int ubeg = blockIdx.x * a.rows_per_slice * WW, uend = min(H, (blockIdx.x + 1) * a.rows_per_slice) * WW;
+        for (int u0 = ubeg + wave; u0 < uend; u0 += 16 * 8) {
+            uint32_t pv[8], tv[8];
+#pragma unroll
+            for (int k = 0; k < 8; ++k) {
+                const int u = u0 + 16 * k, y = u / WW, px = (u - y * WW) * 64 + lane;
+                pv[k] = tv[k] = 0;
+                if (u < uend && px < W) { pv[k] = xp[(size_t)y * W + px]; tv[k] = tp[(size_t)y * W + px]; }
+            }
+#pragma unroll
+            for (int k = 0; k < 8; ++k) {
+                const uint64_t m = __ballot(pv[k] != tv[k]);
+                if (lane == 0 && u0 + 16 * k < uend) d0[u0 + 16 * k] = m;
+            }
+        }
+    }
+    if (!vsm_last_arrival(a.ticket + b, (int)gridDim.x, &s_last)) return;
+    for (int u = tid; u < H * WW; u += 1024) cur[u] = d0[u];
+    if (tid == 0) __hip_atomic_store(a.ticket + b, 0, __ATOMIC_RELAXED, __HIP_MEMORY_SCOPE_AGENT);
+    __syncthreads();
+    int ci = 0;
+    for (int o = 0; o < a.nops; ++o) {
+        if (a.ops[o] == 'C') {
+            for (int u = tid; u < H * WW; u += 1024) {
+                const int y = u / WW, w = u - y * WW;
+                uint64_t r = 0;
+                for (int dy = -1; dy <= 1; ++dy) {
+                    const int yy = y + dy;
+                    if (yy < 0 || yy >= H) continue;
+                    const uint64_t* row = cur + yy * WW;
+                    const uint64_t v = row[w];
+                    r |= v | (v << 1) | (v >> 1);
+                    if (w > 0) r |= row[w - 1] >> 63;
+                    if (w + 1 < WW) r |= row[w + 1] << 63;
+                }
+                nxt[u] = r & vsm_row_mask(W, w, WW);
+            }
+            __syncthreads();
+            uint64_t* t = cur; cur = nxt; nxt = t;
+            const int ty_n = a.tiles_y[ci], tx_n = a.tiles_x[ci], tiles = ty_n * tx_n;
+            for (int t2 = tid; t2 < tiles; t2 += 1024) {
+                const int ty = t2 / tx_n, tx = t2 - ty * tx_n;
+                const int w = (16 * tx) >> 6, sh = (16 * tx) & 63;
+                uint64_t any = 0;
+                for (int y = 16 * ty; y < min(16 * ty + 16, H); ++y) any |= (cur[y * WW + w] >> sh) & 0xffffull;
+                a.flags[ci][(size_t)b * tiles + t2] = any ? 1 : 0;
+            }
+            ++ci;
+        } else {
+            const int H2 = H >> 1, W2 = W >> 1, WW2 = (W2 + 63) >> 6;
+            for (int u = tid; u < H2 * WW2; u += 1024) {
+                const int y = u / WW2, w = u - y * WW2;
+                const uint64_t* r0 = cur + (2 * y) * WW;
+                const uint64_t* r1 = r0 + WW;
+                const uint64_t s0 = r0[2 * w] | r1[2 * w];
+                const uint64_t s1 = 2 * w + 1 < WW ? r0[2 * w + 1] | r1[2 * w + 1] : 0;
+                const uint64_t v = (uint64_t)vsm_even_bits(s0 | (s0 >> 1)) | ((uint64_t)vsm_even_bits(s1 | (s1 >> 1)) << 32);
+                nxt[u] = v & vsm_row_mask(W2, w, WW2);
+            }
+            H = H2; W = W2; WW = WW2;
+            __syncthreads();
+            uint64_t* t = cur; cur = nxt; nxt = t;
+        }
+        __syncthreads();
+    }
+    if (!vsm_last_arrival(a.ticket + a.nb, a.nb, &s_last)) return;
+    for (int c = 0; c < a.nconv; ++c) {
+        const int n = a.nb * a.tiles_y[c] * a.tiles_x[c], nw = (n + 31) >> 5;
+        int carry = 0;
+        for (int w0 = 0; w0 < nw; w0 += 1024) {
+            const int w = w0 + tid;
+            uint32_t word = 0;
+            if (w < nw) {
+                const uint4* fp = reinterpret_cast<const uint4*>(a.flags[c] + 32 * (size_t)w);
+                const uint4 f0 = fp[0], f1 = fp[1];
+                const uint32_t fw[8] = {f0.x, f0.y, f0.z, f0.w, f1.x, f1.y, f1.z, f1.w};
+#pragma unroll
+                for (int i = 0; i < 8; ++i)
+#pragma unroll
+                    for (int j = 0; j < 4; ++j) word |= ((fw[i] >> (8 * j)) & 1u) << (4 * i + j);
+                if (32 * w + 32 > n) word &= (1u << (n - 32 * w)) - 1u;
+                a.bits[c][w] = word;
+            }
+            const int pc = __popc(word);
+            scan[tid] = pc;
+            __syncthreads();
+            for (int d = 1; d < 1024; d <<= 1) {
+                const int v = tid >= d ? scan[tid - d] : 0;
+                __syncthreads();
+                scan[tid] += v;
+                __syncthreads();
+            }
+            int pos = carry + scan[tid] - pc;
+            for (uint32_t m = word; m; m &= m - 1) a.list[c][pos++] = 32 * w + __ffs(m) - 1;
+            carry += scan[1023];
+            __syncthreads();
+        }
+        if (tid == 0) *a.count[c] = carry;
+    }
+    if (tid == 0) __hip_atomic_store(a.ticket + a.nb, 0, __ATOMIC_RELAXED, __HIP_MEMORY_SCOPE_AGENT);
+}
+
+struct VsmLayout {
+    int nconv, nops, H, W;
+    size_t d0;
+    int tiles_y[VSM_MAX_CONV], tiles_x[VSM_MAX_CONV];
+    size_t count[VSM_MAX_CONV], bits[VSM_MAX_CONV], list[VSM_MAX_CONV], flags[VSM_MAX_CONV];
+    size_t bytes;
+};
+static bool vsm_layout(int nb, int H, int W, const char* plan, VsmLayout& L) {
+    if (nb <= 0 || H <= 0 || W <= 0 || !plan) return false;
+    if ((size_t)H * ((W + 63) / 64) > VSM_LDS_WORDS) return false;
+    L = VsmLayout{};
+    L.H = H; L.W = W;
+    L.d0 = 0;
+    size_t off = align_up((size_t)nb * H * ((W + 63) / 64) * sizeof(uint64_t), 16);
+    int h = H, w = W;
+    for (const char* c = plan; *c; ++c) {
+        if (L.nops == VSM_MAX_OPS) return false;
+        ++L.nops;
+        if (*c == 'M') {
+            h >>= 1; w >>= 1;
+            if (h <= 0 || w <= 0) return false;
+        } else if (*c == 'C') {
+            if (L.nconv == VSM_MAX_CONV) return false;
+            const int i = L.nconv++;
+            L.tiles_y[i] = cdiv(h, 16); L.tiles_x[i] = cdiv(w, 16);
+            const size_t n = (size_t)nb * L.tiles_y[i] * L.tiles_x[i];
+            if (n > ((size_t)1 << 30)) return false;
+            L.count[i] = off; off += 16;
+            L.bits[i] = off; off += align_up((n + 31) / 32, 4) * 4;
+            L.list[i] = off; off += align_up(n, 4) * 4;
+            L.flags[i] = off; off += align_up(n, 32);
+        } else {
+            return false;
+        }
+    }
+    L.bytes = off;
+    return L.nconv > 0;
+}
+extern "C" size_t tg_vgg_sparse_map_bytes(int nb, int H, int W, const char* plan) {
+    VsmLayout L;
+    return vsm_layout(nb, H, W, plan, L) ? L.bytes : 0;
+}
+extern "C" int tg_vgg_sparse_map(const float* x, int nb, int H, int W, const char* plan, void* buf, size_t buf_bytes, int* ticket,
+                                 TgSparseMap* maps, tg_stream_t stream) {
+    VsmLayout L;
+    TG_REQUIRE(x && buf && ticket && maps, "tg_vgg_sparse_map: null pointer");
+    TG_REQUIRE(vsm_layout(nb, H, W, plan, L), "tg_vgg_sparse_map: geometry not supported (tg_vgg_sparse_map_bytes is 0)");
+    TG_REQUIRE(buf_bytes >= L.bytes && (reinterpret_cast<uintptr_t>(buf) & 15) == 0, "tg_vgg_sparse_map: buffer too small or unaligned");
+    VggMapArgs a = {};
+    a.x = reinterpret_cast<const uint32_t*>(x);
+    a.nb = nb; a.H = H; a.W = W; a.nops = L.nops; a.nconv = L.nconv; a.ticket = ticket;
+    for (int i = 0; i < L.nops; ++i) a.ops[i] = plan[i];
+    char* base = static_cast<char*>(buf);
+    a.d0 = reinterpret_cast<uint64_t*>(base + L.d0);
+    const int slices = cdiv(H, 8) < cdiv(256, nb) ? cdiv(H, 8) : cdiv(256, nb);
+    a.rows_per_slice = cdiv(H, slices);
+    for (int i = 0; i < L.nconv; ++i) {
+        a.tiles_y[i] = L.tiles_y[i]; a.tiles_x[i] = L.tiles_x[i];
+        a.count[i] = reinterpret_cast<int32_t*>(base + L.count[i]);
+        a.bits[i] = reinterpret_cast<uint32_t*>(base + L.bits[i]);
+        a.list[i] = reinterpret_cast<int32_t*>(base + L.list[i]);
+        a.flags[i] = reinterpret_cast<unsigned char*>(base + L.flags[i]);
+        maps[i] = TgSparseMap{a.bits[i], a.list[i], a.count[i], nb, L.tiles_y[i], L.tiles_x[i], 0};
+    }
+    const size_t lds = 2 * (size_t)H * ((W + 63) / 64) * sizeof(uint64_t);
+    static bool opted[64] = {};
+    int dev = 0;
+    (void)hipGetDevice(&dev);
+    if (dev < 0 || dev >= 64 || !opted[dev]) {
+        if (hipFuncSetAttribute(reinterpret_cast<const void*>(vgg_sparse_map_kernel), hipFuncAttributeMaxDynamicSharedMemorySize,
+                                (int)(2 * VSM_LDS_WORDS * sizeof(uint64_t))) != hipSuccess) {
+            tg_set_error("tg_vgg_sparse_map: LDS opt-in failed");
+            return TG_ERR_LAUNCH;
+        }
+        if (dev >= 0 && dev < 64) opted[dev] = true;
+    }
+    hipLaunchKernelGGL(vgg_sparse_map_kernel, dim3(cdiv(H, a.rows_per_slice), nb), dim3(1024), lds, S(stream), a);
+    TG_CHECK_LAUNCH("vgg_sparse_map_kernel");
     return TG_OK;
 }
 
diff --git a/terra-gan_amd/csrc/wino.inc b/terra-gan_amd/csrc/wino.inc
--- a/terra-gan_amd/csrc/wino.inc
+++ b/terra-gan_amd/csrc/wino.inc
@@ -6,6 +6,10 @@
     int sy_min, sx_min;
     int interleave;
     int* qctr;
+    const uint32_t* sp_bits;
+    const int* sp_list;
+    const int* sp_count;
+    int sp_tiles, sp_nb;
 };
 struct WinoWeights {
     long sn, sk, stap;
@@ -476,7 +480,7 @@
     wk.done(q.qctr);
 }
 
-template <bool GATED, bool STEAL, bool POOL = false, bool GBITS = false>
+template <bool GATED, bool STEAL, bool POOL = false, bool GBITS = false, bool SPARSE = false>
 __global__ __launch_bounds__(WINO_THREADS) void wino_pipe_kernel(const IGemmParams p, const WinoGeom q, const float* __restrict__ U) {
     extern __shared__ __attribute__((aligned(16))) float smem[];
     float* Vs = smem;
@@ -487,13 +491,27 @@
     const int mw = wave & 1, nw = (wave >> 1) & 1, xh = wave >> 2;
     __shared__ int wq_slot[2];
     WinoWork<STEAL> wk;
-    wk.init(q.total_work, q.interleave, q.qctr, wq_slot);
-
-    struct Item { int nt, n0, oy0, ox0, b; uint32_t poff[2]; };
+    int total = q.total_work;
+    if constexpr (SPARSE) {
+        const int cnt = __builtin_amdgcn_readfirstlane(*q.sp_count);
+        total = (q.sp_tiles + min(max(cnt, 0), q.sp_tiles)) * q.nt;
+    }
+    wk.init(total, q.interleave, q.qctr, wq_slot);
+
+    struct Item { int nt, n0, oy0, ox0, b, mirror; uint32_t poff[2]; };
     auto decode_item = [&](int it) {
         Item r;
         r.nt = it % q.nt;
         int tile = it / q.nt;
+        r.mirror = 0;
+        if constexpr (SPARSE) {
+            if (tile < q.sp_tiles) {
+                r.mirror = (__builtin_amdgcn_readfirstlane(q.sp_bits[tile >> 5]) >> (tile & 31)) & 1 ? 0 : 1;
+                tile += q.sp_tiles;
+            } else {
+                tile = __builtin_amdgcn_readfirstlane(q.sp_list[tile - q.sp_tiles]);
+            }
+        }
         const int tx = tile % q.tiles_x;
         tile /= q.tiles_x;
         const int ty = tile % q.tiles_y;
@@ -632,6 +650,7 @@
         const float act_neg = p.act == TG_ACT_RELU ? 0.f : (p.act == TG_ACT_LEAKY ? p.slope : 1.f);
         const float gate_neg = p.gate_act == TG_ACT_LEAKY ? p.gate_slope : 0.f;
         const auto drsrc = __builtin_amdgcn_make_buffer_rsrc(p.dst, 0, (int)((size_t)p.B * p.DH * p.DW * p.N * 4), 0x00020000);
+        const int e_mdelta = SPARSE ? q.sp_nb * p.DH * p.DW * p.N * 4 : 0;
         f32x4 bq = {0.f, 0.f, 0.f, 0.f};
         if (p.bias && e_single) bq = *reinterpret_cast<const f32x4*>(p.bias + e_nb0 + 4 * (lane & 7));
         f32x4 pmx[POOL ? 4 : 1];
@@ -721,6 +740,10 @@
                         if (p.pool_only) return;
                     }
                     __builtin_amdgcn_raw_buffer_store_b128(__builtin_bit_cast(u32x4, o), drsrc, e_voff + (uint32_t)soff, 0, 0);
+                    if constexpr (SPARSE) {
+                        if (ci.mirror)
+                            __builtin_amdgcn_raw_buffer_store_b128(__builtin_bit_cast(u32x4, o), drsrc, e_voff + (uint32_t)(soff - e_mdelta), 0, 0);
+                    }
                 } else {
                     const int t = 32 * mw + rr;
                     const int oy = ci.oy0 + 2 * (t >> 3) + xh, ox = ci.ox0 + 2 * (t & 7) + j;
@@ -770,6 +793,13 @@
                     const int pix = (ci.b * PH + prow) * PW + (ci.ox0 >> 1);
                     __builtin_amdgcn_raw_buffer_store_b128(__builtin_bit_cast(u32x4, m), prsrc, p_voff + (uint32_t)((pix * p.N + e_nb0) * 4), 0, 0);
                     if (p.pool_code) __builtin_amdgcn_raw_buffer_store_b32(code, crsrc, c_voff + (uint32_t)(pix * p.N + e_nb0), 0, 0);
+                    if constexpr (SPARSE) {
+                        if (ci.mirror) {
+                            const int mpix = pix - q.sp_nb * PH * PW;
+                            __builtin_amdgcn_raw_buffer_store_b128(__builtin_bit_cast(u32x4, m), prsrc, p_voff + (uint32_t)((mpix * p.N + e_nb0) * 4), 0, 0);
+                            if (p.pool_code) __builtin_amdgcn_raw_buffer_store_b32(code, crsrc, c_voff + (uint32_t)(mpix * p.N + e_nb0), 0, 0);
+                        }
+                    }
                 }
             }
         }
@@ -842,13 +872,14 @@
     const bool pipe = fast && !no_pipe && nchunks - (p.splits - 1) * q.chunks_per_split >= 2 && q.chunks_per_split >= 2 &&
                       (size_t)p.B * p.DH * p.DW * p.N * 4 < ((size_t)1 << 31);
     typedef void (*WinoKern)(const IGemmParams, const WinoGeom, const float*);
-    static const WinoKern kerns[16] = {wino_kernel<false, false, false>, wino_kernel<false, true, false>, wino_kernel<true, false, false>,
+    static const WinoKern kerns[18] = {wino_kernel<false, false, false>, wino_kernel<false, true, false>, wino_kernel<true, false, false>,
                                        wino_kernel<true, true, false>, wino_pipe_kernel<false, false>, wino_pipe_kernel<true, false>,
                                        wino_kernel<false, false, true>, wino_kernel<false, true, true>, wino_kernel<true, false, true>,
                                        wino_kernel<true, true, true>, wino_pipe_kernel<false, true>, wino_pipe_kernel<true, true>,
                                        wino_pipe_kernel<false, false, true>, wino_pipe_kernel<false, true, true>,
-                                       wino_pipe_kernel<true, false, false, true>, wino_pipe_kernel<true, true, false, true>};
-    static LdsOptIn opts[16];
+                                       wino_pipe_kernel<true, false, false, true>, wino_pipe_kernel<true, true, false, true>,
+                                       wino_pipe_kernel<false, false, false, false, true>, wino_pipe_kernel<false, false, true, false, true>};
+    static LdsOptIn opts[18];
     q.qctr = wino_queue_block(s, p.splits, q.total_work);
     static const bool no_pool = getenv("TG_NO_FUSED_POOL") != nullptr;
     const bool pool = p.pool_dst && !no_pool && pipe && !gated && p.splits == 1 && !(p.OH & 1) && !(p.OW & 1) && p.ds == 1 && p.dy0 == 0 &&
@@ -858,7 +889,16 @@
     TG_REQUIRE(!p.pool_code || p.act == TG_ACT_RELU, "tg_conv_fwd_pool_code: needs a ReLU output");
     const bool gbits = p.gate_bits != nullptr && pipe && p.splits == 1;
     if (gbits) p.gate_bits_done = 1;
-    const int ki = gbits ? (q.qctr ? 15 : 14)
+    const TgSparseMap* sm = p.sparse;
+    const bool sparse = sm && pipe && !gated && !gbits && !q.qctr && p.splits == 1 && !p.accumulate && !p.rowscale && p.ds == 1 &&
+                        p.dy0 == 0 && p.dx0 == 0 && p.DH == p.OH && p.DW == p.OW && (pool || !p.pool_dst) && sm->nb > 0 &&
+                        p.B == 2 * sm->nb && sm->tiles_y == q.tiles_y && sm->tiles_x == q.tiles_x && sm->bits && sm->list && sm->count;
+    if (sparse) {
+        q.sp_bits = sm->bits; q.sp_list = sm->list; q.sp_count = sm->count;
+        q.sp_nb = sm->nb; q.sp_tiles = sm->nb * q.tiles_y * q.tiles_x;
+    }
+    const int ki = sparse ? (pool ? 17 : 16)
+                 : gbits ? (q.qctr ? 15 : 14)
                  : pool ? (q.qctr ? 13 : 12) : (q.qctr ? 6 : 0) + (pipe ? 4 + (gated ? 1 : 0) : (fast ? 2 : 0) + (gated ? 1 : 0));
     if (int rc = lds_opt_in(opts[ki], reinterpret_cast<const void*>(kerns[ki]), lds, "wino")) return rc;
     {
diff --git a/terra-gan_amd/tg_hip/engine.py b/terra-gan_amd/tg_hip/engine.py
--- a/terra-gan_amd/tg_hip/engine.py
+++ b/terra-gan_amd/tg_hip/engine.py
@@ -19,6 +19,7 @@
 VGG_WINO4 = os.environ.get("TG_VGG_WINO4", "1") != "0"
 VGG_WINO4_FWD = os.environ.get("TG_VGG_WINO4_FWD", "0") == "1"
 VGG_WINO4_MINCH = int(os.environ.get("TG_VGG_WINO4_MINCH", "128"))
+VGG_SPARSE = os.environ.get("TG_VGG_SPARSE", "1") != "0"
 POOL_CODE = os.environ.get("TG_NO_POOL_CODE") is None
 
 
@@ -370,6 +371,10 @@
     h = img.reshape(*img.shape, 1)
     steps = []
     pooled = code = None
+    smaps = None
+    if VGG_SPARSE and nb is not None and 2 * nb == img.shape[0]:
+        smaps = O.vgg_sparse_map(img, nb, "".join("M" if it == "M" else "C" for it in VGG_TRUNK))
+    ci = -1
     for i, item in enumerate(VGG_TRUNK):
         if item == "M":
             o = pooled if pooled is not None else O.maxpool2_fwd(h)
@@ -378,14 +383,16 @@
             pooled = code = None
         else:
             w = V["0.folded"] if item == 0 else V[f"{item}.weight"]
+            ci += 1
+            sp = smaps.maps[ci] if smaps is not None else None
             O.tag(f"vgg{item}.fwd")
             pool = i + 1 < len(VGG_TRUNK) and VGG_TRUNK[i + 1] == "M" and h.shape[1] % 2 == 0 and h.shape[2] % 2 == 0
             w4 = _vgg_wino4(w, h.shape[0], h.shape[1], h.shape[2], w.shape[0], wino4, VGG_WINO4_FWD)
             if pool and POOL_CODE and not w4 and O.conv_pool_code_supported(tuple(h.shape), w.shape[0]):
-                pooled, code = O.conv_fwd_pool_code(h, w, V[f"{item}.bias"])
+                pooled, code = O.conv_fwd_pool_code(h, w, V[f"{item}.bias"], sparse=sp)
                 o = None
             else:
-                o = O.conv_fwd(h, w, V[f"{item}.bias"], 3, 1, 1, act=O.ACT_RELU, pool=pool, wino4=w4)
+                o = O.conv_fwd(h, w, V[f"{item}.bias"], 3, 1, 1, act=O.ACT_RELU, pool=pool, wino4=w4, sparse=sp)
                 if pool:
                     o, pooled = o
             if gates:
diff --git a/terra-gan_amd/tg_hip/lib.py b/terra-gan_amd/tg_hip/lib.py
--- a/terra-gan_amd/tg_hip/lib.py
+++ b/terra-gan_amd/tg_hip/lib.py
@@ -25,6 +25,10 @@
 
 class TgBnAct(C.Structure):
     _fields_ = [(n, C.c_void_p) for n in ("mean", "rstd", "gamma", "beta")] + [("act", C.c_int32), ("slope", C.c_float)]
+
+
+class TgSparseMap(C.Structure):
+    _fields_ = [(n, C.c_void_p) for n in ("bits", "list", "count")] + [(n, C.c_int32) for n in ("nb", "tiles_y", "tiles_x", "_pad")]
 
 
 class TgRasterPlan(C.Structure):
@@ -59,6 +63,9 @@
     "tg_conv_pool_code_supported": (I, [CP]),
     "tg_conv_fwd_pool_code": (I, [CP, P, P, P, P, P, P, P, SZ, P]),
     "tg_maxpool2_bwd_code": (I, [P, P, I, I, I, I, P, P]),
+    "tg_vgg_sparse_map_bytes": (SZ, [I, I, I, C.c_char_p]),
+    "tg_vgg_sparse_map": (I, [P, I, I, I, C.c_char_p, P, SZ, P, C.POINTER(TgSparseMap), P]),
+    "tg_conv_fwd_sparse": (I, [CP, P, P, P, P, I, F, P, P, P, C.POINTER(TgSparseMap), P, SZ, P]),
     "tg_conv_bnin_supported": (I, [CP, I]),
     "tg_conv_fwd_bnin": (I, [CP, P, C.POINTER(TgBnAct), P, P, I, F, P, P, SZ, P]),
     "tg_conv_wgrad_bnin": (I, [CP, P, C.POINTER(TgBnAct), P, P, P, P, SZ, P]),
diff --git a/terra-gan_amd/tg_hip/ops.py b/terra-gan_amd/tg_hip/ops.py
--- a/terra-gan_amd/tg_hip/ops.py
+++ b/terra-gan_amd/tg_hip/ops.py
@@ -180,8 +180,51 @@
     return ent[2]
 
 
-def conv_fwd(x, w, bias, k, stride, pad, in_mask=None, ratio=None, act=ACT_NONE, slope=0.0, wino4=False, pool=False):
+_sparse_tickets = {}
+
+
+class SparseMaps:
+
+    def __init__(self, buf, maps):
+        self.buf, self.maps = buf, maps
+
+
+def vgg_sparse_map(x, nb, plan):
+    _chk(x, "x")
+    H, W = x.shape[1], x.shape[2]
+    assert x.shape[0] == 2 * nb and x.numel() == 2 * nb * H * W, (tuple(x.shape), nb)
+    lib = _lib()
+    pb = plan.encode()
+    nbytes = lib.tg_vgg_sparse_map_bytes(nb, H, W, pb)
+    if nbytes == 0:
+        return None
+    dev = x.device.index if x.device.index is not None else torch.cuda.current_device()
+    ticket = _sparse_tickets.get(dev)
+    if ticket is None or ticket.numel() < nb + 1:
+        if torch.cuda.is_current_stream_capturing():
+            return None
+        ticket = _sparse_tickets[dev] = torch.zeros(max(nb + 1, 64), dtype=torch.int32, device=x.device)
+    buf = torch.empty(nbytes, dtype=torch.uint8, device=x.device)
+    nconv = plan.count("C")
+    maps = (L.TgSparseMap * nconv)()
+    L.check(lib.tg_vgg_sparse_map(_p(x), nb, H, W, pb, _p(buf), nbytes, _p(ticket), maps, _stream()), "tg_vgg_sparse_map")
+    return SparseMaps(buf, maps)
+
+
+def conv_fwd(x, w, bias, k, stride, pad, in_mask=None, ratio=None, act=ACT_NONE, slope=0.0, wino4=False, pool=False, sparse=None):
     _chk(x, "x"); _chk(bias, "bias"); _chk(in_mask, "in_mask"); _chk(ratio, "ratio")
+    if sparse is not None:
+        assert in_mask is None and ratio is None
+        wv = weight_view(w)
+        _chk(wv, "weight")
+        g = conv_geom(x, wv.shape[0], k, stride, pad, wino4)
+        y = empty(g.B, g.Ho, g.Wo, g.Cout, like=x)
+        yp = empty(g.B, g.Ho // 2, g.Wo // 2, g.Cout, like=x) if pool else None
+        lib = _lib()
+        ws = workspace(lib.tg_conv_fwd_ws_bytes(C.byref(g)))
+        L.check(lib.tg_conv_fwd_sparse(C.byref(g), _p(x), _p(wv), _p(_prepared(w, wv, g, WPREP_FWD)), _p(bias), act, slope, _p(y),
+                                       _p(yp), None, C.byref(sparse), _p(ws), ws.numel() * 4, _stream()), "tg_conv_fwd_sparse")
+        return (y, yp) if pool else y
     wv = weight_view(w)
     _chk(wv, "weight")
     g = conv_geom(x, wv.shape[0], k, stride, pad, wino4)
@@ -236,7 +279,7 @@
     return bool(_lib().tg_conv_pool_code_supported(C.byref(g)))
 
 
-def conv_fwd_pool_code(x, w, bias):
+def conv_fwd_pool_code(x, w, bias, sparse=None):
     _chk(x, "x"); _chk(bias, "bias")
     wv = weight_view(w)
     _chk(wv, "weight")
@@ -245,6 +288,11 @@
     code = torch.empty((g.B, g.Ho // 2, g.Wo // 2, g.Cout), dtype=torch.uint8, device=x.device)
     lib = _lib()
     ws = workspace(lib.tg_conv_fwd_ws_bytes(C.byref(g)))
+    if sparse is not None:
+        L.check(lib.tg_conv_fwd_sparse(C.byref(g), _p(x), _p(wv), _p(_prepared(w, wv, g, WPREP_FWD)), _p(bias), ACT_RELU, 0.0, None,
+                                       _p(yp), C.c_void_p(code.data_ptr()), C.byref(sparse), _p(ws), ws.numel() * 4, _stream()),
+                "tg_conv_fwd_sparse")
+        return yp, code
     L.check(lib.tg_conv_fwd_pool_code(C.byref(g), _p(x), _p(wv), _p(_prepared(w, wv, g, WPREP_FWD)), _p(bias), _p(yp),
                                       C.c_void_p(code.data_ptr()), _p(ws), ws.numel() * 4, _stream()), "tg_conv_fwd_pool_code")
     return yp, code
```

After: 1051, median of 6. 1.04x the previous value.
